# theEricMa/TriplaneTurbo

Hardware: AMD Instinct MI355X
Metric: rendered rays/sec (fwd+bwd) at 256x256 rays x 128 samples (higher is better)
Workload: dtype f32 (fp32-grade: exact 3-piece fp16 operand split, 6 x v_mfma_f32_32x32x16_f16 per k-step, fp32 accumulation)

## Files before the change

### include/tt_abi.h

```cpp
#ifndef TT_ABI_H
#define TT_ABI_H

#include <stdint.h>

#ifdef __cplusplus
extern "C" {
#endif

#define TT_ABI_VERSION 17
#define TT_CHANNELS 32
#define TT_HIDDEN 64

typedef enum {
    TT_OK = 0,
    TT_ERR_BAD_ARG = -1,
    TT_ERR_UNSUPPORTED = -2,
    TT_ERR_LAUNCH = -3,
    TT_ERR_DEVICE = -4
} tt_status;

typedef struct {
    const float* w1;
    const float* w2;
    const float* w3;
    const float* v1;
    const float* v2;
    const float* v3;
} tt_mlp_weights;

typedef struct {
    float* w1;
    float* w2;
    float* w3;
    float* v1;
    float* v2;
    float* v3;
} tt_mlp_grads;

typedef struct {
    int32_t n_prompts;
    int32_t views_per_prompt;
    int32_t plane_h, plane_w;
    int32_t rays_per_view;
    int32_t n_samples;
    int64_t n_rays;
    float radius;
    float sdf_bias_radius;
    float inv_std;
    float cos_anneal_ratio;
    float rgb_grad_shrink;
    int32_t flags;
    int32_t image_w;
    int32_t tile_sb;
    int32_t grad_copies;
    int32_t tile_chunk;
    float skip_eps_tex;
    float skip_eps_geo;
    const float* inv_std_dev;
    uint64_t* stats;
} tt_render_cfg;

#define TT_R_PER_SAMPLE 1
#define TT_R_EXACT_F32 2
#define TT_R_SPLIT2 32
#define TT_R_SPLIT3 64

#define TT_R_VOLSDF 128

#define TT_R_WGRAD_F32 4
#define TT_R_BWD_SOLO 8
#define TT_R_BWD_PAIR 16

#define TT_Q_NORMAL 1
#define TT_Q_TEX 2
#define TT_Q_EXACT_F32 4
#define TT_Q_SPLIT2 8
#define TT_Q_SPLIT3 16

const char* tt_strerror(int status);
int tt_abi_version(void);
const char* tt_source_hash(void);
int tt_debug_poison_queue(void* stream);

int tt_planes_pack(const float* space_cache, float* packed, int32_t n_prompts, int32_t plane_h, int32_t plane_w,
                   void* stream);
int tt_planes_unpack_grad(const float* grad_packed, float* grad_space_cache, int32_t n_prompts, int32_t plane_h,
                          int32_t plane_w, int32_t n_copies, void* stream);

int tt_query_points(const float* packed, const tt_mlp_weights* w, const float* points, int32_t n_batch,
                    int64_t n_points, int32_t n_prompts, int32_t views_per_prompt, int32_t plane_h, int32_t plane_w,
                    float radius, float sdf_bias_radius, int32_t flags, float* out_sdf, float* out_sdf_grad,
                    float* out_features, void* stream);

int tt_query_field(const float* packed, const tt_mlp_weights* w, const float* points, int32_t n_batch,
                   int64_t n_points, int32_t n_prompts, int32_t views_per_prompt, int32_t plane_h, int32_t plane_w,
                   float radius, float sdf_bias_radius, int32_t flags, float* out_sdf, float* out_deformation,
                   void* stream);

int tt_decode_rays(const float* packed, const tt_mlp_weights* w, const float* rays_o, const float* rays_d,
                   const float* t_starts, const float* t_ends, const tt_render_cfg* cfg, int32_t flags, float* sdf,
                   float* sdf_grad, float* features, void* stream);

enum tt_sample_placement { TT_PLACE_TT = 0, TT_PLACE_CENTER = 1 };
#define TT_PLACE_VOLSDF 0x100

int tt_sample_uniform(int64_t n_rays, int32_t n_samples, float near_plane, float far_plane, const float* jitter,
                      int32_t placement, float* t_starts, float* t_ends, void* stream);

int tt_sample_importance(const float* t_starts, const float* t_ends, const float* sdf, int64_t n_rays,
                         int32_t n_proposal, int32_t n_fine, float inv_std, const float* inv_std_dev,
                         float render_step_size, const float* u_jitter, int32_t placement, float* out_t_starts,
                         float* out_t_ends, void* stream);

int tt_render_fwd(const float* packed, const tt_mlp_weights* w, const float* rays_o, const float* rays_d,
                  const float* t_starts, const float* t_ends, const tt_render_cfg* cfg, float* opacity, float* depth,
                  float* rgb_fg, float* z_variance, float* normal_acc, float* weights, float* trans, float* sdf,
                  float* sdf_grad, float* features, void* stream);

int tt_render_fwd_h2mask(const float* packed, const tt_mlp_weights* w, const float* rays_o, const float* rays_d,
                         const float* t_starts, const float* t_ends, const tt_render_cfg* cfg, float* opacity,
                         float* depth, float* rgb_fg, float* z_variance, float* normal_acc, float* weights, float* trans,
                         float* sdf, float* sdf_grad, float* features, uint32_t* h2_mask, void* stream);

int tt_render_eval(const float* packed, const tt_mlp_weights* w, const float* rays_o, const float* rays_d,
                   const float* t_starts, const float* t_ends, const tt_render_cfg* cfg, float transmittance_eps,
                   float weight_eps, float* opacity, float* depth, float* rgb_fg, float* z_variance, float* normal_acc,
                   uint64_t* stats, void* stream);

int tt_march_fwd(const float* rays_d, const float* t_starts, const float* t_ends, const tt_render_cfg* cfg,
                 const float* sdf, const float* sdf_grad, const float* features, float* opacity, float* depth,
                 float* rgb_fg, float* z_variance, float* normal_acc, float* weights, float* trans, void* stream);

int tt_march_bwd(const float* rays_d, const float* t_starts, const float* t_ends, const tt_render_cfg* cfg,
                 const float* opacity, const float* depth, const float* trans, const float* sdf,
                 const float* sdf_grad, const float* features, const float* g_opacity, const float* g_depth,
                 const float* g_rgb_fg, const float* g_z_variance, const float* g_normal_acc, const float* g_weights,
                 const float* g_sdf, const float* g_sdf_grad, float* g_inv_std_rays, float* out_grad, void* stream);

int tt_render_bwd_geo(const float* packed, const tt_mlp_weights* w, const float* rays_o, const float* rays_d,
                      const float* t_starts, const float* t_ends, const tt_render_cfg* cfg, const float* opacity,
                      const float* depth, const float* trans, const float* sdf, const float* sdf_grad,
                      const float* features, const float* g_opacity, const float* g_depth, const float* g_rgb_fg,
                      const float* g_z_variance, const float* g_normal_acc, const float* g_weights,
                      const float* g_sdf, const float* g_sdf_grad, float* g_inv_std_rays, float* workspace,
                      float* grad_packed, const tt_mlp_grads* grads, void* stream);

int tt_render_bwd_geo_h2mask(const float* packed, const tt_mlp_weights* w, const float* rays_o, const float* rays_d,
                             const float* t_starts, const float* t_ends, const tt_render_cfg* cfg,
                             const float* opacity, const float* depth, const float* trans, const float* sdf,
                             const float* sdf_grad, const float* features, const float* g_opacity,
                             const float* g_depth, const float* g_rgb_fg, const float* g_z_variance,
                             const float* g_normal_acc, const float* g_weights, const float* g_sdf,
                             const float* g_sdf_grad, float* g_inv_std_rays, float* workspace, float* grad_packed,
                             const tt_mlp_grads* grads, const uint32_t* h2_mask, void* stream);

int tt_render_bwd_tex(const float* packed, const tt_mlp_weights* w, const float* rays_o, const float* rays_d,
                      const float* t_starts, const float* t_ends, const tt_render_cfg* cfg, const float* weights,
                      const float* features, const float* g_rgb_fg, const float* g_features, float* grad_packed,
                      const tt_mlp_grads* grads, void* stream);

int tt_points_bwd_geo(const float* packed, const tt_mlp_weights* w, const float* points, int32_t n_batch,
                      int64_t n_points, int32_t n_prompts, int32_t views_per_prompt, int32_t plane_h, int32_t plane_w,
                      float radius, float sdf_bias_radius, int32_t flags, const float* g_sdf, const float* g_sdf_grad,
                      float* workspace, float* grad_packed, const tt_mlp_grads* grads, void* stream);
int tt_points_bwd_tex(const float* packed, const tt_mlp_weights* w, const float* points, int32_t n_batch,
                      int64_t n_points, int32_t n_prompts, int32_t views_per_prompt, int32_t plane_h, int32_t plane_w,
                      float radius, int32_t plane_base, int32_t flags, const float* g_features, float* grad_packed,
                      const tt_mlp_grads* grads, void* stream);

int tt_points_bwd_x(const float* packed, const tt_mlp_weights* w, const float* points, int32_t n_batch,
                    int64_t n_points, int32_t n_prompts, int32_t views_per_prompt, int32_t plane_h, int32_t plane_w,
                    float radius, int32_t flags, const float* g_sdf, const float* g_sdf_grad, const float* g_features,
                    float* grad_points, void* stream);

typedef struct {
    int32_t n_levels;
    int32_t n_features_per_level;
    int32_t log2_hashmap_size;
    int32_t base_resolution;
    float per_level_scale;
} tt_hashgrid_cfg;
int64_t tt_hashgrid_n_params(const tt_hashgrid_cfg* cfg);
int tt_hashgrid_fwd(const float* x, int64_t n, const float* params, const tt_hashgrid_cfg* cfg, float* out,
                    void* stream);
int tt_hashgrid_bwd(const float* x, int64_t n, const float* g_out, const tt_hashgrid_cfg* cfg, float* grad_params,
                    void* stream);

int tt_patch_composite_fwd(const float* low, const float* patch, float* out, int32_t B, int32_t h, int32_t w, int32_t H,
                           int32_t W, int32_t C, int32_t PS, int32_t py, int32_t px, void* stream);
int tt_patch_composite_bwd(const float* g_out, float* g_low, float* g_patch, int32_t B, int32_t h, int32_t w, int32_t H,
                           int32_t W, int32_t C, int32_t PS, int32_t py, int32_t px, void* stream);

int tt_eikonal_fwd(const float* sdf_grad, int64_t n, float* loss, void* stream);
int tt_eikonal_bwd(const float* sdf_grad, const float* g_loss, int64_t n, float* g_sdf_grad, void* stream);

int tt_composite_fwd(const float* opacity, const float* depth, const float* rgb_fg, const float* normal_acc,
                     const float* bg, int32_t bg_stride, const float* camera_distances, const float* c2w, int64_t n_rays,
                     int32_t rays_per_view, int32_t mode, int32_t view_group, float* comp_rgb, float* disparity,
                     float* comp_normal, float* normal_cam_vis, float* normal_cam_vis_white, void* stream);
int tt_composite_bwd(const float* opacity, const float* depth, const float* rgb_fg, const float* normal_acc,
                     const float* bg, int32_t bg_stride, const float* camera_distances, const float* c2w, int64_t n_rays,
                     int32_t rays_per_view, int32_t mode, int32_t view_group, const float* g_comp_rgb,
                     const float* g_disparity, const float* g_comp_normal, const float* g_normal_cam_vis,
                     const float* g_normal_cam_vis_white, float* g_opacity, float* g_depth, float* g_rgb_fg,
                     float* g_normal_acc, float* g_bg, void* stream);

#define TT_DTYPE_F32 0
#define TT_DTYPE_F16 1
#define TT_DTYPE_F64 2
int tt_grid_sample_2d_grad2_typed(int32_t dtype, const void* grad2_grad_input, const void* grad2_grad_grid,
                                  const void* grad_output, const void* input, const void* grid, int32_t n, int32_t c,
                                  int32_t h, int32_t w, int64_t n_points_per_batch, int32_t padding_mode,
                                  int32_t align_corners, void* grad_grad_output, void* grad_input, void* grad_grid,
                                  void* stream);
int tt_grid_sample_2d_grad2(const float* grad2_grad_input, const float* grad2_grad_grid, const float* grad_output,
                            const float* input, const float* grid, int32_t n, int32_t c, int32_t h, int32_t w,
                            int64_t n_points_per_batch, int32_t padding_mode, int32_t align_corners,
                            float* grad_grad_output, float* grad_input, float* grad_grid, void* stream);

#define TT_MC_MAX_RES 512
int64_t tt_mc_workspace_bytes(int32_t res);
int tt_mc_count(const float* level, int32_t res, float isovalue, void* workspace, int32_t* out_totals, void* stream);
int tt_mc_emit(const float* level, const float* deformation, int32_t res, float isovalue, void* workspace, float* v_pos,
               int32_t* t_pos_idx, void* stream);
int tt_mc_bwd(const float* level, const float* deformation, int32_t res, float isovalue, void* workspace,
              const float* grad_v, float* grad_level, float* grad_deformation, void* stream);

int64_t tt_mt_workspace_bytes(int32_t n_edges, int32_t n_tets);
int tt_mt_count(const float* level, const int32_t* edges, const int32_t* tets, int32_t n_edges, int32_t n_tets,
                void* workspace, int32_t* out_totals, void* stream);
int tt_mt_emit(const float* pos, const float* level, const int32_t* edges, const int32_t* tet_edge, int32_t n_edges,
               int32_t n_tets, void* workspace, float* v_pos, int32_t* t_pos_idx, void* stream);
int tt_mt_bwd(const float* pos, const float* level, const int32_t* edges, const int32_t* vert_ptr,
              const int32_t* vert_col, int32_t n_vertices, int32_t n_edges, int32_t n_tets, void* workspace,
              const float* grad_v, float* grad_level, float* grad_pos, void* stream);

#define TT_RAST_MAX_TRIS (1 << 24)
int64_t tt_rast_workspace_bytes(int32_t B, int32_t T, int32_t H, int32_t W);
int tt_rast_fwd(const float* pos, const int32_t* tri, int32_t B, int32_t V, int32_t T, int32_t H, int32_t W,
                void* workspace, float* rast, void* stream);
int tt_rast_bwd(const float* pos, const int32_t* tri, const float* rast, const float* grad_rast, int32_t B, int32_t V,
                int32_t T, int32_t H, int32_t W, float* grad_pos, void* stream);
int tt_interp_fwd(const float* attr, int32_t attr_batch, const float* rast, const int32_t* tri, int32_t B, int32_t V,
                  int32_t T, int32_t H, int32_t W, int32_t C, float* out, void* stream);
int tt_interp_bwd(const float* attr, int32_t attr_batch, const float* rast, const int32_t* tri, const float* grad_out,
                  int32_t B, int32_t V, int32_t T, int32_t H, int32_t W, int32_t C, float* grad_attr, float* grad_rast,
                  void* stream);
int tt_aa_fwd(const float* color, const float* rast, const float* pos, const int32_t* tri, const int32_t* edge_ofs,
              const int32_t* edge_tri, int32_t B, int32_t V, int32_t T, int32_t H, int32_t W, int32_t C, float* out,
              void* stream);
int tt_aa_bwd(const float* color, const float* rast, const float* pos, const int32_t* tri, const int32_t* edge_ofs,
              const int32_t* edge_tri, const float* grad_out, int32_t B, int32_t V, int32_t T, int32_t H, int32_t W,
              int32_t C, float* grad_color, float* grad_pos, void* stream);
int64_t tt_rast_range_workspace_bytes(int32_t B, int64_t n_slots, int32_t H, int32_t W);
int tt_rast_range_fwd(const float* pos, const int32_t* tri, const int32_t* ranges_dev, const int32_t* ranges_host,
                      int32_t B, int32_t V, int32_t T, int32_t H, int32_t W, void* workspace, float* rast,
                      void* stream);
int tt_rast_range_bwd(const float* pos, const int32_t* tri, const float* rast, const float* grad_rast, int32_t B,
                      int32_t V, int32_t T, int32_t H, int32_t W, float* grad_pos, void* stream);
int tt_aa_range_fwd(const float* color, const float* rast, const float* pos, const int32_t* tri,
                    const int32_t* edge_ofs, const int32_t* edge_tri, int32_t B, int32_t V, int32_t T, int32_t H,
                    int32_t W, int32_t C, float* out, void* stream);
int tt_aa_range_bwd(const float* color, const float* rast, const float* pos, const int32_t* tri,
                    const int32_t* edge_ofs, const int32_t* edge_tri, const float* grad_out, int32_t B, int32_t V,
                    int32_t T, int32_t H, int32_t W, int32_t C, float* grad_color, float* grad_pos, void* stream);

#define TT_TEX_FILTER_NEAREST 0
#define TT_TEX_FILTER_LINEAR 1
#define TT_TEX_BOUNDARY_WRAP 0
#define TT_TEX_BOUNDARY_CLAMP 1
#define TT_TEX_BOUNDARY_ZERO 2
#define TT_TEX_MAX_SIZE 16777216
int tt_tex_fwd(const float* tex, int32_t tex_batch, const float* uv, int32_t B, int32_t H, int32_t W, int32_t TH,
               int32_t TW, int32_t C, int32_t filter, int32_t boundary, float* out, void* stream);
int tt_tex_bwd(const float* tex, int32_t tex_batch, const float* uv, const float* grad_out, int32_t B, int32_t H,
               int32_t W, int32_t TH, int32_t TW, int32_t C, int32_t filter, int32_t boundary, float* grad_tex,
               float* grad_uv, void* stream);

#define TT_MESH_MAX_ITEMS (1 << 28)
#define TT_MESH_COS_EPS 1e-8f
int64_t tt_mesh_workspace_bytes(int32_t V, int32_t T);
int tt_mesh_components(const int32_t* face_pairs, int32_t P, int32_t T, void* workspace, int32_t* labels,
                       void* stream);
int tt_mesh_compact_count(const int32_t* t_pos_idx, const int32_t* labels, int32_t V, int32_t T, int32_t frac_mode,
                          double frac, int64_t threshold, void* workspace, int32_t* out_totals, void* stream);
int tt_mesh_compact_emit(const float* v_pos, const int32_t* t_pos_idx, int32_t V, int32_t T, void* workspace,
                         float* v_out, int32_t* t_out, void* stream);
int tt_mesh_laplacian_fwd(const float* v_pos, const int32_t* nbr_ptr, const int32_t* nbr_col, int32_t V, int32_t T,
                          void* workspace, float* loss, void* stream);
int tt_mesh_laplacian_bwd(const float* v_pos, const int32_t* nbr_ptr, const int32_t* nbr_col, int32_t V, int32_t T,
                          const float* grad_loss, void* workspace, float* grad_v, void* stream);
int tt_mesh_nc_fwd(const float* v_nrm, const int32_t* edges, int32_t V, int32_t T, int32_t E, void* workspace,
                   float* loss, void* stream);
int tt_mesh_nc_bwd(const float* v_nrm, const int32_t* nbr_ptr, const int32_t* nbr_col, int32_t V, int32_t E,
                   const float* grad_loss, float* grad_nrm, void* stream);

#define TT_UV_DEFAULT_ROUNDS 8
#define TT_UV_DEFAULT_TAU 0.3f
#define TT_UV_MAX_TAU 0.577f
#define TT_UV_MAX_SMOOTH_ROUNDS 1024
#define TT_UV_MAX_FACES ((1 << 24) - 1)
#define TT_UV_MAX_TEX 16384
#define TT_UV_MAX_PADDING 256
#define TT_UV_MAX_CHANNELS 64
#define TT_UV_MAX_OVERLAP_ROUNDS 4
#define TT_UV_PACK_REL_PREC 1e-4
int64_t tt_uv_workspace_bytes(int32_t V, int32_t T, int32_t N);
int tt_uv_labels(const float* v_pos, const int32_t* t_pos_idx, const int32_t* face_pairs, int32_t V, int32_t T,
                 int32_t P, int32_t rounds, float tau, int32_t N, void* workspace, int32_t* labels, void* stream);
int tt_uv_charts(const float* v_pos, const int32_t* t_pos_idx, const int32_t* face_pairs, const int32_t* labels,
                 const uint8_t* singleton, int32_t V, int32_t T, int32_t P, int32_t N, void* workspace, int32_t* chart,
                 float* chart_box, int32_t* out_totals, void* stream);
int tt_uv_pack(const float* chart_box, int32_t C, int32_t N, int32_t padding, int32_t* offsets, float* scale);
int tt_uv_emit_count(const int32_t* t_pos_idx, const int32_t* chart, int32_t V, int32_t T, int32_t N, void* workspace,
                     int32_t* out_totals, void* stream);
int tt_uv_emit(const float* v_pos, const int32_t* t_pos_idx, const int32_t* labels, const int32_t* chart,
               const float* chart_box, const int32_t* offsets, int32_t C, float scale, int32_t V, int32_t T, int32_t N,
               int32_t padding, void* workspace, float* v_tex, int32_t* t_tex_idx, void* stream);
int tt_uv_overlap(const float* v_tex, const int32_t* t_tex_idx, int32_t Vt, int32_t V, int32_t T, int32_t N,
                  void* workspace, uint8_t* flags, int32_t* out_totals, void* stream);
int64_t tt_tex_fill_workspace_bytes(int32_t H, int32_t W);
int tt_tex_fill(const float* img, const uint8_t* mask, int32_t H, int32_t W, int32_t C, void* workspace, float* out,
                void* stream);

#define TT_SIMPLIFY_MIN_GRID 2
#define TT_SIMPLIFY_MAX_GRID 1024
#define TT_SIMPLIFY_MAX_CLUSTERS 2097151
int64_t tt_simplify_workspace_bytes(int32_t V, int32_t T);
int tt_simplify_keys(const float* v_pos, int32_t V, int32_t grid, float lo_x, float lo_y, float lo_z, float inv_h,
                     int64_t* keys, void* stream);
int tt_simplify_ranks(const int64_t* sorted_keys, const int64_t* perm, int32_t V, int32_t T, int32_t grid,
                      void* workspace, int32_t* rank, int32_t* out_totals, void* stream);
int tt_simplify_pairs(const int32_t* t_pos_idx, const int32_t* rank, int32_t V, int32_t T, int32_t C, void* workspace,
                      int64_t* pair_keys, void* stream);
int tt_simplify_solve(const float* v_pos, const int32_t* t_pos_idx, const int64_t* sorted_pair_keys,
                      const int64_t* perm, int32_t V, int32_t T, int32_t C, int32_t grid, float lo_x, float lo_y,
                      float lo_z, float h, double lam, void* workspace, float* cluster_pos, void* stream);
int tt_simplify_faces(const int32_t* t_pos_idx, const int32_t* rank, int32_t V, int32_t T, int32_t C,
                      int64_t* face_keys, void* stream);
int tt_simplify_emit_count(const int64_t* sorted_face_keys, const int64_t* face_perm, const int32_t* t_pos_idx,
                           const int32_t* rank, int32_t V, int32_t T, int32_t C, void* workspace, int32_t* out_totals,
                           void* stream);
int tt_simplify_emit(const float* cluster_pos, const int32_t* t_pos_idx, const int32_t* rank, int32_t V, int32_t T,
                     int32_t C, void* workspace, float* v_out, int32_t* t_out, int32_t* vertex_map, void* stream);

#define TT_BAKE_GROUP_POS 0
#define TT_BAKE_GROUP_TEX 1
#define TT_BAKE_MAX_POINTS 268435456
int tt_bake_tangents(const float* v_pos, const int32_t* t_pos_idx, const float* v_tex, const int32_t* t_tex_idx,
                     const float* v_nrm, const int32_t* group_ptr, const int32_t* group_corner, int32_t V, int32_t Vt,
                     int32_t T, int32_t group, float* out, void* stream);
int tt_bake_project(float* points, const float* sdf, const float* sdf_grad, const uint8_t* mask, int64_t M,
                    float max_step, void* stream);
int tt_bake_encode(const float* rast, const float* v_nrm, const int32_t* t_pos_idx, const float* tng_tex,
                   const int32_t* t_tex_idx, const float* field_nrm, int32_t V, int32_t Vt, int32_t T, int32_t H,
                   int32_t W, float* out, int32_t* out_counts, void* stream);

#define TT_DIST_MAX_GRID 256
#define TT_DIST_MAX_SAMPLES (1 << 26)
int64_t tt_dist_workspace_bytes(int32_t grid);
int tt_dist_build_count(const float* v_pos, const int32_t* t_pos_idx, int32_t V, int32_t T, int32_t grid, float lo_x,
                        float lo_y, float lo_z, float ext, float inv_h, void* workspace, float* records,
                        int32_t* cell_ptr, int64_t* out_total, void* stream);
int tt_dist_build_fill(const float* records, int32_t T, int32_t grid, float lo_x, float lo_y, float lo_z, float ext,
                       float inv_h, void* workspace, const int32_t* cell_ptr, int32_t M, int32_t* cell_tri,
                       void* stream);
int tt_dist_keys(const float* points, int32_t N, int32_t grid, float lo_x, float lo_y, float lo_z, float ext,
                 float inv_h, int64_t* keys, void* stream);
int tt_dist_query(const float* points, const int64_t* order, int32_t N, const float* records, const int32_t* cell_ptr,
                  const int32_t* cell_tri, int32_t T, int32_t M, int32_t grid, float lo_x, float lo_y, float lo_z,
                  float ext, float h, float inv_h, float* d2, int32_t* face, float* bary, void* stream);
int tt_dist_bwd(const float* points, const float* v_pos, const int32_t* t_pos_idx, const int32_t* face,
                const float* bary, const float* g_d2, int32_t N, int32_t V, int32_t T, float* grad_points,
                float* grad_v_pos, void* stream);
int64_t tt_dist_sample_workspace_bytes(int32_t T);
int tt_dist_sample_count(const float* v_pos, const int32_t* t_pos_idx, int32_t V, int32_t T, float spacing,
                         void* workspace, int64_t* offsets, void* stream);
int tt_dist_sample_emit(const float* v_pos, const int32_t* t_pos_idx, const int64_t* offsets, int32_t V, int32_t T,
                        float spacing, int32_t S, float* points, int32_t* face, void* stream);

#define TT_WIND_MAX_LEVELS 6
int64_t tt_wind_node_count(int32_t levels);
int tt_wind_face_keys(const float* v_pos, const int32_t* t_pos_idx, int32_t V, int32_t T, int32_t levels, float lo_x,
                      float lo_y, float lo_z, float ext, float inv_h, float* records, int64_t* keys, void* stream);
int tt_wind_build(const float* sorted_records, const int32_t* leaf_ptr, int32_t T, int32_t levels, float* nodes,
                  void* stream);
int tt_wind_point_keys(const float* points, int32_t N, int32_t levels, float lo_x, float lo_y, float lo_z, float ext,
                       float inv_h, int64_t* keys, void* stream);
int tt_wind_exact(const float* points, int32_t N, const float* records, int32_t T, float* out, void* stream);
int tt_wind_fast(const float* points, const int64_t* order, int32_t N, const float* sorted_records,
                 const int32_t* leaf_ptr, const float* nodes, int32_t T, int32_t levels, float beta, float* out,
                 void* stream);

#define TT_RAY_MAX_DIRS 1024
int tt_ray_cast(const float* origins, const float* dirs, const int64_t* order, int32_t N, float t_max,
                const float* records, const int32_t* cell_ptr, const int32_t* cell_tri, int32_t T, int32_t M,
                int32_t grid, float lo_x, float lo_y, float lo_z, float ext, float h, float inv_h, float* t,
                int32_t* face, float* bary, void* stream);
int tt_ray_any(const float* origins, const float* dirs, const int64_t* order, int32_t N, float t_max,
               const float* records, const int32_t* cell_ptr, const int32_t* cell_tri, int32_t T, int32_t M,
               int32_t grid, float lo_x, float lo_y, float lo_z, float ext, float h, float inv_h, uint8_t* hit,
               void* stream);
int tt_ray_ao(const float* points, const float* normals, const float* dirs_local, int32_t N, int32_t K, float bias,
              float max_distance, const float* records, const int32_t* cell_ptr, const int32_t* cell_tri, int32_t T,
              int32_t M, int32_t grid, float lo_x, float lo_y, float lo_z, float ext, float h, float inv_h,
              int32_t* hits, void* stream);

#ifdef __cplusplus
}
#endif
#endif
```

### triplaneturbo_amd/csrc/tt_backward.hip

```cpp
#include "tt_backward_common.h"

struct BwdGeoParams {
    const float* packed;
    MlpPtrs w;
    const float* rays_o;
    const float* rays_d;
    const float* t_starts;
    const float* t_ends;
    tt_render_cfg cfg;
    TileGeom geom;
    long long n_items;
    int* queue;
    const float* ws;
    const unsigned* h2_mask;
    int n_copies;
    float* grad_packed;
    MlpGradPtrs grads;
    unsigned long long* phase_cycles;
};

#define GEO_SCRATCH_FLOATS (2 * 64 * XS)
template <int PREC, bool FMASK>
struct GeoMap : LdsMap<PREC, LdsImage<64, 32>, LdsImage<64, 64, !(FMASK && PREC != PREC_F32)>, LdsRows<1, 64>,
                       LdsImage<32, 64>, LdsImage<64, 64>> {
    static constexpr bool NOW2 = FMASK && PREC != PREC_F32;
    typedef typename GeoMap::template at<0> W1;
    typedef typename GeoMap::template at<1> W2;
    typedef typename GeoMap::template at<2> W3;
    typedef typename GeoMap::template at<3> W1T;
    typedef typename GeoMap::template at<4> CT;
};

template <int PREC, bool STATS = false, bool FMASK = false>
__global__ __launch_bounds__(256, 1) void k_decode_bwd_geo(BwdGeoParams p) {
    constexpr bool EXACT = PREC == PREC_F32;
    constexpr bool WG16 = !EXACT;
    typedef GeoMap<PREC, FMASK> G;
    constexpr int NT = PrecNT<PREC>::value, WF = G::FLOATS;
    __shared__ __attribute__((aligned(16))) float L[WF + 4 * (GEO_SCRATCH_FLOATS + SCATTER_TAG_INTS)];
    stage_weights<PREC>(L, typename G::W1{}, p.w.w1);
    if constexpr (!G::NOW2) stage_weights<PREC>(L, typename G::W2{}, p.w.w2);
    stage_weights<PREC>(L, typename G::W3{}, p.w.w3);
    stage_weights_t<PREC>(L, typename G::W1T{}, p.w.w1);
    if constexpr (!EXACT) stage_image16_rowscaled_t<NT>(L, typename G::CT{}, p.w.w2, p.w.w3);
    const tt_render_cfg& cfg = p.cfg;
    float sA1 = 1.f, sU = 1.f, sV = 1.f;
    if (WG16) {
        const unsigned* bnd = reinterpret_cast<const unsigned*>(p.queue) + TT_SLOT_BOUNDS;
        const float Pm = __builtin_bit_cast(float, bnd[TT_BOUND_PLANES]), Sb = __builtin_bit_cast(float, bnd[TT_BOUND_UP0]),
                    Gb = __builtin_bit_cast(float, bnd[TT_BOUND_UP1]);
        unsigned* word = reinterpret_cast<unsigned*>(L + WF);
        const int t = threadIdx.x;
        float w1row = 0.f, a1col = 0.f;
        if (t < 64) {
            for (int c = 0; c < 32; ++c) w1row += __builtin_fabsf(p.w.w1[t * 32 + c]);
            for (int r = 0; r < 64; ++r) a1col += __builtin_fabsf(p.w.w2[r * 64 + t]) * __builtin_fabsf(p.w.w3[r]);
        }
        const float W1max = block_max(w1row, word), A1max = block_max(a1col, word);
        const float jsum = (0.5f * cfg.plane_w + 0.5f * cfg.plane_h) / cfg.radius;
        const float Fmax = 3.f * Pm, H1max = W1max * Fmax;
        const float Umax = Fmax * (Sb + 2.f * jsum * Gb), QBmax = Fmax * 2.f * jsum * Gb;
        const float Vmax = Sb * H1max + W1max * QBmax;
        sA1 = wg16_scale(A1max);
        sU = wg16_scale(Umax);
        sV = wg16_scale(Vmax);
    }
    const TileGeom& tg = p.geom;
    const int lane = threadIdx.x & 63, i = lane & 31, hi = lane >> 5, wave_in_blk = threadIdx.x >> 6;
    float* Xs = L + WF + wave_in_blk * (GEO_SCRATCH_FLOATS + SCATTER_TAG_INTS);
    float* Ys = Xs + 64 * XS;
    int* tags = reinterpret_cast<int*>(Ys + 64 * XS);
    scatter_init_tags(tags, lane);
    __syncthreads();
    const int S = cfg.n_samples;
    ItemQueue iq = item_queue(p.queue, tg.n_blocks, tg.n_chunks, tg.unit);
    const int H = cfg.plane_h, W = cfg.plane_w;
    const size_t HW = (size_t)H * W;
    const size_t plane_stride = 6 * HW * TT_C;
    const float ju = 0.5f * W / cfg.radius, jv = 0.5f * H / cfg.radius;
    float* const grad_out =
        p.grad_packed + (size_t)(blockIdx.x % (unsigned)p.n_copies) * cfg.n_prompts * plane_stride;
    const unsigned grad_bytes =
        TT_DBG(cfg.flags, TT_DBG_NO_ATOMICS) ? 0u : (unsigned)(cfg.n_prompts * plane_stride * sizeof(float));

    const TileStats st = STATS ? tile_stats(cfg.stats) : TileStats{nullptr};
    f32x16 accW1[2][1] = {{ZERO16}, {ZERO16}};
    f32x16 accW2[2][2] = {{ZERO16, ZERO16}, {ZERO16, ZERO16}};
#ifdef TT_TUNING
    unsigned long long ph_acc[20] = {0, 0, 0, 0, 0, 0, 0, 0, 0, 0, 0, 0, 0, 0, 0, 0, 0, 0, 0, 0};
    unsigned long long ph_t = __builtin_amdgcn_s_memtime();
#endif

#pragma nounroll
    for (;;) {
        long long b;
        int ck;
        if (!item_pop(iq, tg.order, tg.n_chunks, b, ck)) break;
        if (b >= tg.n_blocks) continue;
        bool ray_ok;
        const long long ray = tile_ray(tg, b, i, ray_ok);
        const float ray_okf = tt_opaque(ray_ok ? 1.f : 0.f);
        const int ks = i % tg.sb;
        const int view = (int)(ray / cfg.rays_per_view);
        const size_t pofs = (size_t)(view / cfg.views_per_prompt) * plane_stride;
        const float ox = p.rays_o[ray * 3 + 0], oy = p.rays_o[ray * 3 + 1], oz = p.rays_o[ray * 3 + 2];
        const float dx = p.rays_d ? p.rays_d[ray * 3 + 0] : 0.f, dy = p.rays_d ? p.rays_d[ray * 3 + 1] : 0.f,
                    dz = p.rays_d ? p.rays_d[ray * 3 + 2] : 0.f;
        const int s_end = (ck + 1) * tg.chunk < S ? (ck + 1) * tg.chunk : S;
        struct StepIn {
            f32x4 up;
            float ts, te;
            unsigned m2;
        };
        auto load_step = [&](int sb0) {
            StepIn r;
            const int si = sb0 + ks;
            const long long sidx = ray * S + (si < S ? si : S - 1);
            r.up = *reinterpret_cast<const f32x4*>(p.ws + sidx * 4);
            r.ts = p.rays_d ? p.t_starts[sidx] : 0.f;
            r.te = p.rays_d ? p.t_ends[sidx] : 0.f;
            r.m2 = FMASK ? p.h2_mask[2 * sidx + hi] : 0u;
            return r;
        };
        StepIn in = load_step(ck * tg.chunk), in_next;
#pragma nounroll
        for (int sb0 = ck * tg.chunk; sb0 < s_end; sb0 += tg.sb, in = in_next) {
            in_next = load_step(sb0 + tg.sb);
            const int si = sb0 + ks;
            const bool rvalid = ray_ok && si < s_end;
            const float vf = ray_okf * (si < s_end ? 1.f : 0.f);
            const float sbar = in.up[0] * vf, gbx = in.up[1] * vf, gby = in.up[2] * vf, gbz = in.up[3] * vf;
            tile_stat(st, TT_STAT_VISITED);
            TT_PHASE(0);
            if (!__any(!((__builtin_fabsf(sbar) + __builtin_fabsf(gbx)) + (__builtin_fabsf(gby) + __builtin_fabsf(gbz)) <=
                         cfg.skip_eps_geo)))
                continue;
            float tm, px, py, pz;
            sample_position(ox, oy, oz, dx, dy, dz, in.ts, in.te, tm, px, py, pz);
            const float X = scale_coord(px, cfg.radius), Y = scale_coord(py, cfg.radius),
                        Z = scale_coord(pz, cfg.radius);
            float f[16], u[16];
            unsigned pmask;
            const bool any = __any(gather_geo_bwd_c(p.packed, (unsigned)(pofs / TT_C), H, W, X, Y, Z, rvalid, sbar, gbx,
                                                    gby, gbz, ju, jv, lane, Xs, f, u, pmask,
                                                    tile_stat_ptr(st, TT_STAT_INBOUNDS)));
            TT_PHASE(1);
            if (!any) continue;
            const bool one = single_plane(pmask);
            tile_stat_executed(st, one);
            float h1[32], h2[32], a1[32], q[16], u1, uh2;
            mvx<PREC, true>(L, typename G::W1{}, f, h1, i, hi, 1.f, &u1);
#pragma unroll
            for (int r = 0; r < 32; ++r) h1[r] = fmaxf(h1[r], 0.f);
            const unsigned m2w = FMASK ? in.m2 & (0u - (unsigned)vf) : 0u;
            if constexpr (!FMASK) {
                mvx<PREC, true>(L, typename G::W2{}, h1, h2, i, hi, u1, &uh2);
#pragma unroll
                for (int r = 0; r < 32; ++r) h2[r] = fmaxf(h2[r], 0.f);
            } else if constexpr (EXACT) {
#pragma unroll
                for (int r = 0; r < 32; ++r) h2[r] = (float)((m2w >> r) & 1u);
            }
            unsigned m2p[16];
            Split16<64, PAIR_SEQ, NT> a1s;
            float ua1 = 1.f;
            if (WG16) {
                if constexpr (FMASK)
                    mask16_pairs_bits<64>(m2w, m2p);
                else
                    mask16_pairs<64>(h2, m2p);
                mv16_mask<NT>(L, typename G::CT{}, m2p, a1, i, hi, &ua1);
            } else {
                float a2[32];
#pragma unroll
                for (int g = 0; g < 8; ++g) {
                    f32x4 w3 = *reinterpret_cast<const f32x4*>(lds_at(L, typename G::W3{}) + 8 * g + 4 * hi);
#pragma unroll
                    for (int e2 = 0; e2 < 4; ++e2) a2[4 * g + e2] = h2[4 * g + e2] > 0.f ? w3[e2] : 0.f;
                }
                mvtx_copy<PREC>(L, typename G::CT{}, typename G::W2{}, a2, a1, i, hi);
            }
#pragma unroll
            for (int r = 0; r < 32; ++r) a1[r] = h1[r] > 0.f ? a1[r] : 0.f;
            float uq = 1.f;
            if (WG16) {
                split16_vec<64, PAIR_SEQ, NT>(a1, sA1 * ua1, a1s);
                mv16_pre<true, true>(L, typename G::W1T{}, a1s, 1.f / sA1, q, i, hi, &uq);
            } else {
                mvtx_copy<PREC>(L, typename G::W1T{}, typename G::W1{}, a1, q, i, hi);
            }
            TT_PHASE(3);
            {
                float qb[16];
#pragma unroll
                for (int r = 0; r < 16; ++r) qb[r] = fmaf(-sbar, f[r], u[r]);
                const bool region = WG16 || cfg.flags >= 0;
                const bool do_wgrad = region && !TT_DBG(cfg.flags, TT_DBG_NO_WGRAD);
                if (do_wgrad) {
                    if (WG16) {
                        stage_rows16_pre<64>(Xs, a1s, i, hi);
                        stage_rows16<32>(Ys, u, i, hi, sU);
                        wgrad16<64, 32>(accW1, Xs, Ys, i, hi);
                    } else {
                        stage_rows<64>(Xs, a1, i, hi);
                        stage_rows<32>(Ys, u, i, hi);
                        wgrad<64, 32>(accW1, Xs, Ys, i, hi);
                    }
                }
                TT_PHASE(7);
                float t1[32];
                mvx<PREC>(L, typename G::W1{}, qb, t1, i, hi);
#pragma unroll
                for (int r = 0; r < 32; ++r) t1[r] = h1[r] > 0.f ? t1[r] : 0.f;
                float v[32];
#pragma unroll
                for (int r = 0; r < 32; ++r) v[r] = fmaf(sbar * u1, h1[r], t1[r]);
                TT_PHASE(4);
                if (do_wgrad) {
                    if (WG16) {
                        stage_rows16_mask<64>(Xs, m2p, i, hi);
                        stage_rows16<64>(Ys, v, i, hi, sV);
                        wgrad16_mask<64, 64>(accW2, Xs, Ys, i, hi);
                    } else {
                        stage_rows_mask<64>(Xs, h2, i, hi);
                        stage_rows<64>(Ys, v, i, hi);
                        wgrad<64, 64>(accW2, Xs, Ys, i, hi);
                    }
                }
                TT_PHASE(8);
                if (region && !TT_DBG(cfg.flags, TT_DBG_NO_SCATTER)) {
                    scatter_clear<EXACT>(Xs, lane);
                    float* Qs = Xs + SCATTER_M_FLOATS;
                    TT_PHASE(9);
                    const int tex0 = (int)(pofs / TT_C);
                    auto corners = [&](int pl, PlaneRefs& refs) {
                        Corners c;
                        float coef[4];
                        geo_corner_coefs(pl, H, W, X, Y, Z, rvalid, sbar, gbx, gby, gbz, ju, jv, c, coef);
                        int aoff[4];
#pragma unroll
                        for (int q4 = 0; q4 < 4; ++q4) aoff[q4] = tex0 + (int)(pl * HW) + c.off[q4];
                        refs = plane_refs<!EXACT>(coef, aoff, c.hs, hi);
                    };
#ifdef TT_TUNING
                    unsigned long long* const sc_st = ph_acc + 14;
#else
                    unsigned long long* const sc_st = nullptr;
#endif
                    const ScatterQ<EXACT> sq{Qs, tags, i, hi};
                    if (one)
                        scatter_one_plane<EXACT>(grad_out, grad_bytes, sq, Xs, Qs + 32 * 33,
                                                 single_plane_index(pmask), corners, q, uq, sc_st);
                    else
                        scatter_planes<EXACT>(grad_out, grad_bytes, sq, Xs, Qs + 32 * 33, corners, [&](int) { return q; }, uq, sc_st);
                    TT_PHASE(10);
                }
            }
        }
    }
#ifdef TT_TUNING
    TT_PHASE(11);
    if (p.phase_cycles && lane == 0)
        for (int k = 0; k < 20; ++k) atomicAdd(p.phase_cycles + 20 + k, ph_acc[k]);
#endif
    __syncthreads();
    int parity = 0;
    flush_wgrad_reduced<64, 32>(L, parity, accW1, p.grads.w1, wave_in_blk, lane, 1.f / sA1, 1.f / sU);
    flush_d_reduced<64, 64>(L, parity, accW2, p.w.w2, p.w.w3, p.grads.w2, p.grads.w3, wave_in_blk, lane, 1.f / sV);
    tile_stats_flush(st);
}

#ifdef TT_TUNING
unsigned long long* g_phase_cycles = nullptr;
extern "C" int tt_tuning_phase_cycles(unsigned long long* out40) {
    if (!g_phase_cycles) {
        if (hipMalloc((void**)&g_phase_cycles, 40 * sizeof(unsigned long long)) != hipSuccess) return -4;
        if (hipMemset(g_phase_cycles, 0, 40 * sizeof(unsigned long long)) != hipSuccess) return -4;
    }
    if (hipDeviceSynchronize() != hipSuccess) return -4;
    if (out40 && hipMemcpy(out40, g_phase_cycles, 40 * sizeof(unsigned long long), hipMemcpyDeviceToHost) != hipSuccess)
        return -4;
    return hipMemset(g_phase_cycles, 0, 40 * sizeof(unsigned long long)) == hipSuccess ? 0 : -4;
}
#endif
static void launch_bwd_geo(const BwdGeoParams& p0, long long blocks, hipStream_t s) {
    BwdGeoParams p = p0;
#ifdef TT_TUNING
    p.phase_cycles = g_phase_cycles;
#else
    p.phase_cycles = nullptr;
#endif
    if (use_wg16(p.cfg)) {
        unsigned* bnd = reinterpret_cast<unsigned*>(p.queue) + TT_SLOT_BOUNDS;
        launch_planes_bound(p.packed, p.cfg, 0, bnd + TT_BOUND_PLANES, s);
        const long long n = p.cfg.n_rays * p.cfg.n_samples;
        hipLaunchKernelGGL(k_absmax4, dim3(absmax_blocks(n), 1), dim3(256), 0, s, reinterpret_cast<const f32x4*>(p.ws), n, n,
                           bnd + TT_BOUND_UP0, bnd + TT_BOUND_UP1);
    }
    tt_dispatch_prec(tt_prec_of_r(p.cfg.flags), [&](auto P) {
        constexpr int PREC = decltype(P)::value;
        const dim3 grid((unsigned)blocks), block(256);
        if (p.cfg.stats && p.h2_mask)
            hipLaunchKernelGGL((k_decode_bwd_geo<PREC, true, true>), grid, block, 0, s, p);
        else if (p.cfg.stats)
            hipLaunchKernelGGL((k_decode_bwd_geo<PREC, true>), grid, block, 0, s, p);
        else if (p.h2_mask)
            hipLaunchKernelGGL((k_decode_bwd_geo<PREC, false, true>), grid, block, 0, s, p);
        else
            hipLaunchKernelGGL((k_decode_bwd_geo<PREC>), grid, block, 0, s, p);
    });
}

static int render_bwd_geo(const float* packed, const tt_mlp_weights* w, const float* rays_o, const float* rays_d,
                          const float* t_starts, const float* t_ends, const tt_render_cfg* cfg, const float* opacity,
                          const float* depth, const float* trans, const float* sdf, const float* sdf_grad,
                          const float* features, const float* g_opacity, const float* g_depth, const float* g_rgb_fg,
                          const float* g_z_variance, const float* g_normal_acc, const float* g_weights,
                          const float* g_sdf, const float* g_sdf_grad, float* g_inv_std_rays, float* workspace,
                          float* grad_packed, const tt_mlp_grads* grads, const uint32_t* h2_mask, void* stream) {
    int st = tt_validate_cfg(cfg);
    if (st != TT_OK) return st;
    if (!packed || !w || !rays_o || !rays_d || !t_starts || !t_ends || !opacity || !depth || !trans || !sdf ||
        !sdf_grad || !features || !workspace || !grad_packed || !grads)
        return TT_ERR_BAD_ARG;
    if (!w->w1 || !w->w2 || !w->w3 || !grads->w1 || !grads->w2 || !grads->w3) return TT_ERR_BAD_ARG;
    if (grad_buffer_too_large(cfg)) return TT_ERR_UNSUPPORTED;
    int cus = tt_num_cus();
    if (cus <= 0) return TT_ERR_DEVICE;
    hipStream_t s = (hipStream_t)stream;
    st = tt_launch_march_bwd(rays_d, t_starts, t_ends, cfg, sdf, sdf_grad, features, trans, opacity, depth, g_opacity,
                             g_depth, g_rgb_fg, g_z_variance, g_normal_acc, g_weights, g_sdf, g_sdf_grad, g_inv_std_rays,
                             workspace, s);
    if (st != TT_OK) return st;
    BwdGeoParams p;
    tt_fill_rays(p, packed, w, rays_o, rays_d, t_starts, t_ends, *cfg);
    p.cfg.flags |= debug_flags();
    p.ws = workspace;
    p.h2_mask = h2_mask;
    p.grad_packed = grad_packed;
    p.n_copies = cfg->grad_copies > 0 ? cfg->grad_copies : 1;
    p.grads = to_gptrs(grads);
    st = tt_plan_queue(cfg, 4LL * cus, s, &p.geom, &p.n_items, &p.queue);
    if (st != TT_OK) return st;
    launch_bwd_geo(p, tt_persistent_blocks(p.n_items, cus, 4), s);
    return tt_check_launch();
}

extern "C" int tt_render_bwd_geo(const float* packed, const tt_mlp_weights* w, const float* rays_o,
                                 const float* rays_d, const float* t_starts, const float* t_ends,
                                 const tt_render_cfg* cfg, const float* opacity, const float* depth,
                                 const float* trans, const float* sdf, const float* sdf_grad, const float* features,
                                 const float* g_opacity, const float* g_depth, const float* g_rgb_fg,
                                 const float* g_z_variance, const float* g_normal_acc, const float* g_weights,
                                 const float* g_sdf, const float* g_sdf_grad, float* g_inv_std_rays, float* workspace,
                                 float* grad_packed, const tt_mlp_grads* grads, void* stream) {
    return render_bwd_geo(packed, w, rays_o, rays_d, t_starts, t_ends, cfg, opacity, depth, trans, sdf, sdf_grad, features,
                          g_opacity, g_depth, g_rgb_fg, g_z_variance, g_normal_acc, g_weights, g_sdf, g_sdf_grad,
                          g_inv_std_rays, workspace, grad_packed, grads, nullptr, stream);
}

extern "C" int tt_render_bwd_geo_h2mask(const float* packed, const tt_mlp_weights* w, const float* rays_o,
                                        const float* rays_d, const float* t_starts, const float* t_ends,
                                        const tt_render_cfg* cfg, const float* opacity, const float* depth,
                                        const float* trans, const float* sdf, const float* sdf_grad,
                                        const float* features, const float* g_opacity, const float* g_depth,
                                        const float* g_rgb_fg, const float* g_z_variance, const float* g_normal_acc,
                                        const float* g_weights, const float* g_sdf, const float* g_sdf_grad,
                                        float* g_inv_std_rays, float* workspace, float* grad_packed,
                                        const tt_mlp_grads* grads, const uint32_t* h2_mask, void* stream) {
    if (!h2_mask) return TT_ERR_BAD_ARG;
    return render_bwd_geo(packed, w, rays_o, rays_d, t_starts, t_ends, cfg, opacity, depth, trans, sdf, sdf_grad, features,
                          g_opacity, g_depth, g_rgb_fg, g_z_variance, g_normal_acc, g_weights, g_sdf, g_sdf_grad,
                          g_inv_std_rays, workspace, grad_packed, grads, h2_mask, stream);
}

__global__ void k_interleave_ws(const float* __restrict__ g_sdf, const float* __restrict__ g_sdf_grad,
                                float* __restrict__ ws, long long n) {
    const long long i = (long long)blockIdx.x * blockDim.x + threadIdx.x;
    if (i >= n) return;
    f32x4 o = {g_sdf ? g_sdf[i] : 0.f, g_sdf_grad ? g_sdf_grad[i * 3 + 0] : 0.f,
               g_sdf_grad ? g_sdf_grad[i * 3 + 1] : 0.f, g_sdf_grad ? g_sdf_grad[i * 3 + 2] : 0.f};
    *reinterpret_cast<f32x4*>(ws + i * 4) = o;
}

extern "C" int tt_points_bwd_geo(const float* packed, const tt_mlp_weights* w, const float* points, int32_t n_batch,
                                 int64_t n_points, int32_t n_prompts, int32_t views_per_prompt, int32_t plane_h,
                                 int32_t plane_w, float radius, float sdf_bias_radius, int32_t flags,
                                 const float* g_sdf, const float* g_sdf_grad, float* workspace, float* grad_packed,
                                 const tt_mlp_grads* grads, void* stream) {
    tt_render_cfg cfg;
    int st = points_cfg(&cfg, n_batch, n_points, n_prompts, views_per_prompt, plane_h, plane_w, radius,
                        sdf_bias_radius, 1, flags);
    if (st != TT_OK) return st;
    if (grad_buffer_too_large(&cfg)) return TT_ERR_UNSUPPORTED;
    if (!packed || !w || !points || !workspace || !grad_packed || !grads || (!g_sdf && !g_sdf_grad))
        return TT_ERR_BAD_ARG;
    if (!w->w1 || !w->w2 || !w->w3 || !grads->w1 || !grads->w2 || !grads->w3) return TT_ERR_BAD_ARG;
    int cus = tt_num_cus();
    if (cus <= 0) return TT_ERR_DEVICE;
    hipStream_t s = (hipStream_t)stream;
    const long long n = cfg.n_rays;
    hipLaunchKernelGGL(k_interleave_ws, dim3((unsigned)((n + 255) / 256)), dim3(256), 0, s, g_sdf, g_sdf_grad,
                       workspace, n);
    st = tt_check_launch();
    if (st != TT_OK) return st;
    BwdGeoParams p;
    tt_fill_rays(p, packed, w, points, nullptr, nullptr, nullptr, cfg);
    p.ws = workspace;
    p.h2_mask = nullptr;
    p.grad_packed = grad_packed;
    p.n_copies = 1;
    p.grads = to_gptrs(grads);
    st = tt_plan_queue(&cfg, 4LL * cus, s, &p.geom, &p.n_items, &p.queue);
    if (st != TT_OK) return st;
    launch_bwd_geo(p, tt_persistent_blocks(p.n_items, cus, 4), s);
    return tt_check_launch();
}
```

### triplaneturbo_amd/csrc/tt_device.h

```cpp
#pragma once
#include <hip/hip_runtime.h>
#include <stdint.h>

typedef float f32x16 __attribute__((ext_vector_type(16)));
typedef float f32x4 __attribute__((ext_vector_type(4)));

#ifdef TT_TUNING
#define TT_DBG(flags, bit) (((flags) & (bit)) != 0)
#else
#define TT_DBG(flags, bit) false
#endif
#define TT_DBG_NO_SCATTER 0x100
#define TT_DBG_NO_WGRAD 0x200
#define TT_DBG_NO_GATHER 0x400
#define TT_DBG_NO_MLP 0x800
#define TT_DBG_NO_STORE 0x1000
#define TT_DBG_NO_ATOMICS 0x2000

#define TT_C 32
#define TT_TILE 32

#define LIDX(r, hi) (((r) & 3) + 8 * ((r) >> 2) + 4 * (hi))

#include "tt_mask.h"
// ... 25 lines not shown
#pragma unroll
    for (int m = 0; m < MT; ++m) {
        acc[m] = f32x16{0.f, 0.f, 0.f, 0.f, 0.f, 0.f, 0.f, 0.f, 0.f, 0.f, 0.f, 0.f, 0.f, 0.f, 0.f, 0.f};
        a_cur[m] = *reinterpret_cast<const f32x4*>(row + 32 * m * (NIN + 4));
    }
#pragma unroll
    for (int g = 0; g < NIN / 8; ++g) {
        if (g + 1 < NIN / 8) {
#pragma unroll
            for (int m = 0; m < MT; ++m)
                a_nxt[m] = *reinterpret_cast<const f32x4*>(row + 32 * m * (NIN + 4) + 8 * (g + 1));
        }
#pragma unroll
        for (int k = 0; k < 4; ++k)
#pragma unroll
            for (int m = 0; m < MT; ++m)
                acc[m] = __builtin_amdgcn_mfma_f32_32x32x2f32(a_cur[m][k], x[4 * g + k], acc[m], 0, 0, 0);
#pragma unroll
        for (int m = 0; m < MT; ++m) a_cur[m] = a_nxt[m];
    }
#pragma unroll
    for (int m = 0; m < MT; ++m)
#pragma unroll
        for (int k = 0; k < 16; ++k) y[16 * m + k] = acc[m][k];
}

template <int NOUT, int NIN, int NG>
__device__ __forceinline__ void mv_fwd_cols(const float* Wl, const float (&x)[4 * NG], int g0, float (&y)[NOUT / 2], int i,
                                            int hi) {
    constexpr int MT = NOUT / 32;
    f32x16 acc[MT];
    const float* row = Wl + i * (NIN + 4) + 4 * hi + 8 * g0;
#pragma unroll
    for (int m = 0; m < MT; ++m)
        acc[m] = f32x16{0.f, 0.f, 0.f, 0.f, 0.f, 0.f, 0.f, 0.f, 0.f, 0.f, 0.f, 0.f, 0.f, 0.f, 0.f, 0.f};
#pragma unroll
    for (int g = 0; g < NG; ++g) {
        f32x4 a[MT];
#pragma unroll
        for (int m = 0; m < MT; ++m) a[m] = *reinterpret_cast<const f32x4*>(row + 32 * m * (NIN + 4) + 8 * g);
#pragma unroll
        for (int k = 0; k < 4; ++k)
#pragma unroll
            for (int m = 0; m < MT; ++m)
                acc[m] = __builtin_amdgcn_mfma_f32_32x32x2f32(a[m][k], x[4 * g + k], acc[m], 0, 0, 0);
    }
#pragma unroll
    for (int m = 0; m < MT; ++m)
#pragma unroll
        for (int k = 0; k < 16; ++k) y[16 * m + k] = acc[m][k];
}

template <int NOUT, int NIN, int STRIDE = NOUT + 4>
__device__ __forceinline__ void mv_bwd(const float* Wl, const float (&x)[NIN / 2], float (&y)[NOUT / 2], int i,
                                       int hi) {
    constexpr int MT = NOUT / 32;
    const float* base = Wl + 4 * hi * STRIDE + i;
    if (MT == 1) {
        f32x16 acc0 = {0.f, 0.f, 0.f, 0.f, 0.f, 0.f, 0.f, 0.f, 0.f, 0.f, 0.f, 0.f, 0.f, 0.f, 0.f, 0.f};
        f32x16 acc1 = acc0;
#pragma unroll
        for (int r = 0; r < NIN / 4; ++r) {
            const float a0 = base[LIDX(r, 0) * STRIDE], a1 = base[LIDX(r + NIN / 4, 0) * STRIDE];
            acc0 = __builtin_amdgcn_mfma_f32_32x32x2f32(a0, x[r], acc0, 0, 0, 0);
            acc1 = __builtin_amdgcn_mfma_f32_32x32x2f32(a1, x[r + NIN / 4], acc1, 0, 0, 0);
        }
#pragma unroll
        for (int k = 0; k < 16; ++k) y[k] = acc0[k] + acc1[k];
    } else {
        f32x16 acc[MT];
#pragma unroll
        for (int m = 0; m < MT; ++m)
            acc[m] = f32x16{0.f, 0.f, 0.f, 0.f, 0.f, 0.f, 0.f, 0.f, 0.f, 0.f, 0.f, 0.f, 0.f, 0.f, 0.f, 0.f};
#pragma unroll
        for (int r = 0; r < NIN / 2; ++r) {
#pragma unroll
            for (int m = 0; m < MT; ++m) {
                const float a = base[LIDX(r, 0) * STRIDE + 32 * m];
                acc[m] = __builtin_amdgcn_mfma_f32_32x32x2f32(a, x[r], acc[m], 0, 0, 0);
            }
        }
#pragma unroll
        for (int m = 0; m < MT; ++m)
#pragma unroll
            for (int k = 0; k < 16; ++k) y[16 * m + k] = acc[m][k];
    }
}

template <int N>
__device__ __forceinline__ float dot_lds(const float* wl, const float (&x)[N / 2], int hi) {
    float s = 0.f;
#pragma unroll
    for (int g = 0; g < N / 8; ++g) {
        f32x4 a = *reinterpret_cast<const f32x4*>(wl + 8 * g + 4 * hi);
        s = fmaf(a[0], x[4 * g + 0], s);
        s = fmaf(a[1], x[4 * g + 1], s);
        s = fmaf(a[2], x[4 * g + 2], s);
        s = fmaf(a[3], x[4 * g + 3], s);
    }
    return s + __shfl_xor(s, 32);
}

struct Corners {
    int off[4];
    float w[4];
    float du[4];
    float dv[4];
    int hs[4];
    bool any;
    int inmask;
};

#pragma clang fp contract(off)
__device__ __forceinline__ void corners_setup(float gx, float gy, int H, int W, bool valid, Corners& c) {
    gx = __builtin_fabsf(gx) < 1e30f ? gx : 4.f;
    gy = __builtin_fabsf(gy) < 1e30f ? gy : 4.f;
    float ix = ((gx + 1.f) * (float)W - 1.f) / 2.f;
    float iy = ((gy + 1.f) * (float)H - 1.f) / 2.f;
    float fx = floorf(ix), fy = floorf(iy);
    float wx1 = ix - fx, wx0 = (fx + 1.f) - ix;
    float wy1 = iy - fy, wy0 = (fy + 1.f) - iy;
    int x0 = (int)fminf(fmaxf(fx, -2.f), (float)W + 1.f);
    int y0 = (int)fminf(fmaxf(fy, -2.f), (float)H + 1.f);
    x0 = valid ? x0 : -2;
    const float bx0 = (unsigned)x0 < (unsigned)W ? 1.f : 0.f, bx1 = (unsigned)(x0 + 1) < (unsigned)W ? 1.f : 0.f;
    const float by0 = (unsigned)y0 < (unsigned)H ? 1.f : 0.f, by1 = (unsigned)(y0 + 1) < (unsigned)H ? 1.f : 0.f;
    const float mx0 = wx0 * bx0, mx1 = wx1 * bx1, my0 = wy0 * by0, my1 = wy1 * by1;
    c.w[0] = mx0 * my0;
    c.w[1] = mx1 * my0;
    c.w[2] = mx0 * my1;
    c.w[3] = mx1 * my1;
    c.du[0] = -(my0 * bx0);
    c.du[1] = my0 * bx1;
    c.du[2] = -(my1 * bx0);
    c.du[3] = my1 * bx1;
    c.dv[0] = -(mx0 * by0);
    c.dv[1] = -(mx1 * by0);
    c.dv[2] = mx0 * by1;
    c.dv[3] = mx1 * by1;
    const int xc0 = min(max(x0, 0), W - 1), xc1 = min(max(x0 + 1, 0), W - 1);
    const int yc0 = min(max(y0, 0), H - 1) * W, yc1 = min(max(y0 + 1, 0), H - 1) * W;
    c.off[0] = yc0 + xc0;
    c.off[1] = yc0 + xc1;
    c.off[2] = yc1 + xc0;
    c.off[3] = yc1 + xc1;
    const float i0 = bx0 * by0, i1 = bx1 * by0, i2 = bx0 * by1, i3 = bx1 * by1;
    c.hs[0] = ((y0 & 15) << 4) | (x0 & 15);
    c.hs[1] = ((y0 & 15) << 4) | ((x0 + 1) & 15);
    c.hs[2] = (((y0 + 1) & 15) << 4) | (x0 & 15);
    c.hs[3] = (((y0 + 1) & 15) << 4) | ((x0 + 1) & 15);
    c.any = (bx0 + bx1) * (by0 + by1) != 0.f;
    c.inmask = (int)i0 | ((int)i1 << 1) | ((int)i2 << 2) | ((int)i3 << 3);
}

__device__ __forceinline__ float scale_coord(float x, float radius) {
    float t = (x - (-radius)) / (radius - (-radius));
    return t * 2.f + (-1.f);
}

__device__ __forceinline__ void sample_position(float ox, float oy, float oz, float dx, float dy, float dz, float ts,
                                                float te, float& tm, float& px, float& py, float& pz) {
    tm = (ts + te) / 2.f;
    px = ox + dx * tm;
    py = oy + dy * tm;
    pz = oz + dz * tm;
}

__device__ __forceinline__ float sphere_bias(float px, float py, float pz, float bias_radius, float& nrm) {
    nrm = sqrtf((px * px + py * py) + pz * pz);
    return nrm - bias_radius;
}
#pragma clang fp contract(fast)

#define PLANE_U(p, X, Y, Z) ((p) == 2 ? (Z) : (X))
#define PLANE_V(p, X, Y, Z) ((p) == 1 ? (Z) : (Y))

template <bool NEED_J>
__device__ __forceinline__ bool gather_geo(const float* __restrict__ planes, int H, int W, float X, float Y, float Z,
                                           bool valid, float jscale_u, float jscale_v, int hi, float (&f)[16],
                                           float (&jx)[16], float (&jy)[16], float (&jz)[16], int dbg = 0) {
#pragma unroll
    for (int r = 0; r < 16; ++r) {
        f[r] = 0.f;
        jx[r] = 0.f;
        jy[r] = 0.f;
        jz[r] = 0.f;
    }
    bool any = false;
    const size_t HW = (size_t)H * W;
#pragma unroll
    for (int p = 0; p < 3; ++p) {
        Corners c;
        corners_setup(PLANE_U(p, X, Y, Z), PLANE_V(p, X, Y, Z), H, W, valid, c);
        if (!__any(c.any)) continue;
        any = any || c.any;
#pragma unroll
        for (int k = 0; k < 4; ++k) {
            const f32x4* t = reinterpret_cast<const f32x4*>(planes + (p * HW + (size_t)c.off[k]) * TT_C) + hi;
            f32x4 v[4];
            if (TT_DBG(dbg, TT_DBG_NO_GATHER)) {
                const f32x4 z = {c.w[k], c.du[k], c.dv[k], X};
                v[0] = v[1] = v[2] = v[3] = z;
            } else {
                v[0] = t[0];
                v[1] = t[2];
                v[2] = t[4];
                v[3] = t[6];
            }
            const float wk = c.w[k], a = c.du[k] * jscale_u, b = c.dv[k] * jscale_v;
#pragma unroll
            for (int q = 0; q < 4; ++q)
#pragma unroll
                for (int e = 0; e < 4; ++e) {
                    const float tv = v[q][e];
                    f[4 * q + e] = fmaf(wk, tv, f[4 * q + e]);
                    if (NEED_J) {
                        if (p == 0) {
                            jx[4 * q + e] = fmaf(a, tv, jx[4 * q + e]);
                            jy[4 * q + e] = fmaf(b, tv, jy[4 * q + e]);
                        } else if (p == 1) {
                            jx[4 * q + e] = fmaf(a, tv, jx[4 * q + e]);
                            jz[4 * q + e] = fmaf(b, tv, jz[4 * q + e]);
                        } else {
                            jz[4 * q + e] = fmaf(a, tv, jz[4 * q + e]);
                            jy[4 * q + e] = fmaf(b, tv, jy[4 * q + e]);
                        }
                    }
                }
        }
    }
    return any;
}

__device__ __forceinline__ bool gather_tex(const float* __restrict__ planes, int H, int W, float X, float Y, float Z,
                                           bool valid, int hi, float (&e)[48], int dbg = 0) {
#pragma unroll
    for (int r = 0; r < 48; ++r) e[r] = 0.f;
    bool any = false;
    const size_t HW = (size_t)H * W;
#pragma unroll
    for (int p = 0; p < 3; ++p) {
        Corners c;
        corners_setup(PLANE_U(p, X, Y, Z), PLANE_V(p, X, Y, Z), H, W, valid, c);
        if (!__any(c.any)) continue;
        any = any || c.any;
#pragma unroll
        for (int k = 0; k < 4; ++k) {
            const f32x4* t = reinterpret_cast<const f32x4*>(planes + ((3 + p) * HW + (size_t)c.off[k]) * TT_C) + hi;
            f32x4 v[4];
            if (TT_DBG(dbg, TT_DBG_NO_GATHER)) {
                const f32x4 z = {c.w[k], Y, Z, X};
                v[0] = v[1] = v[2] = v[3] = z;
            } else {
                v[0] = t[0];
                v[1] = t[2];
                v[2] = t[4];
                v[3] = t[6];
            }
            const float wk = c.w[k];
#pragma unroll
            for (int q = 0; q < 4; ++q)
#pragma unroll
                for (int ee = 0; ee < 4; ++ee) e[16 * p + 4 * q + ee] = fmaf(wk, v[q][ee], e[16 * p + 4 * q + ee]);
        }
    }
    return any;
}

struct TileStats {
    unsigned long long* p;
    unsigned* w;
};
enum { TT_STAT_VISITED = 0, TT_STAT_EXECUTED = 1, TT_STAT_INBOUNDS = 2, TT_STAT_SINGLE = 3 };
__device__ __forceinline__ TileStats tile_stats(uint64_t* stats64) {
    TileStats st = {nullptr, nullptr};
    __shared__ unsigned tt_stat_slots[16 * 4];
    st.p = reinterpret_cast<unsigned long long*>(stats64);
    if (st.p) {
        st.w = tt_stat_slots + 4 * __builtin_amdgcn_readfirstlane((int)(threadIdx.x >> 6));
        if ((threadIdx.x & 63) < 4) st.w[threadIdx.x & 63] = 0u;
    }
    return st;
}
__device__ __forceinline__ void tile_stat(const TileStats& st, int which, unsigned v = 1) {
    if (st.p) {
        if ((threadIdx.x & 63) == 0) st.w[which] += v;
    }
}
__device__ __forceinline__ void tile_stat_executed(const TileStats& st, bool single) {
    if (st.p) {
        if ((threadIdx.x & 63) == 0) {
            st.w[TT_STAT_EXECUTED] += 1u;
            st.w[TT_STAT_SINGLE] += single ? 1u : 0u;
        }
    }
}
__device__ __forceinline__ unsigned* tile_stat_ptr(const TileStats& st, int which) { return st.p ? st.w + which : nullptr; }
__device__ __forceinline__ void tile_stats_flush(const TileStats& st) {
    if (st.p) {
        const int l = threadIdx.x & 63;
        if (l < 4) atomicAdd(st.p + l, (unsigned long long)st.w[l]);
    }
}

__device__ __forceinline__ bool single_plane(unsigned pmask) { return pmask != 0u && (pmask & (pmask - 1u)) == 0u; }
__device__ __forceinline__ int single_plane_index(unsigned pmask) { return __builtin_ctz(pmask | 8u); }
__device__ __forceinline__ void live_block16(const float (&e)[48], float (&e1)[16]) {
#pragma unroll
    for (int r = 0; r < 16; ++r)
        e1[r] = __builtin_bit_cast(float, __builtin_bit_cast(unsigned, e[r]) | __builtin_bit_cast(unsigned, e[16 + r]) |
                                              __builtin_bit_cast(unsigned, e[32 + r]));
}

typedef int ti32x4 __attribute__((ext_vector_type(4)));
#define GC_TABLE_FLOATS(NW) (3 * 32 * 4 * (1 + (NW)))
#define GC_TILE_FLOATS (32 * 36)

#define GC_PLANE_TABLE_FLOATS (32 * 16)
#define GC_SCRATCH_FLOATS (GC_PLANE_TABLE_FLOATS + GC_TILE_FLOATS)

__device__ __forceinline__ const f32x4* gc_addr(const float* __restrict__ planes, int texel, unsigned cbyte) {
    return reinterpret_cast<const f32x4*>(reinterpret_cast<const char*>(planes) + (((unsigned)texel << 7) | cbyte));
}

__device__ __forceinline__ void gc_load16(const float* __restrict__ pl, const int* Toff, int js, f32x4 (&t)[4][4]) {
#pragma unroll
    for (int n = 0; n < 4; ++n) {
        const ti32x4 o4 = *reinterpret_cast<const ti32x4*>(Toff + (8 * n + js) * 4);
#pragma unroll
        for (int k = 0; k < 4; ++k) t[n][k] = *reinterpret_cast<const f32x4*>(pl + (size_t)(unsigned)o4[k] * TT_C);
    }
}

__device__ __forceinline__ void gc_transpose(float* R, const f32x4 (&acc)[4], int i, int hi, int js, int c,
                                             float* out16) {
#pragma unroll
    for (int n = 0; n < 4; ++n) *reinterpret_cast<f32x4*>(R + (8 * n + js) * 36 + 4 * c) = acc[n];
#pragma unroll
    for (int q = 0; q < 4; ++q) {
        const f32x4 v = *reinterpret_cast<const f32x4*>(R + i * 36 + 4 * (hi + 2 * q));
#pragma unroll
        for (int ee = 0; ee < 4; ++ee) out16[4 * q + ee] = v[ee];
    }
}

template <bool NEED_J>
__device__ __forceinline__ bool gather_geo_c(const float* __restrict__ planes, unsigned tex0, int H, int W, float X,
                                             float Y, float Z, bool valid, float jscale_u, float jscale_v, int lane,
                                             float* T, float (&f)[16], float (&jx)[16], float (&jy)[16],
                                             float (&jz)[16], unsigned& pmask, unsigned* inb = nullptr) {
    const int i = lane & 31, hi = lane >> 5, js = lane >> 3, c = lane & 7;
    int* Toff = reinterpret_cast<int*>(T);
    float* Tw = T + 32 * 4;
    float* Ta = T + 2 * 32 * 4;
    float* Tb = T + 3 * 32 * 4;
    float* R = T + GC_PLANE_TABLE_FLOATS;
    const size_t HW = (size_t)H * W;
    const f32x4 z4 = {0.f, 0.f, 0.f, 0.f};
    f32x4 af[4] = {z4, z4, z4, z4}, ax[4] = {z4, z4, z4, z4}, ay[4] = {z4, z4, z4, z4}, az[4] = {z4, z4, z4, z4};
    bool any = false;
    pmask = 0u;
#pragma unroll
    for (int p = 0; p < 3; ++p) {
        Corners cn;
        corners_setup(PLANE_U(p, X, Y, Z), PLANE_V(p, X, Y, Z), H, W, valid, cn);
        any = any || cn.any;
        const unsigned long long inmask = __ballot(cn.any);
        if (inb) {
            if ((threadIdx.x & 63) == 0) *inb += (unsigned)__popcll(inmask & 0xffffffffull);
        }
        if (inmask == 0) continue;
        pmask |= 1u << p;
        if (hi == 0) {
            const unsigned b = tex0 + (unsigned)(p * HW);
            const ti32x4 o = {(int)(b + cn.off[0]), (int)(b + cn.off[1]), (int)(b + cn.off[2]), (int)(b + cn.off[3])};
            *reinterpret_cast<ti32x4*>(Toff + i * 4) = o;
            const f32x4 w = {cn.w[0], cn.w[1], cn.w[2], cn.w[3]};
            *reinterpret_cast<f32x4*>(Tw + i * 4) = w;
        } else if (NEED_J) {
            const f32x4 a = {cn.du[0] * jscale_u, cn.du[1] * jscale_u, cn.du[2] * jscale_u, cn.du[3] * jscale_u};
            const f32x4 b = {cn.dv[0] * jscale_v, cn.dv[1] * jscale_v, cn.dv[2] * jscale_v, cn.dv[3] * jscale_v};
            *reinterpret_cast<f32x4*>(Ta + i * 4) = a;
            *reinterpret_cast<f32x4*>(Tb + i * 4) = b;
        }
        f32x4 t[4][4];
        gc_load16(planes + 4 * c, Toff, js, t);
#pragma unroll
        for (int n = 0; n < 4; ++n) {
            const f32x4 w4 = *reinterpret_cast<const f32x4*>(Tw + (8 * n + js) * 4);
            f32x4 a4 = z4, b4 = z4;
            if (NEED_J) {
                a4 = *reinterpret_cast<const f32x4*>(Ta + (8 * n + js) * 4);
                b4 = *reinterpret_cast<const f32x4*>(Tb + (8 * n + js) * 4);
            }
#pragma unroll
            for (int k = 0; k < 4; ++k)
#pragma unroll
                for (int ee = 0; ee < 4; ++ee) {
                    const float tv = t[n][k][ee];
                    af[n][ee] = fmaf(w4[k], tv, af[n][ee]);
                    if (NEED_J) {
                        if (p == 0) {
                            ax[n][ee] = fmaf(a4[k], tv, ax[n][ee]);
                            ay[n][ee] = fmaf(b4[k], tv, ay[n][ee]);
                        } else if (p == 1) {
                            ax[n][ee] = fmaf(a4[k], tv, ax[n][ee]);
                            az[n][ee] = fmaf(b4[k], tv, az[n][ee]);
                        } else {
                            az[n][ee] = fmaf(a4[k], tv, az[n][ee]);
                            ay[n][ee] = fmaf(b4[k], tv, ay[n][ee]);
                        }
                    }
                }
        }
    }
    gc_transpose(R, af, i, hi, js, c, f);
    if (NEED_J) {
        gc_transpose(R, ax, i, hi, js, c, jx);
        gc_transpose(R, ay, i, hi, js, c, jy);
        gc_transpose(R, az, i, hi, js, c, jz);
    }
    return any;
}

__device__ __forceinline__ bool gather_tex_cp(const float* __restrict__ planes, unsigned tex0, int H, int W, float X,
                                              float Y, float Z, bool valid, int lane, float* T, float (&e)[48],
                                              unsigned& pmask) {
    const int i = lane & 31, hi = lane >> 5, js = lane >> 3, c = lane & 7;
    int* Toff = reinterpret_cast<int*>(T);
    float* Tw = T + 32 * 4;
    float* R = T + GC_PLANE_TABLE_FLOATS;
    const size_t HW = (size_t)H * W;
    bool any = false;
    pmask = 0u;
#pragma unroll
    for (int p = 0; p < 3; ++p) {
        Corners cn;
        corners_setup(PLANE_U(p, X, Y, Z), PLANE_V(p, X, Y, Z), H, W, valid, cn);
        any = any || cn.any;
        if (!__any(cn.any)) {
#pragma unroll
            for (int r = 0; r < 16; ++r) e[16 * p + r] = 0.f;
            continue;
        }
        pmask |= 1u << p;
        if (hi == 0) {
            const unsigned b = tex0 + (unsigned)((3 + p) * HW);
            const ti32x4 o = {(int)(b + cn.off[0]), (int)(b + cn.off[1]), (int)(b + cn.off[2]), (int)(b + cn.off[3])};
            *reinterpret_cast<ti32x4*>(Toff + i * 4) = o;
        } else {
            const f32x4 w = {cn.w[0], cn.w[1], cn.w[2], cn.w[3]};
            *reinterpret_cast<f32x4*>(Tw + i * 4) = w;
        }
        f32x4 t[4][4], acc[4];
        gc_load16(planes + 4 * c, Toff, js, t);
#pragma unroll
        for (int n = 0; n < 4; ++n) {
            const f32x4 w4 = *reinterpret_cast<const f32x4*>(Tw + (8 * n + js) * 4);
            f32x4 a = {0.f, 0.f, 0.f, 0.f};
#pragma unroll
            for (int k = 0; k < 4; ++k)
#pragma unroll
                for (int ee = 0; ee < 4; ++ee) a[ee] = fmaf(w4[k], t[n][k][ee], a[ee]);
            acc[n] = a;
        }
        gc_transpose(R, acc, i, hi, js, c, &e[16 * p]);
    }
    return any;
}

__device__ __forceinline__ bool gather_tex_c(const float* __restrict__ planes, unsigned tex0, int H, int W, float X,
                                             float Y, float Z, bool valid, int lane, float* T, float (&e)[48],
                                             unsigned& pmask, unsigned* inb = nullptr) {
    const int i = lane & 31, hi = lane >> 5, js = lane >> 3, c = lane & 7;
    int* Toff = reinterpret_cast<int*>(T);
    float* Tw = T + 3 * 32 * 4;
    float* R = T + GC_TABLE_FLOATS(1);
    const size_t HW = (size_t)H * W;
    bool any = false, anyp[3];
    pmask = 0u;
#pragma unroll
    for (int p = 0; p < 3; ++p) {
        Corners cn;
        corners_setup(PLANE_U(p, X, Y, Z), PLANE_V(p, X, Y, Z), H, W, valid, cn);
        const unsigned long long inmask = __ballot(cn.any);
        if (inb) {
            if ((threadIdx.x & 63) == 0) *inb += (unsigned)__popcll(inmask & 0xffffffffull);
        }
        anyp[p] = inmask != 0;
        pmask |= anyp[p] ? 1u << p : 0u;
        any = any || cn.any;
        if (hi == 0) {
            const unsigned b = tex0 + (unsigned)((3 + p) * HW);
            const ti32x4 o = {(int)(b + cn.off[0]), (int)(b + cn.off[1]), (int)(b + cn.off[2]), (int)(b + cn.off[3])};
            *reinterpret_cast<ti32x4*>(Toff + (p * 32 + i) * 4) = o;
        } else {
            const f32x4 w = {cn.w[0], cn.w[1], cn.w[2], cn.w[3]};
            *reinterpret_cast<f32x4*>(Tw + (p * 32 + i) * 4) = w;
        }
    }
#pragma unroll
    for (int p = 0; p < 3; ++p) {
        if (!anyp[p]) {
#pragma unroll
            for (int r = 0; r < 16; ++r) e[16 * p + r] = 0.f;
            continue;
        }
        f32x4 acc[4];
#pragma unroll
        for (int n = 0; n < 4; ++n) {
            const int sidx = (p * 32 + 8 * n + js) * 4;
            const ti32x4 o4 = *reinterpret_cast<const ti32x4*>(Toff + sidx);
            const f32x4 w4 = *reinterpret_cast<const f32x4*>(Tw + sidx);
            f32x4 a = {0.f, 0.f, 0.f, 0.f};
#pragma unroll
            for (int k = 0; k < 4; ++k) {
                const f32x4 t = *gc_addr(planes, o4[k], 16u * (unsigned)c);
#pragma unroll
                for (int ee = 0; ee < 4; ++ee) a[ee] = fmaf(w4[k], t[ee], a[ee]);
            }
            acc[n] = a;
        }
#pragma unroll
        for (int n = 0; n < 4; ++n) *reinterpret_cast<f32x4*>(R + (8 * n + js) * 36 + 4 * c) = acc[n];
#pragma unroll
        for (int q = 0; q < 4; ++q) {
            const f32x4 v = *reinterpret_cast<const f32x4*>(R + i * 36 + 4 * (hi + 2 * q));
#pragma unroll
            for (int ee = 0; ee < 4; ++ee) e[16 * p + 4 * q + ee] = v[ee];
        }
    }
    return any;
}

__device__ __forceinline__ void geo_corner_coefs(int p, int H, int W, float X, float Y, float Z, bool valid, float sbar,
                                                 float gux, float guy, float guz, float jscale_u, float jscale_v,
                                                 Corners& cn, float (&coef)[4]) {
    corners_setup(PLANE_U(p, X, Y, Z), PLANE_V(p, X, Y, Z), H, W, valid, cn);
    const float gu = (p == 2 ? guz : gux) * jscale_u, gv = (p == 1 ? guz : guy) * jscale_v;
#pragma unroll
    for (int k = 0; k < 4; ++k) coef[k] = fmaf(cn.w[k], sbar, fmaf(cn.du[k], gu, cn.dv[k] * gv));
}

__device__ __forceinline__ bool gather_geo_bwd_c(const float* __restrict__ planes, unsigned tex0, int H, int W, float X,
                                                 float Y, float Z, bool valid, float sbar, float gux, float guy,
                                                 float guz, float jscale_u, float jscale_v, int lane, float* T,
                                                 float (&f)[16], float (&u)[16], unsigned& pmask,
                                                 unsigned* inb = nullptr) {
    const int i = lane & 31, hi = lane >> 5, js = lane >> 3, c = lane & 7;
    int* Toff = reinterpret_cast<int*>(T);
    float* Tw = T + 3 * 32 * 4;
    float* Tc = T + 2 * 3 * 32 * 4;
    float* R = T + GC_TABLE_FLOATS(2);
    const size_t HW = (size_t)H * W;
    bool any = false, anyp[3];
    pmask = 0u;
#pragma unroll
    for (int p = 0; p < 3; ++p) {
        Corners cn;
        float coef[4];
        geo_corner_coefs(p, H, W, X, Y, Z, valid, sbar, gux, guy, guz, jscale_u, jscale_v, cn, coef);
        const unsigned long long inmask = __ballot(cn.any);
        if (inb) {
            if ((threadIdx.x & 63) == 0) *inb += (unsigned)__popcll(inmask & 0xffffffffull);
        }
        anyp[p] = inmask != 0;
        pmask |= anyp[p] ? 1u << p : 0u;
        any = any || cn.any;
        if (hi == 0) {
            const unsigned b = tex0 + (unsigned)(p * HW);
            const ti32x4 o = {(int)(b + cn.off[0]), (int)(b + cn.off[1]), (int)(b + cn.off[2]), (int)(b + cn.off[3])};
            *reinterpret_cast<ti32x4*>(Toff + (p * 32 + i) * 4) = o;
            const f32x4 w = {cn.w[0], cn.w[1], cn.w[2], cn.w[3]};
            *reinterpret_cast<f32x4*>(Tw + (p * 32 + i) * 4) = w;
        } else {
            const f32x4 w = {coef[0], coef[1], coef[2], coef[3]};
            *reinterpret_cast<f32x4*>(Tc + (p * 32 + i) * 4) = w;
        }
    }
    f32x4 af[4], au[4];
#pragma unroll
    for (int n = 0; n < 4; ++n) {
        const f32x4 z = {0.f, 0.f, 0.f, 0.f};
        af[n] = z;
        au[n] = z;
    }
#pragma unroll
    for (int p = 0; p < 3; ++p) {
        if (!anyp[p]) continue;
        f32x4 t[4][4];
#pragma unroll
        for (int n = 0; n < 4; ++n) {
            const ti32x4 o4 = *reinterpret_cast<const ti32x4*>(Toff + (p * 32 + 8 * n + js) * 4);
#pragma unroll
            for (int k = 0; k < 4; ++k)
                t[n][k] = *gc_addr(planes, o4[k], 16u * (unsigned)c);
        }
#pragma unroll
        for (int n = 0; n < 4; ++n) {
            const int sidx = (p * 32 + 8 * n + js) * 4;
            const f32x4 w4 = *reinterpret_cast<const f32x4*>(Tw + sidx);
            const f32x4 c4 = *reinterpret_cast<const f32x4*>(Tc + sidx);
#pragma unroll
            for (int k = 0; k < 4; ++k)
#pragma unroll
                for (int ee = 0; ee < 4; ++ee) {
                    af[n][ee] = fmaf(w4[k], t[n][k][ee], af[n][ee]);
                    au[n][ee] = fmaf(c4[k], t[n][k][ee], au[n][ee]);
                }
        }
    }
#pragma unroll
    for (int n = 0; n < 4; ++n) *reinterpret_cast<f32x4*>(R + (8 * n + js) * 36 + 4 * c) = af[n];
#pragma unroll
    for (int q = 0; q < 4; ++q) {
        const f32x4 v = *reinterpret_cast<const f32x4*>(R + i * 36 + 4 * (hi + 2 * q));
#pragma unroll
        for (int ee = 0; ee < 4; ++ee) f[4 * q + ee] = v[ee];
    }
#pragma unroll
    for (int n = 0; n < 4; ++n) *reinterpret_cast<f32x4*>(R + (8 * n + js) * 36 + 4 * c) = au[n];
#pragma unroll
    for (int q = 0; q < 4; ++q) {
        const f32x4 v = *reinterpret_cast<const f32x4*>(R + i * 36 + 4 * (hi + 2 * q));
#pragma unroll
        for (int ee = 0; ee < 4; ++ee) u[4 * q + ee] = v[ee];
    }
    return any;
}

struct ItemQueue {
    int* ctr;
    long long unit;
    long long nb;
    long long n_local;
    int home;
    int hop;
};
__device__ __forceinline__ ItemQueue item_queue(int* ctr, long long n_blocks, int n_chunks, long long unit) {
    ItemQueue q;
    q.ctr = ctr;
    q.unit = unit;
    const long long n_units = (n_blocks + unit - 1) / unit;
    q.nb = ((n_units + 7) / 8) * unit;
    q.n_local = q.nb * n_chunks;
    q.home = blockIdx.x & 7;
    q.hop = 0;
    return q;
}
__device__ __forceinline__ bool item_pop(ItemQueue& q, int order, int n_chunks, long long& b, int& ck) {
    while (q.hop < 8) {
        const int xcd = (q.home + q.hop) & 7;
        int li = 0;
        if ((threadIdx.x & 63) == 0) li = atomicAdd(q.ctr + xcd, 1);
        li = __builtin_amdgcn_readfirstlane(li);
        if (li < q.n_local) {
            long long bl;
            if (order == 0) {
                ck = (int)(li / q.nb);
                bl = li - (long long)ck * q.nb;
            } else {
                bl = li / n_chunks;
                ck = (int)(li - bl * n_chunks);
            }
            const long long round = bl / q.unit;
            b = (round * 8 + xcd) * q.unit + (bl - round * q.unit);
            return true;
        }
        ++q.hop;
    }
    return false;
}

struct TileGeom {
    long long n_rays;
    int rays_per_view;
    int image_w, image_h;
    int sb, bw, bh;
    int bpr, bpv;
    int n_samples, chunk, n_chunks;
    long long n_blocks;
    long long unit;
    int order;
};

__device__ __forceinline__ long long tile_ray(const TileGeom& g, long long b, int j, bool& rvalid) {
    long long ray;
    float okf = 1.f;
    const int jr = j / g.sb;
    if (g.image_w > 0) {
        const long long view = b / g.bpv;
        const int rem = (int)(b - view * g.bpv);
        const int by = rem / g.bpr, bx = rem - by * g.bpr;
        const int x = bx * g.bw + (jr % g.bw), y = by * g.bh + (jr / g.bw);
        okf = tt_opaque(x < g.image_w ? 1.f : 0.f) * (y < g.image_h ? 1.f : 0.f);
        ray = view * g.rays_per_view + (long long)min(y, g.image_h - 1) * g.image_w + min(x, g.image_w - 1);
    } else {
        ray = b * (32 / g.sb) + jr;
    }
    okf = tt_opaque(okf) * (ray < g.n_rays ? 1.f : 0.f);
    rvalid = okf != 0.f;
    return ray < g.n_rays - 1 ? ray : g.n_rays - 1;
}

__device__ __forceinline__ float sigmoidf_(float x) { return 1.f / (1.f + expf(-x)); }
```

### triplaneturbo_amd/csrc/tt_forward.hip

```cpp
#ifndef TT_MV16_FENCE
#define TT_MV16_FENCE 1
#endif
#include "tt_device.h"
#include "tt_mfma16.h"
#include "tt_alpha.h"
#include "tt_launch.h"

__device__ __forceinline__ void rot_dst(int k3, int y, int x, int H, int W, int& h, int& w) {
    if (k3 == 0) {
        h = x;
        w = y;
    } else if (k3 == 1) {
        h = H - 1 - y;
        w = W - 1 - x;
    } else {
        h = x;
        w = H - 1 - y;
    }
}

template <bool UNPACK>
__global__ __launch_bounds__(256) void k_planes_pack(const float* __restrict__ src, float* __restrict__ dst, int H,
                                                     int W, int n_copies, size_t copy_stride) {
    extern __shared__ float tile[];
    const int y = blockIdx.x, plane = blockIdx.y;
    const int k3 = plane % 3;
    const size_t HW = (size_t)H * W;
    const float* nchw_c = (UNPACK ? dst : src) + (size_t)plane * TT_C * HW;
    float* nchw = const_cast<float*>(nchw_c);
    const float* nhwc_c = (UNPACK ? src : dst) + (size_t)plane * HW * TT_C;
    float* nhwc = const_cast<float*>(nhwc_c);
    const int ws = W + 1;
    if (!UNPACK) {
        for (int e = threadIdx.x; e < TT_C * W; e += blockDim.x) {
            int c = e / W, x = e - c * W;
            tile[c * ws + x] = nchw[(size_t)c * HW + (size_t)y * W + x];
        }
        __syncthreads();
        for (int e = threadIdx.x; e < TT_C * W; e += blockDim.x) {
            int x = e >> 5, c = e & 31, h, w;
            rot_dst(k3, y, x, H, W, h, w);
            nhwc[((size_t)h * W + w) * TT_C + c] = tile[c * ws + x];
        }
    } else {
        for (int e = threadIdx.x; e < TT_C * W; e += blockDim.x) {
            int x = e >> 5, c = e & 31, h, w;
            rot_dst(k3, y, x, H, W, h, w);
            const size_t o = ((size_t)h * W + w) * TT_C + c;
            float acc = nhwc[o];
            for (int k = 1; k < n_copies; ++k) acc += nhwc[o + (size_t)k * copy_stride];
            tile[c * ws + x] = acc;
        }
        __syncthreads();
        for (int e = threadIdx.x; e < TT_C * W; e += blockDim.x) {
            int c = e / W, x = e - c * W;
            nchw[(size_t)c * HW + (size_t)y * W + x] = tile[c * ws + x];
        }
    }
}

__host__ __device__ inline int pack4_row_stride(int W) { return W + (36 - W % 32) % 32; }
template <bool UNPACK>
__global__ __launch_bounds__(256) void k_planes_pack4(const float* __restrict__ src, float* __restrict__ dst, int H,
                                                      int W, int n_copies, size_t copy_stride) {
    extern __shared__ __attribute__((aligned(16))) float tile[];
    const int y = blockIdx.x, plane = blockIdx.y;
    const int k3 = plane % 3;
    const size_t HW = (size_t)H * W;
    const float* nchw_c = (UNPACK ? dst : src) + (size_t)plane * TT_C * HW + (size_t)y * W;
    float* nchw = const_cast<float*>(nchw_c);
    const float* nhwc_c = (UNPACK ? src : dst) + (size_t)plane * HW * TT_C;
    float* nhwc = const_cast<float*>(nhwc_c);
    const int RS = pack4_row_stride(W), W4 = W >> 2;
    const int c_lane = threadIdx.x & 31, x4_0 = threadIdx.x >> 5;
    if (!UNPACK) {
        for (int e4 = threadIdx.x; e4 < TT_C * W4; e4 += 256) {
            const int c = e4 / W4, x4 = e4 - c * W4;
            *reinterpret_cast<f32x4*>(tile + c * RS + 4 * x4) =
                *reinterpret_cast<const f32x4*>(nchw_c + (size_t)c * HW + 4 * x4);
        }
        __syncthreads();
        for (int x4 = x4_0; x4 < W4; x4 += 8) {
            const f32x4 v = *reinterpret_cast<const f32x4*>(tile + c_lane * RS + 4 * x4);
#pragma unroll
            for (int j = 0; j < 4; ++j) {
                int h, w;
                rot_dst(k3, y, 4 * x4 + j, H, W, h, w);
                nhwc[((size_t)h * W + w) * TT_C + c_lane] = v[j];
            }
        }
    } else {
        for (int x4 = x4_0; x4 < W4; x4 += 8) {
            f32x4 v;
#pragma unroll
            for (int j = 0; j < 4; ++j) {
                int h, w;
                rot_dst(k3, y, 4 * x4 + j, H, W, h, w);
                const size_t o = ((size_t)h * W + w) * TT_C + c_lane;
                float acc = nhwc_c[o];
                for (int k = 1; k < n_copies; ++k) acc += nhwc_c[o + (size_t)k * copy_stride];
                v[j] = acc;
            }
            *reinterpret_cast<f32x4*>(tile + c_lane * RS + 4 * x4) = v;
        }
        __syncthreads();
        for (int e4 = threadIdx.x; e4 < TT_C * W4; e4 += 256) {
            const int c = e4 / W4, x4 = e4 - c * W4;
            *reinterpret_cast<f32x4*>(nchw + (size_t)c * HW + 4 * x4) =
                *reinterpret_cast<const f32x4*>(tile + c * RS + 4 * x4);
        }
    }
}

template <int PREC>
using FwdMap = DecodeMap<PREC, 96>;

struct DecodeCfg {
    const float* planes;
    unsigned tex0;
    float* T;
    int H, W;
    float radius;
    float ju, jv;
    int dbg;
    TileStats st = {nullptr};
};


template <int PREC>
__device__ __forceinline__ void decode_tex_fwd(const float* L, const DecodeCfg& dc, float X, float Y, float Z,
                                               bool valid, int i, int hi, float (&c)[3]) {
    typedef FwdMap<PREC> F;
    c[0] = c[1] = c[2] = 0.f;
    float e[48];
    unsigned pmask;
    bool any = gather_tex_cp(dc.planes, dc.tex0, dc.H, dc.W, X, Y, Z, valid, 32 * hi + i, dc.T, e, pmask);
    if (TT_DBG(dc.dbg, TT_DBG_NO_MLP)) {
        float t = 0.f;
#pragma unroll
        for (int r = 0; r < 48; ++r) t += e[r];
        c[0] = c[1] = c[2] = t;
    } else if (__any(any)) {
        float k1[32], k2[32], u1, u2;
        if (single_plane(pmask)) {
            tile_stat(dc.st, TT_STAT_SINGLE);
            float e1[16];
            live_block16(e, e1);
            mvx_plane<PREC, true>(L, typename F::V1{}, e1, single_plane_index(pmask), k1, i, hi, &u1);
        } else {
            mvx<PREC, true>(L, typename F::V1{}, e, k1, i, hi, 1.f, &u1);
        }
#pragma unroll
        for (int r = 0; r < 32; ++r) k1[r] = fmaxf(k1[r], 0.f);
        mvx<PREC, true>(L, typename F::V2{}, k1, k2, i, hi, u1, &u2);
#pragma unroll
        for (int r = 0; r < 32; ++r) k2[r] = fmaxf(k2[r], 0.f);
#pragma unroll
        for (int o = 0; o < 3; ++o) c[o] = dot_lds<64>(lds_at(L, typename F::V3{}) + 64 * o, k2, hi) * u2;
    }
}

__device__ __forceinline__ unsigned sign_mask32(const float (&h)[32]) {
    unsigned m = 0u;
#pragma unroll
    for (int g = 3; g >= 0; --g)
        asm("v_cmp_lt_f32 vcc, 0, %8\n\tv_addc_co_u32 %0, vcc, %0, %0, vcc\n\t"
            "v_cmp_lt_f32 vcc, 0, %7\n\tv_addc_co_u32 %0, vcc, %0, %0, vcc\n\t"
            "v_cmp_lt_f32 vcc, 0, %6\n\tv_addc_co_u32 %0, vcc, %0, %0, vcc\n\t"
            "v_cmp_lt_f32 vcc, 0, %5\n\tv_addc_co_u32 %0, vcc, %0, %0, vcc\n\t"
            "v_cmp_lt_f32 vcc, 0, %4\n\tv_addc_co_u32 %0, vcc, %0, %0, vcc\n\t"
            "v_cmp_lt_f32 vcc, 0, %3\n\tv_addc_co_u32 %0, vcc, %0, %0, vcc\n\t"
            "v_cmp_lt_f32 vcc, 0, %2\n\tv_addc_co_u32 %0, vcc, %0, %0, vcc\n\t"
            "v_cmp_lt_f32 vcc, 0, %1\n\tv_addc_co_u32 %0, vcc, %0, %0, vcc"
            : "+v"(m)
            : "v"(h[8 * g]), "v"(h[8 * g + 1]), "v"(h[8 * g + 2]), "v"(h[8 * g + 3]), "v"(h[8 * g + 4]), "v"(h[8 * g + 5]),
              "v"(h[8 * g + 6]), "v"(h[8 * g + 7])
            : "vcc");
    return m;
}

__device__ __forceinline__ void store_mask_word(unsigned* mask, long long sidx, int hi, bool valid, unsigned m) {
    asm volatile("" : "+v"(sidx));
    if (valid) mask[2 * sidx + hi] = m;
}

template <bool NEED_N, int PREC, bool MASK = false>
__device__ __forceinline__ void decode_geo_fwd(const float* L, const DecodeCfg& dc, float X, float Y, float Z,
                                               bool valid, int i, int hi, float& s0, float (&gq)[3],
                                               unsigned* mask = nullptr, long long sidx = 0) {
    typedef FwdMap<PREC> F;
    s0 = 0.f;
    gq[0] = gq[1] = gq[2] = 0.f;
    float f[16], jx[16], jy[16], jz[16];
    unsigned pmask;
    bool any = gather_geo_c<NEED_N>(dc.planes, dc.tex0, dc.H, dc.W, X, Y, Z, valid, dc.ju, dc.jv, 32 * hi + i, dc.T, f, jx,
                                 jy, jz, pmask, tile_stat_ptr(dc.st, TT_STAT_INBOUNDS));
    if (TT_DBG(dc.dbg, TT_DBG_NO_MLP)) {
        float t = 0.f, tx = 0.f, ty = 0.f, tz = 0.f;
#pragma unroll
        for (int r = 0; r < 16; ++r) {
            t += f[r];
            tx += jx[r];
            ty += jy[r];
            tz += jz[r];
        }
        s0 = t;
        gq[0] = tx;
        gq[1] = ty;
        gq[2] = tz;
    } else if (__any(any)) {
        tile_stat(dc.st, TT_STAT_EXECUTED);
        float h1[32], h2[32], u1, u2;
        mvx<PREC, true>(L, typename F::W1{}, f, h1, i, hi, 1.f, &u1);
#pragma unroll
        for (int r = 0; r < 32; ++r) h1[r] = fmaxf(h1[r], 0.f);
        mvx<PREC, true>(L, typename F::W2{}, h1, h2, i, hi, u1, &u2);
#pragma unroll
        for (int r = 0; r < 32; ++r) h2[r] = fmaxf(h2[r], 0.f);
        if constexpr (MASK) {
            store_mask_word(mask, sidx, hi, valid, sign_mask32(h2));
        }
        s0 = dot_lds<64>(lds_at(L, typename F::W3{}), h2, hi) * u2;
        if (NEED_N) {
            float a2[32], a1[32], q[16];
#pragma unroll
            for (int g = 0; g < 8; ++g) {
                f32x4 w3 = *reinterpret_cast<const f32x4*>(lds_at(L, typename F::W3{}) + 8 * g + 4 * hi);
#pragma unroll
                for (int e2 = 0; e2 < 4; ++e2) a2[4 * g + e2] = h2[4 * g + e2] > 0.f ? w3[e2] : 0.f;
            }
            float ua1;
            mvtx<PREC, true>(L, typename F::W2{}, a2, a1, i, hi, 1.f, &ua1);
#pragma unroll
            for (int r = 0; r < 32; ++r) a1[r] = h1[r] > 0.f ? a1[r] : 0.f;
            mvtx<PREC>(L, typename F::W1{}, a1, q, i, hi, ua1);
            float sx = 0.f, sy = 0.f, sz = 0.f;
#pragma unroll
            for (int r = 0; r < 16; ++r) {
                sx = fmaf(q[r], jx[r], sx);
                sy = fmaf(q[r], jy[r], sy);
                sz = fmaf(q[r], jz[r], sz);
            }
            gq[0] = sx + __shfl_xor(sx, 32);
            gq[1] = sy + __shfl_xor(sy, 32);
            gq[2] = sz + __shfl_xor(sz, 32);
        }
    } else if constexpr (MASK) {
        store_mask_word(mask, sidx, hi, valid, 0u);
    }
}

template <bool NEED_N, bool NEED_TEX, int PREC, bool MASK = false>
__device__ __forceinline__ void decode_fwd(const float* L, const DecodeCfg& dc, float px, float py, float pz,
                                           bool valid, int i, int hi, float& s0, float (&gq)[3], float (&c)[3],
                                           unsigned* mask = nullptr, long long sidx = 0) {
    const float X = scale_coord(px, dc.radius), Y = scale_coord(py, dc.radius), Z = scale_coord(pz, dc.radius);
    c[0] = c[1] = c[2] = 0.f;
    if (NEED_TEX) decode_tex_fwd<PREC>(L, dc, X, Y, Z, valid, i, hi, c);
    decode_geo_fwd<NEED_N, PREC, MASK>(L, dc, X, Y, Z, valid, i, hi, s0, gq, mask, sidx);
}

struct QueryParams {
    const float* packed;
    MlpPtrs w;
    const float* points;
    int n_batch;
    long long n_points;
    int views_per_prompt;
    int H, W;
    float radius, bias_radius;
    float* out_sdf;
    float* out_grad;
    float* out_feat;
};

#define TT_DR_GEO_SAMPLES 64
#define TT_DR_GEO_MIN_ITEMS 0
#define DECODE_THREADS 512

template <bool NEED_N, bool NEED_TEX, int PREC>
__global__ __launch_bounds__(DECODE_THREADS) void k_query_points(QueryParams p) {
    __shared__ __attribute__((aligned(16))) float L[FwdMap<PREC>::FLOATS + (DECODE_THREADS / 64) * GC_SCRATCH_FLOATS];
    float* T = L + FwdMap<PREC>::FLOATS + (threadIdx.x >> 6) * GC_SCRATCH_FLOATS;
    stage_weights(L, FwdMap<PREC>{}, p.w, NEED_TEX);
    __syncthreads();
    const int lane = threadIdx.x & 63, i = lane & 31, hi = lane >> 5;
    const long long tiles_per_batch = (p.n_points + TT_TILE - 1) / TT_TILE;
    const long long n_tiles = tiles_per_batch * p.n_batch;
    const long long wave0 = (long long)blockIdx.x * (blockDim.x >> 6) + (threadIdx.x >> 6);
    const long long n_waves = (long long)gridDim.x * (blockDim.x >> 6);
    const size_t plane_stride = (size_t)6 * p.H * p.W * TT_C;
#pragma nounroll
    for (long long tile = wave0; tile < n_tiles; tile += n_waves) {
        const int b = (int)(tile / tiles_per_batch);
        const long long n = (tile - (long long)b * tiles_per_batch) * TT_TILE + i;
        const bool valid = n < p.n_points;
        const long long idx = (long long)b * p.n_points + (valid ? n : 0);
        DecodeCfg dc;
        dc.planes = p.packed;
        dc.tex0 = (unsigned)((size_t)(b / p.views_per_prompt) * (plane_stride / TT_C));
        dc.T = T;
        dc.H = p.H;
        dc.W = p.W;
        dc.radius = p.radius;
        dc.ju = 0.5f * p.W / p.radius;
        dc.jv = 0.5f * p.H / p.radius;
        dc.dbg = 0;
        const float px = p.points[idx * 3 + 0], py = p.points[idx * 3 + 1], pz = p.points[idx * 3 + 2];
        float s0, gq[3], c[3];
        decode_fwd<NEED_N, NEED_TEX, PREC>(L, dc, px, py, pz, valid, i, hi, s0, gq, c);
        float nrm;
        const float sdf = s0 + sphere_bias(px, py, pz, p.bias_radius, nrm);
        if (valid && hi == 0) {
            if (p.out_sdf) p.out_sdf[idx] = sdf;
            if (NEED_N && p.out_grad) {
                p.out_grad[idx * 3 + 0] = gq[0] + px / nrm;
                p.out_grad[idx * 3 + 1] = gq[1] + py / nrm;
                p.out_grad[idx * 3 + 2] = gq[2] + pz / nrm;
            }
            if (NEED_TEX && p.out_feat) {
                p.out_feat[idx * 3 + 0] = c[0];
                p.out_feat[idx * 3 + 1] = c[1];
                p.out_feat[idx * 3 + 2] = c[2];
            }
        }
    }
}

struct QueryFieldParams {
    const float* packed;
    MlpPtrs w;
    const float* points;
    int n_batch;
    long long n_points;
    int views_per_prompt;
    int H, W;
    float radius, bias_radius;
    float* out_sdf;
    float* out_def;
};

template <int PREC>
struct QueryFieldWaves {
    static constexpr int value = PREC == PREC_S3 ? 8 : 4;
};
template <int PREC>
__global__ __launch_bounds__(64 * QueryFieldWaves<PREC>::value, PREC == PREC_S3 ? 1 : 2) void k_query_field(QueryFieldParams p) {
    typedef DecodeMap<PREC, 32> F;
    __shared__ __attribute__((aligned(16))) float L[DecodeMap<PREC, 32>::FLOATS + QueryFieldWaves<PREC>::value * GC_SCRATCH_FLOATS];
    float* T = L + DecodeMap<PREC, 32>::FLOATS + (threadIdx.x >> 6) * GC_SCRATCH_FLOATS;
    stage_weights(L, F{}, p.w, true);
    __syncthreads();
    const int lane = threadIdx.x & 63, i = lane & 31, hi = lane >> 5;
    const long long tiles_per_batch = (p.n_points + TT_TILE - 1) / TT_TILE;
    const long long n_tiles = tiles_per_batch * p.n_batch;
    const long long wave0 = (long long)blockIdx.x * (blockDim.x >> 6) + (threadIdx.x >> 6);
    const long long n_waves = (long long)gridDim.x * (blockDim.x >> 6);
    const size_t plane_stride = (size_t)6 * p.H * p.W * TT_C;
#pragma nounroll
    for (long long tile = wave0; tile < n_tiles; tile += n_waves) {
        const int b = (int)(tile / tiles_per_batch);
        const long long n = (tile - (long long)b * tiles_per_batch) * TT_TILE + i;
        const bool valid = n < p.n_points;
        const long long idx = (long long)b * p.n_points + (valid ? n : 0);
        const unsigned tex0 = (unsigned)((size_t)(b / p.views_per_prompt) * (plane_stride / TT_C));
        const float px = p.points[idx * 3 + 0], py = p.points[idx * 3 + 1], pz = p.points[idx * 3 + 2];
        const float X = scale_coord(px, p.radius), Y = scale_coord(py, p.radius), Z = scale_coord(pz, p.radius);
        float f[16], jx[16], jy[16], jz[16];
        unsigned pmask;
        const bool any =
            __any(gather_geo_c<false>(p.packed, tex0, p.H, p.W, X, Y, Z, valid, 0.f, 0.f, lane, T, f, jx, jy, jz, pmask));
        float s0 = 0.f, d[3] = {0.f, 0.f, 0.f};
        if (any) {
            float h1[32], h2[32];
            mvx<PREC>(L, typename F::W1{}, f, h1, i, hi);
#pragma unroll
            for (int r = 0; r < 32; ++r) h1[r] = fmaxf(h1[r], 0.f);
            mvx<PREC>(L, typename F::W2{}, h1, h2, i, hi);
#pragma unroll
            for (int r = 0; r < 32; ++r) h2[r] = fmaxf(h2[r], 0.f);
            s0 = dot_lds<64>(lds_at(L, typename F::W3{}), h2, hi);
            mvx<PREC>(L, typename F::V1{}, f, h1, i, hi);
#pragma unroll
            for (int r = 0; r < 32; ++r) h1[r] = fmaxf(h1[r], 0.f);
            mvx<PREC>(L, typename F::V2{}, h1, h2, i, hi);
#pragma unroll
            for (int r = 0; r < 32; ++r) h2[r] = fmaxf(h2[r], 0.f);
#pragma unroll
            for (int o = 0; o < 3; ++o) d[o] = dot_lds<64>(lds_at(L, typename F::V3{}) + 64 * o, h2, hi);
        }
        float nrm;
        const float sdf = s0 + sphere_bias(px, py, pz, p.bias_radius, nrm);
        if (valid && hi == 0) {
            p.out_sdf[idx] = sdf;
            p.out_def[idx * 3 + 0] = d[0];
            p.out_def[idx * 3 + 1] = d[1];
            p.out_def[idx * 3 + 2] = d[2];
        }
    }
}

struct DecodeRaysParams {
    const float* packed;
    MlpPtrs w;
    const float* rays_o;
    const float* rays_d;
    const float* t_starts;
    const float* t_ends;
    tt_render_cfg cfg;
    TileGeom geom;
    long long n_items;
    int* queue;
    float* sdf;
    float* sdf_grad;
    float* features;
    unsigned* h2_mask;
};

template <bool NEED_N, bool NEED_TEX, int PREC, bool MASK = false>
__global__ __launch_bounds__(DECODE_THREADS) void k_decode_rays(DecodeRaysParams p) {
    __shared__ __attribute__((aligned(16))) float L[FwdMap<PREC>::FLOATS + (DECODE_THREADS / 64) * GC_SCRATCH_FLOATS];
    float* T = L + FwdMap<PREC>::FLOATS + (threadIdx.x >> 6) * GC_SCRATCH_FLOATS;
    stage_weights(L, FwdMap<PREC>{}, p.w, NEED_TEX);
    __syncthreads();
    const tt_render_cfg& cfg = p.cfg;
    const TileGeom& tg = p.geom;
    const int lane = threadIdx.x & 63, i = lane & 31, hi = lane >> 5;
    const int S = cfg.n_samples;
    ItemQueue iq = item_queue(p.queue, tg.n_blocks, tg.n_chunks, tg.unit);
    const size_t plane_stride = (size_t)6 * cfg.plane_h * cfg.plane_w * TT_C;
    const TileStats st = tile_stats(cfg.stats);

#pragma nounroll
    for (;;) {
        long long b;
        int ck;
        if (!item_pop(iq, tg.order, tg.n_chunks, b, ck)) break;
        if (b >= tg.n_blocks) continue;
        bool ray_ok;
        const long long ray = tile_ray(tg, b, i, ray_ok);
        const float ray_okf = tt_opaque(ray_ok ? 1.f : 0.f);
        const int ks = i % tg.sb;
        const int view = (int)(ray / cfg.rays_per_view);
        DecodeCfg dc;
        dc.st = st;
        dc.planes = p.packed;
        dc.tex0 = (unsigned)((size_t)(view / cfg.views_per_prompt) * (plane_stride / TT_C));
        dc.T = T;
        dc.H = cfg.plane_h;
        dc.W = cfg.plane_w;
        dc.radius = cfg.radius;
        dc.ju = 0.5f * cfg.plane_w / cfg.radius;
        dc.jv = 0.5f * cfg.plane_h / cfg.radius;
        dc.dbg = cfg.flags;
        const float ox = p.rays_o[ray * 3 + 0], oy = p.rays_o[ray * 3 + 1], oz = p.rays_o[ray * 3 + 2];
        const float dx = p.rays_d[ray * 3 + 0], dy = p.rays_d[ray * 3 + 1], dz = p.rays_d[ray * 3 + 2];
        const int s_end = (ck + 1) * tg.chunk < S ? (ck + 1) * tg.chunk : S;
        auto load_t = [&](int sb0_, float& ts_, float& te_) {
            const int si_ = sb0_ + ks;
            const long long sidx_ = ray * S + (si_ < S ? si_ : S - 1);
            ts_ = p.t_starts[sidx_];
            te_ = p.t_ends[sidx_];
        };
        float ts_n, te_n;
        load_t(ck * tg.chunk, ts_n, te_n);
#pragma nounroll
        for (int sb0 = ck * tg.chunk; sb0 < s_end; sb0 += tg.sb) {
            const int si = sb0 + ks;
            const bool rvalid = ray_okf * (si < s_end ? 1.f : 0.f) != 0.f;
            tile_stat(st, TT_STAT_VISITED);
            const long long sidx = ray * S + (si < S ? si : S - 1);
            const float ts = ts_n, te = te_n;
            load_t(sb0 + tg.sb, ts_n, te_n);
            float tm, px, py, pz;
            sample_position(ox, oy, oz, dx, dy, dz, ts, te, tm, px, py, pz);
            float s0, gq[3], c[3];
            decode_fwd<NEED_N, NEED_TEX, PREC, MASK>(L, dc, px, py, pz, rvalid, i, hi, s0, gq, c, p.h2_mask, sidx);
            float nrm;
            const float sdf = s0 + sphere_bias(px, py, pz, cfg.sdf_bias_radius, nrm);
            if (rvalid && hi == 0 && !TT_DBG(cfg.flags, TT_DBG_NO_STORE)) {
                p.sdf[sidx] = sdf;
                if (NEED_N) {
                    p.sdf_grad[sidx * 3 + 0] = gq[0] + px / nrm;
                    p.sdf_grad[sidx * 3 + 1] = gq[1] + py / nrm;
                    p.sdf_grad[sidx * 3 + 2] = gq[2] + pz / nrm;
                }
                if (NEED_TEX) {
                    p.features[sidx * 3 + 0] = c[0];
                    p.features[sidx * 3 + 1] = c[1];
                    p.features[sidx * 3 + 2] = c[2];
                }
            }
        }
    }
    tile_stats_flush(st);
}

struct RenderEvalParams {
    const float* packed;
    MlpPtrs w;
    const float* rays_o;
    const float* rays_d;
    const float* t_starts;
    const float* t_ends;
    tt_render_cfg cfg;
    TileGeom geom;
    int* queue;
    float eps_T, eps_w;
    float* opacity;
    float* depth;
    float* rgb_fg;
    float* z_var;
    float* nacc;
    unsigned long long* stats;
};

template <int PREC>
__global__ __launch_bounds__(DECODE_THREADS) void k_render_eval(RenderEvalParams p) {
    __shared__ __attribute__((aligned(16))) float L[FwdMap<PREC>::FLOATS + (DECODE_THREADS / 64) * GC_SCRATCH_FLOATS];
    float* T = L + FwdMap<PREC>::FLOATS + (threadIdx.x >> 6) * GC_SCRATCH_FLOATS;
    stage_weights(L, FwdMap<PREC>{}, p.w, true);
    __syncthreads();
    const tt_render_cfg& cfg = p.cfg;
    const TileGeom& tg = p.geom;
    const int lane = threadIdx.x & 63, i = lane & 31, hi = lane >> 5;
    const int S = cfg.n_samples;
    const float kstd = load_inv_std(cfg.inv_std_dev, cfg.inv_std);
    ItemQueue iq = item_queue(p.queue, tg.n_blocks, 1, tg.unit);
    const size_t plane_stride = (size_t)6 * cfg.plane_h * cfg.plane_w * TT_C;
    unsigned long long n_geo = 0, n_tex = 0;
#pragma nounroll
    for (;;) {
        long long b;
        int ck;
        if (!item_pop(iq, 1, 1, b, ck)) break;
        if (b >= tg.n_blocks) continue;
        bool ray_ok;
        const long long ray = tile_ray(tg, b, i, ray_ok);
        const float ray_okf = tt_opaque(ray_ok ? 1.f : 0.f);
        const int view = (int)(ray / cfg.rays_per_view);
        DecodeCfg dc;
        dc.planes = p.packed;
        dc.tex0 = (unsigned)((size_t)(view / cfg.views_per_prompt) * (plane_stride / TT_C));
        dc.T = T;
        dc.H = cfg.plane_h;
        dc.W = cfg.plane_w;
        dc.radius = cfg.radius;
        dc.ju = 0.5f * cfg.plane_w / cfg.radius;
        dc.jv = 0.5f * cfg.plane_h / cfg.radius;
        dc.dbg = 0;
        float T = 1.f, acc0 = 0.f, acc1 = 0.f, acc2 = 0.f, acc3 = 0.f, acc4 = 0.f;
        const float hif = (float)hi, lof = 1.f - hif;
#pragma nounroll
        for (int si = 0; si < S; ++si) {
            float tm, px, py, pz, cosv, ux, uy, uz, sdf, dt;
            {
                long long rr = ray;
                asm volatile("" : "+v"(rr));
                const float* ro = p.rays_o + rr * 3;
                const float* rd = p.rays_d + rr * 3;
                const float ts = p.t_starts[rr * S + si], te = p.t_ends[rr * S + si];
                const float ox = ro[0], oy = ro[1], oz = ro[2];
                const float dx = rd[0], dy = rd[1], dz = rd[2];
                sample_position(ox, oy, oz, dx, dy, dz, ts, te, tm, px, py, pz);
            }
            const float X = scale_coord(px, dc.radius), Y = scale_coord(py, dc.radius), Z = scale_coord(pz, dc.radius);
            const float livef = ray_okf * (__builtin_fabsf(T) < p.eps_T ? 0.f : 1.f);
            const bool live = livef != 0.f;
            {
                float s0, gq[3];
                decode_geo_fwd<true, PREC>(L, dc, X, Y, Z, live, i, hi, s0, gq);
                ++n_geo;
                float nrm;
                long long rr = ray;
                asm volatile("" : "+v"(rr));
                const float* ro = p.rays_o + rr * 3;
                const float* rd = p.rays_d + rr * 3;
                const float ts = p.t_starts[rr * S + si], te = p.t_ends[rr * S + si];
                dt = te - ts;
                const float ox = ro[0], oy = ro[1], oz = ro[2];
                const float dx = rd[0], dy = rd[1], dz = rd[2];
                sample_position(ox, oy, oz, dx, dy, dz, ts, te, tm, px, py, pz);
                sdf = s0 + sphere_bias(px, py, pz, cfg.sdf_bias_radius, nrm);
                const float gx = gq[0] + px / nrm, gy = gq[1] + py / nrm, gz = gq[2] + pz / nrm;
                const float gn = fmaxf(sqrtf(gx * gx + gy * gy + gz * gz), 1e-12f);
                const float ign = rcp_(gn);
                ux = gx * ign, uy = gy * ign, uz = gz * ign;
                cosv = dx * ux + dy * uy + dz * uz;
            }
            float alpha = (cfg.flags & TT_R_VOLSDF) ? volsdf_alpha_terms(sdf, dt, kstd).alpha
                                                    : neus_alpha_terms(sdf, cosv, dt, kstd, cfg.cos_anneal_ratio).alpha;
            if (!live) alpha = 0.f;
            const float wgt = alpha * T;
            T *= 1.f - alpha;
            acc0 = fmaf(wgt, lof, acc0);
            acc1 = fmaf(wgt * lof, tm, acc1);
            acc2 = fmaf(wgt * lof * tm, tm, acc2);
            acc3 = fmaf(wgt, hi ? uz : ux, acc3);
            acc4 = fmaf(wgt * lof, uy, acc4);
            const bool want_tex = __builtin_fabsf(wgt) > p.eps_w;
            if (__any(want_tex)) {
                float c[3];
                if constexpr (PREC == PREC_F32) {
                    long long rr = ray;
                    asm volatile("" : "+v"(rr));
                    const float* ro = p.rays_o + rr * 3;
                    const float* rd = p.rays_d + rr * 3;
                    float tm2, qx, qy, qz;
                    sample_position(ro[0], ro[1], ro[2], rd[0], rd[1], rd[2], p.t_starts[rr * S + si], p.t_ends[rr * S + si], tm2,
                                    qx, qy, qz);
                    decode_tex_fwd<PREC>(L, dc, scale_coord(qx, dc.radius), scale_coord(qy, dc.radius),
                                         scale_coord(qz, dc.radius), want_tex, i, hi, c);
                } else {
                    decode_tex_fwd<PREC>(L, dc, X, Y, Z, want_tex, i, hi, c);
                }
                ++n_tex;
                if (want_tex) {
                    const float wh = wgt * hif;
                    acc0 = fmaf(wh, sigmoid_(c[0]) * 1.002f - 0.001f, acc0);
                    acc1 = fmaf(wh, sigmoid_(c[1]) * 1.002f - 0.001f, acc1);
                    acc2 = fmaf(wh, sigmoid_(c[2]) * 1.002f - 0.001f, acc2);
                }
            }
            if (p.eps_T > 0.f && !__any(ray_okf * (__builtin_fabsf(T) < p.eps_T ? 0.f : 1.f) != 0.f)) break;
        }
        if (ray_ok) {
            if (hi == 0) {
                const float op = acc0, dep = acc1, wt2 = acc2;
                p.opacity[ray] = op;
                p.depth[ray] = dep;
                p.z_var[ray] = wt2 - 2.f * dep * dep + dep * dep * op;
                p.nacc[ray * 3 + 0] = acc3;
                p.nacc[ray * 3 + 1] = acc4;
            } else {
                p.rgb_fg[ray * 3 + 0] = acc0;
                p.rgb_fg[ray * 3 + 1] = acc1;
                p.rgb_fg[ray * 3 + 2] = acc2;
                p.nacc[ray * 3 + 2] = acc3;
            }
        }
    }
    if (p.stats && lane == 0) {
        atomicAdd(p.stats + 0, n_geo);
        atomicAdd(p.stats + 1, n_tex);
    }
}

extern "C" int tt_planes_pack(const float* space_cache, float* packed, int32_t n_prompts, int32_t plane_h,
                              int32_t plane_w, void* stream) {
    if (!space_cache || !packed || n_prompts <= 0 || plane_h <= 0 || plane_w <= 0) return TT_ERR_BAD_ARG;
    if (plane_h != plane_w) return TT_ERR_UNSUPPORTED;
    dim3 grid(plane_h, n_prompts * 6);
    if (plane_w % 4 == 0 && ((uintptr_t)space_cache & 15) == 0) {
        size_t lds = (size_t)TT_C * pack4_row_stride(plane_w) * sizeof(float);
        hipLaunchKernelGGL(k_planes_pack4<false>, grid, dim3(256), lds, (hipStream_t)stream, space_cache, packed,
                           plane_h, plane_w, 1, (size_t)0);
    } else {
        size_t lds = (size_t)TT_C * (plane_w + 1) * sizeof(float);
        hipLaunchKernelGGL(k_planes_pack<false>, grid, dim3(256), lds, (hipStream_t)stream, space_cache, packed,
                           plane_h, plane_w, 1, (size_t)0);
    }
    return tt_check_launch();
}

extern "C" int tt_planes_unpack_grad(const float* grad_packed, float* grad_space_cache, int32_t n_prompts,
                                     int32_t plane_h, int32_t plane_w, int32_t n_copies, void* stream) {
    if (!grad_packed || !grad_space_cache || n_prompts <= 0 || plane_h <= 0 || plane_w <= 0 || n_copies <= 0)
        return TT_ERR_BAD_ARG;
    if (plane_h != plane_w) return TT_ERR_UNSUPPORTED;
    dim3 grid(plane_h, n_prompts * 6);
    const size_t copy_stride = (size_t)n_prompts * 6 * plane_h * plane_w * TT_C;
    if (plane_w % 4 == 0 && ((uintptr_t)grad_space_cache & 15) == 0) {
        size_t lds = (size_t)TT_C * pack4_row_stride(plane_w) * sizeof(float);
        hipLaunchKernelGGL(k_planes_pack4<true>, grid, dim3(256), lds, (hipStream_t)stream, grad_packed,
                           grad_space_cache, plane_h, plane_w, n_copies, copy_stride);
    } else {
        size_t lds = (size_t)TT_C * (plane_w + 1) * sizeof(float);
        hipLaunchKernelGGL(k_planes_pack<true>, grid, dim3(256), lds, (hipStream_t)stream, grad_packed,
                           grad_space_cache, plane_h, plane_w, n_copies, copy_stride);
    }
    return tt_check_launch();
}

extern "C" int tt_query_points(const float* packed, const tt_mlp_weights* w, const float* points, int32_t n_batch,
                               int64_t n_points, int32_t n_prompts, int32_t views_per_prompt, int32_t plane_h,
                               int32_t plane_w, float radius, float sdf_bias_radius, int32_t flags, float* out_sdf,
                               float* out_sdf_grad, float* out_features, void* stream) {
    if (!packed || !w || !points) return TT_ERR_BAD_ARG;
    const int st = tt_validate_points(n_batch, n_points, n_prompts, views_per_prompt, plane_h, plane_w, radius, flags);
    if (st != TT_OK) return st;
    const bool need_n = (flags & TT_Q_NORMAL) != 0, need_t = (flags & TT_Q_TEX) != 0;
    if (!w->w1 || !w->w2 || !w->w3 || (need_t && (!w->v1 || !w->v2 || !w->v3))) return TT_ERR_BAD_ARG;
    QueryParams p;
    tt_fill_points(p, packed, w, points, n_batch, n_points, views_per_prompt, plane_h, plane_w, radius);
    p.bias_radius = sdf_bias_radius;
    p.out_sdf = out_sdf;
    p.out_grad = out_sdf_grad;
    p.out_feat = out_features;
    const int cus = tt_num_cus();
    if (cus <= 0) return TT_ERR_DEVICE;
    const dim3 grid = tt_point_blocks(n_points, n_batch, DECODE_THREADS / 64, cus);
    tt_dispatch(tt_prec_of_q(flags), need_n, need_t, [&](auto P, auto N, auto T) {
        hipLaunchKernelGGL((k_query_points<decltype(N)::value, decltype(T)::value, decltype(P)::value>), grid,
                           dim3(DECODE_THREADS), 0, (hipStream_t)stream, p);
    });
    return tt_check_launch();
}

bool tt_planes_too_large(long long n_prompts, int plane_h, int plane_w) {
    return n_prompts * 6 * plane_h * plane_w * TT_C * 4 >= (1LL << 32);
}

int tt_validate_cfg(const tt_render_cfg* cfg) {
    if (!cfg) return TT_ERR_BAD_ARG;
    if (cfg->n_prompts <= 0 || cfg->views_per_prompt <= 0 || cfg->rays_per_view <= 0 || cfg->n_samples <= 0 ||
        cfg->n_rays <= 0)
        return TT_ERR_BAD_ARG;
    if (cfg->n_rays != (int64_t)cfg->n_prompts * cfg->views_per_prompt * cfg->rays_per_view) return TT_ERR_BAD_ARG;
    if (cfg->plane_h <= 0 || cfg->plane_h != cfg->plane_w) return TT_ERR_UNSUPPORTED;
    if (tt_planes_too_large(cfg->n_prompts, cfg->plane_h, cfg->plane_w)) return TT_ERR_UNSUPPORTED;
    if (!(cfg->radius > 0.f) || (!cfg->inv_std_dev && !(cfg->inv_std > 0.f))) return TT_ERR_BAD_ARG;
    if (cfg->flags < 0) return TT_ERR_BAD_ARG;
    {
        const int pbits = cfg->flags & (TT_R_EXACT_F32 | TT_R_SPLIT2 | TT_R_SPLIT3);
        if (pbits & (pbits - 1)) return TT_ERR_BAD_ARG;
    }
    if (cfg->flags & (TT_R_BWD_PAIR | TT_R_WGRAD_F32)) return TT_ERR_UNSUPPORTED;
    if (!(cfg->skip_eps_tex >= 0.f) || !(cfg->skip_eps_geo >= 0.f)) return TT_ERR_BAD_ARG;
    return TT_OK;
}

long long tt_make_geom(const tt_render_cfg* cfg, long long wave_slots, TileGeom* g, int default_order,
                       int steps_per_item, int min_items_per_slot) {
    g->n_rays = cfg->n_rays;
    g->rays_per_view = cfg->rays_per_view;
    g->n_samples = cfg->n_samples;
    g->image_w = 0;
    g->image_h = 0;
    g->bpr = g->bpv = 0;
    int sb = cfg->tile_sb;
#ifdef TT_TUNING
    if (const char* e = getenv("TT_SB")) sb = atoi(e);
#endif
    if (!(sb == 1 || sb == 2 || sb == 4 || sb == 8 || sb == 16 || sb == 32)) sb = 2;
    while (sb > 1 && sb > cfg->n_samples) sb /= 2;
    g->sb = sb;
    static const int BW[6] = {8, 4, 4, 2, 2, 1}, BH[6] = {4, 4, 2, 2, 1, 1};
    int l2 = 0;
    while ((1 << l2) < sb) ++l2;
    g->bw = BW[l2];
    g->bh = BH[l2];
    const int rb = 32 / sb;
    long long n_blocks;
    if (cfg->image_w > 0 && cfg->rays_per_view % cfg->image_w == 0) {
        g->image_w = cfg->image_w;
        g->image_h = cfg->rays_per_view / cfg->image_w;
        g->bpr = (g->image_w + g->bw - 1) / g->bw;
        g->bpv = g->bpr * ((g->image_h + g->bh - 1) / g->bh);
        n_blocks = (cfg->n_rays / cfg->rays_per_view) * g->bpv;
    } else {
        n_blocks = (cfg->n_rays + rb - 1) / rb;
    }
    const int n_steps = (cfg->n_samples + sb - 1) / sb;
    int n_chunks = (n_steps + steps_per_item - 1) / steps_per_item;
    const int min_chunks = (int)(((long long)min_items_per_slot * wave_slots + n_blocks - 1) / n_blocks);
    if (n_chunks < min_chunks) n_chunks = min_chunks;
    if (n_chunks < 1) n_chunks = 1;
    if (n_chunks > n_steps) n_chunks = n_steps;
    if (cfg->tile_chunk > 0) {
        n_chunks = (cfg->n_samples + cfg->tile_chunk - 1) / cfg->tile_chunk;
        if (n_chunks > n_steps) n_chunks = n_steps;
    }
#ifdef TT_TUNING
    if (const char* e = getenv("TT_CHUNK")) {
        int c = atoi(e);
        if (c > 0) n_chunks = (cfg->n_samples + c - 1) / c;
        if (n_chunks > n_steps) n_chunks = n_steps;
    }
#endif
    const int steps_per_chunk = (n_steps + n_chunks - 1) / n_chunks;
    g->chunk = steps_per_chunk * sb;
    g->n_chunks = (cfg->n_samples + g->chunk - 1) / g->chunk;
    g->n_blocks = n_blocks;
    g->unit = n_blocks / 256;
    if (g->unit > 32) g->unit = 32;
#ifdef TT_TUNING
    if (const char* e = getenv("TT_UNIT")) {
        long long u = atoll(e);
        if (u > 0) g->unit = u;
    }
#endif
    if (g->unit < 1) g->unit = 1;
    g->order = default_order;
#ifdef TT_TUNING
    if (const char* e = getenv("TT_ORDER")) g->order = atoi(e) ? 1 : 0;
#endif
    return n_blocks * g->n_chunks;
}

static int render_fwd(const float* packed, const tt_mlp_weights* w, const float* rays_o, const float* rays_d,
                      const float* t_starts, const float* t_ends, const tt_render_cfg* cfg, float* opacity, float* depth,
                      float* rgb_fg, float* z_variance, float* normal_acc, float* weights, float* trans, float* sdf,
                      float* sdf_grad, float* features, uint32_t* h2_mask, void* stream) {
    int st = tt_validate_cfg(cfg);
    if (st != TT_OK) return st;
    if (!packed || !w || !rays_o || !rays_d || !t_starts || !t_ends || !opacity || !depth || !rgb_fg || !z_variance ||
        !normal_acc || !weights || !trans || !sdf || !sdf_grad || !features)
        return TT_ERR_BAD_ARG;
    if (!w->w1 || !w->w2 || !w->w3 || !w->v1 || !w->v2 || !w->v3) return TT_ERR_BAD_ARG;
    const int cus = tt_num_cus();
    if (cus <= 0) return TT_ERR_DEVICE;
    DecodeRaysParams p;
    tt_fill_rays(p, packed, w, rays_o, rays_d, t_starts, t_ends, *cfg);
    p.cfg.flags |= debug_flags();
    p.sdf = sdf;
    p.sdf_grad = sdf_grad;
    p.features = features;
    p.h2_mask = h2_mask;
    hipStream_t s = (hipStream_t)stream;
    st = tt_plan_queue(cfg, (long long)cus * (DECODE_THREADS / 64), s, &p.geom, &p.n_items, &p.queue, 12);
    if (st != TT_OK) return st;
    const dim3 grid((unsigned)tt_persistent_blocks(p.n_items, cus, DECODE_THREADS / 64));
    tt_dispatch_prec(tt_prec_of_r(cfg->flags), [&](auto P) {
        if (h2_mask)
            hipLaunchKernelGGL((k_decode_rays<true, true, decltype(P)::value, true>), grid, dim3(DECODE_THREADS), 0, s, p);
        else
            hipLaunchKernelGGL((k_decode_rays<true, true, decltype(P)::value>), grid, dim3(DECODE_THREADS), 0, s, p);
    });
    st = tt_check_launch();
    if (st != TT_OK) return st;
    return tt_launch_march_fwd(rays_d, t_starts, t_ends, cfg, sdf, sdf_grad, features, opacity, depth, rgb_fg,
                               z_variance, normal_acc, weights, trans, s);
}

extern "C" int tt_render_fwd(const float* packed, const tt_mlp_weights* w, const float* rays_o, const float* rays_d,
                             const float* t_starts, const float* t_ends, const tt_render_cfg* cfg, float* opacity,
                             float* depth, float* rgb_fg, float* z_variance, float* normal_acc, float* weights,
                             float* trans, float* sdf, float* sdf_grad, float* features, void* stream) {
    return render_fwd(packed, w, rays_o, rays_d, t_starts, t_ends, cfg, opacity, depth, rgb_fg, z_variance, normal_acc,
                      weights, trans, sdf, sdf_grad, features, nullptr, stream);
}

extern "C" int tt_render_fwd_h2mask(const float* packed, const tt_mlp_weights* w, const float* rays_o,
                                    const float* rays_d, const float* t_starts, const float* t_ends,
                                    const tt_render_cfg* cfg, float* opacity, float* depth, float* rgb_fg,
                                    float* z_variance, float* normal_acc, float* weights, float* trans, float* sdf,
                                    float* sdf_grad, float* features, uint32_t* h2_mask, void* stream) {
    if (!h2_mask) return TT_ERR_BAD_ARG;
    return render_fwd(packed, w, rays_o, rays_d, t_starts, t_ends, cfg, opacity, depth, rgb_fg, z_variance, normal_acc,
                      weights, trans, sdf, sdf_grad, features, h2_mask, stream);
}

extern "C" int tt_decode_rays(const float* packed, const tt_mlp_weights* w, const float* rays_o, const float* rays_d,
                              const float* t_starts, const float* t_ends, const tt_render_cfg* cfg, int32_t flags,
                              float* sdf, float* sdf_grad, float* features, void* stream) {
    int st = tt_validate_cfg(cfg);
    if (st != TT_OK) return st;
    const bool need_n = (flags & TT_Q_NORMAL) != 0, need_t = (flags & TT_Q_TEX) != 0;
    if (!packed || !w || !rays_o || !rays_d || !t_starts || !t_ends || !sdf || (need_n && !sdf_grad) ||
        (need_t && !features) || !tt_qflags_ok(flags))
        return TT_ERR_BAD_ARG;
    if (!w->w1 || !w->w2 || !w->w3 || (need_t && (!w->v1 || !w->v2 || !w->v3))) return TT_ERR_BAD_ARG;
    const int cus = tt_num_cus();
    if (cus <= 0) return TT_ERR_DEVICE;
    DecodeRaysParams p;
    tt_fill_rays(p, packed, w, rays_o, rays_d, t_starts, t_ends, *cfg);
    p.sdf = sdf;
    p.sdf_grad = sdf_grad;
    p.features = features;
    p.h2_mask = nullptr;
    hipStream_t s = (hipStream_t)stream;
    const long long slots = (long long)cus * (DECODE_THREADS / 64);
    int steps_per_item = 12, min_items_per_slot = 8;
    if (!need_n && !need_t) {
        const int sb = cfg->tile_sb > 0 ? cfg->tile_sb : 2;
        const int spi = (TT_DR_GEO_SAMPLES + sb - 1) / sb;
        steps_per_item = spi > 1 ? spi : 1;
        min_items_per_slot = TT_DR_GEO_MIN_ITEMS;
    }
    st = tt_plan_queue(cfg, slots, s, &p.geom, &p.n_items, &p.queue, steps_per_item, min_items_per_slot);
    if (st != TT_OK) return st;
    const dim3 grid((unsigned)tt_persistent_blocks(p.n_items, cus, DECODE_THREADS / 64));
    const int prec = (flags & (TT_Q_EXACT_F32 | TT_Q_SPLIT2 | TT_Q_SPLIT3)) ? tt_prec_of_q(flags) : tt_prec_of_r(cfg->flags);
    tt_dispatch(prec, need_n, need_t, [&](auto P, auto N, auto T) {
        hipLaunchKernelGGL((k_decode_rays<decltype(N)::value, decltype(T)::value, decltype(P)::value>), grid,
                           dim3(DECODE_THREADS), 0, s, p);
    });
    return tt_check_launch();
}

extern "C" int tt_query_field(const float* packed, const tt_mlp_weights* w, const float* points, int32_t n_batch,
                              int64_t n_points, int32_t n_prompts, int32_t views_per_prompt, int32_t plane_h,
                              int32_t plane_w, float radius, float sdf_bias_radius, int32_t flags, float* out_sdf,
                              float* out_deformation, void* stream) {
    if (!packed || !w || !points || !out_sdf || !out_deformation) return TT_ERR_BAD_ARG;
    const int st = tt_validate_points(n_batch, n_points, n_prompts, views_per_prompt, plane_h, plane_w, radius, flags);
    if (st != TT_OK) return st;
    if (!w->w1 || !w->w2 || !w->w3 || !w->v1 || !w->v2 || !w->v3) return TT_ERR_BAD_ARG;
    QueryFieldParams p;
    tt_fill_points(p, packed, w, points, n_batch, n_points, views_per_prompt, plane_h, plane_w, radius);
    p.bias_radius = sdf_bias_radius;
    p.out_sdf = out_sdf;
    p.out_def = out_deformation;
    const int cus = tt_num_cus();
    if (cus <= 0) return TT_ERR_DEVICE;
    tt_dispatch_prec(tt_prec_of_q(flags), [&](auto P) {
        constexpr int PREC = decltype(P)::value, waves = QueryFieldWaves<PREC>::value;
        hipLaunchKernelGGL(k_query_field<PREC>, tt_point_blocks(n_points, n_batch, waves, (8LL / waves) * cus),
                           dim3(64 * waves), 0, (hipStream_t)stream, p);
    });
    return tt_check_launch();
}

extern "C" int tt_render_eval(const float* packed, const tt_mlp_weights* w, const float* rays_o, const float* rays_d,
                              const float* t_starts, const float* t_ends, const tt_render_cfg* cfg,
                              float transmittance_eps, float weight_eps, float* opacity, float* depth, float* rgb_fg,
                              float* z_variance, float* normal_acc, uint64_t* stats, void* stream) {
    int st = tt_validate_cfg(cfg);
    if (st != TT_OK) return st;
    if (!packed || !w || !rays_o || !rays_d || !t_starts || !t_ends || !opacity || !depth || !rgb_fg || !z_variance ||
        !normal_acc)
        return TT_ERR_BAD_ARG;
    if (!w->w1 || !w->w2 || !w->w3 || !w->v1 || !w->v2 || !w->v3) return TT_ERR_BAD_ARG;
    if (!(transmittance_eps >= 0.f) || !(weight_eps >= 0.f)) return TT_ERR_BAD_ARG;
    const int cus = tt_num_cus();
    if (cus <= 0) return TT_ERR_DEVICE;
    RenderEvalParams p;
    tt_fill_rays(p, packed, w, rays_o, rays_d, t_starts, t_ends, *cfg);
    p.cfg.tile_sb = 1;
    p.cfg.tile_chunk = cfg->n_samples;
    p.eps_T = transmittance_eps;
    p.eps_w = weight_eps;
    p.opacity = opacity;
    p.depth = depth;
    p.rgb_fg = rgb_fg;
    p.z_var = z_variance;
    p.nacc = normal_acc;
    p.stats = (unsigned long long*)stats;
    hipStream_t s = (hipStream_t)stream;
    long long n_items;
    st = tt_plan_queue(&p.cfg, (long long)cus * (DECODE_THREADS / 64), s, &p.geom, &n_items, &p.queue);
    if (st != TT_OK) return st;
    if (p.geom.n_chunks != 1) return TT_ERR_UNSUPPORTED;
    const dim3 grid((unsigned)tt_persistent_blocks(n_items, cus, DECODE_THREADS / 64));
    tt_dispatch_prec(tt_prec_of_r(cfg->flags), [&](auto P) {
        hipLaunchKernelGGL(k_render_eval<decltype(P)::value>, grid, dim3(DECODE_THREADS), 0, s, p);
    });
    return tt_check_launch();
}
```

### triplaneturbo_amd/ops.py

```python
from __future__ import annotations

import ctypes
import dataclasses
from dataclasses import dataclass
from functools import cached_property
from typing import List, NamedTuple, Optional, Sequence, Tuple, Union

import numpy as np
import torch

from . import _lib

Tensor = torch.Tensor


class KernelTimer:

    def __init__(self):
        self.events = []

    def summary(self, median: bool = False):
        torch.cuda.synchronize()
        acc = {}
        for label, a, b in self.events:
            acc.setdefault(label, []).append(a.elapsed_time(b))
        mid = (lambda v: sorted(v)[len(v) // 2]) if median else (lambda v: sum(v) / len(v))
        return {k: (mid(v), len(v)) for k, v in acc.items()}


_TIMER: Optional[KernelTimer] = None


def set_kernel_timer(t: Optional[KernelTimer]) -> None:
    global _TIMER
    _TIMER = t


class _timed:
    def __init__(self, label):
        self.label = label

    def __enter__(self):
        if _TIMER is not None:
            self.a = torch.cuda.Event(enable_timing=True)
            self.b = torch.cuda.Event(enable_timing=True)
            self.a.record()
        return self

    def __exit__(self, *exc):
        if _TIMER is not None:
            self.b.record()
            _TIMER.events.append((self.label, self.a, self.b))
        return False


def _ptr(t: Optional[Tensor]) -> ctypes.c_void_p:
    if t is None:
        return ctypes.c_void_p(0)
    return ctypes.c_void_p(t.data_ptr())


def _stream() -> ctypes.c_void_p:
    return ctypes.c_void_p(torch.cuda.current_stream().cuda_stream)


def _contig(t: Optional[Tensor]) -> Optional[Tensor]:
    return None if t is None else t.contiguous()


def _launch(name: str, *args, label: Optional[str] = None) -> None:
    fn = getattr(_lib.load(), name)
    ptrs = [a.data_ptr() if isinstance(a, Tensor) else a for a in args]
    if label is None:
        status = fn(*ptrs, _stream())
    else:
        with _timed(label):
            status = fn(*ptrs, _stream())
    _lib.check(status, name)


def _workspace(name: str, *dims: int, device) -> Tensor:
    nbytes = int(getattr(_lib.load(), name)(*dims))
    _lib.check(min(nbytes, 0), name)
    return torch.empty(nbytes, device=device, dtype=torch.uint8)


def _chk_gpu(t: Tensor, name: str) -> None:
    if not isinstance(t, torch.Tensor):
        raise TypeError(f"{name} must be a tensor")
    if not t.is_cuda:
        raise RuntimeError(f"{name} must live on the GPU (triplaneturbo_amd has no CPU path)")
    if t.device.index != torch.cuda.current_device():
        raise RuntimeError(f"{name} lives on {t.device} but the current device is cuda:{torch.cuda.current_device()}; "
                           f"call torch.cuda.set_device (one process per GPU)")


def _chk(t: Tensor, name: str, shape: Optional[Sequence[Optional[int]]] = None, dtype=torch.float32) -> Tensor:
    _chk_gpu(t, name)
    if t.dtype != dtype:
        raise TypeError(f"{name} must be {dtype}, got {t.dtype}")
    if shape is not None and (t.dim() != len(shape) or any(e not in (None, n) for e, n in zip(shape, t.shape))):
        raise ValueError(f"{name} has shape {tuple(t.shape)}, expected {str(tuple(shape)).replace('None', '*')}")
    return t.contiguous()


def _chk_index(t: Tensor, name: str, width: int, rows: Optional[int] = None) -> Tensor:
    _chk_gpu(t, name)
    if t.dtype not in (torch.int32, torch.int64) or t.dim() != 2 or t.shape[1] != width:
        raise TypeError(f"{name} must be (N,{width}) int32 / int64, got {tuple(t.shape)} {t.dtype}")
    if rows is not None and t.shape[0] != rows:
        raise ValueError(f"{name} has {t.shape[0]} rows, expected {rows}")
    return t


def _minmax(*tables: Tensor) -> Tensor:
    return torch.stack([x for t in tables for x in (t.aminmax() if t.numel() else t.new_tensor([0, -1]).unbind())])


def _chk_range(name: str, lo: int, hi: int, n: int) -> None:
    if lo < 0 or hi >= n:
        raise ValueError(f"{name} holds an index outside [0, {n})")


def _chk_size(what: str, **counts: int) -> None:
    if max(counts.values()) > _lib.TT_MESH_MAX_ITEMS:
        sizes = ", ".join(f"{k}={v}" for k, v in counts.items())
        raise ValueError(f"{what}: {sizes} (limit TT_MESH_MAX_ITEMS = {_lib.TT_MESH_MAX_ITEMS})")


def _csr(row: Tensor, col: Optional[Tensor], n_rows: int, n_cols: int) -> Tuple[Tensor, Tensor]:
    order = torch.sort(row if col is None else torch.add(col, row, alpha=max(n_cols, 1)), stable=True)[1]
    out = (order if col is None else col[order]).int().contiguous()
    ptr = torch.zeros(n_rows + 1, dtype=torch.int64, device=row.device)
    ptr[1:] = torch.cumsum(torch.bincount(row, minlength=n_rows), 0)
    return ptr.int().contiguous(), out


def _weights_struct(sdf_w: Sequence[Tensor], net2_w: Optional[Sequence[Tensor]], net2: str = "feat v",
                    net2_in: int = 96):
    sw = [_chk(sdf_w[0], "sdf w1", (64, 32)), _chk(sdf_w[1], "sdf w2", (64, 64)), _chk(sdf_w[2], "sdf w3", (1, 64))]
    fw: List[Optional[Tensor]] = [None, None, None]
    if net2_w is not None:
        fw = [_chk(net2_w[0], net2 + "1", (64, net2_in)), _chk(net2_w[1], net2 + "2", (64, 64)),
              _chk(net2_w[2], net2 + "3", (3, 64))]
    st = _lib.MlpWeights(*[_ptr(t) for t in sw + fw])
    return st, sw + fw


@dataclass
class RenderConfig:
    radius: float = 1.0
    sdf_bias_radius: float = 0.5
    inv_std: float = 100.0
    cos_anneal_ratio: float = 1.0
    rgb_grad_shrink: float = 1.0
    tile_sb: int = 0
    grad_copies: int = 1
    tile_chunk: int = 0
    precision: Optional[str] = None
    exact_f32: bool = False
    use_volsdf: bool = False

    @property
    def prec(self) -> str:
        return _lib.resolve_precision(self.precision, self.exact_f32)
    skip_eps_tex: float = 0.0
    skip_eps_geo: float = 0.0
    inv_std_t: Optional[Tensor] = None
    stats: Optional[Tensor] = None
    fwd_mask: bool = True


def planes_pack(space_cache: Tensor) -> Tensor:
    space_cache = _chk(space_cache, "space_cache", (None, 6, 32, None, None))
    P, _, _, H, W = space_cache.shape
    out = torch.empty((P, 6, H, W, 32), device=space_cache.device, dtype=torch.float32)
    _launch("tt_planes_pack", space_cache, out, P, H, W)
    return out


def planes_unpack_grad(grad_packed: Tensor) -> Tensor:
    grad_packed = _chk(grad_packed, "grad_packed")
    copies = grad_packed.shape[0] if grad_packed.ndim == 6 else 1
    P, _, H, W, _ = grad_packed.shape[-5:]
    out = torch.empty((P, 6, 32, H, W), device=grad_packed.device, dtype=torch.float32)
    _launch("tt_planes_unpack_grad", grad_packed, out, P, H, W, copies)
    return out


class _PackPlanesFn(torch.autograd.Function):

    @staticmethod
    def forward(ctx, space_cache):
        return planes_pack(space_cache)

    @staticmethod
    @torch.autograd.function.once_differentiable
    def backward(ctx, grad_packed):
        return planes_unpack_grad(grad_packed.contiguous())


def pack_planes(space_cache: Tensor) -> Tensor:
    return _PackPlanesFn.apply(space_cache)


def query_points(packed: Tensor, sdf_w: Sequence[Tensor], feat_w: Optional[Sequence[Tensor]], points: Tensor,
                 views_per_prompt: int = 1, radius: float = 1.0, sdf_bias_radius: float = 0.5,
                 need_normal: bool = True, need_features: bool = True, exact_f32: bool = False,
                 precision: Optional[str] = None):
    packed = _chk(packed, "packed")
    points = _chk(points, "points")
    B, N, _ = points.shape
    P, _, H, W, _ = packed.shape
    wst, keep = _weights_struct(sdf_w, feat_w if need_features else None)
    dev = points.device
    sdf = torch.empty((B * N, 1), device=dev, dtype=torch.float32)
    grad = torch.empty((B * N, 3), device=dev, dtype=torch.float32) if need_normal else None
    feat = torch.empty((B * N, 3), device=dev, dtype=torch.float32) if need_features else None
    flags = (_lib.TT_Q_NORMAL if need_normal else 0) | (_lib.TT_Q_TEX if need_features else 0) | _lib.q_flag(
        _lib.resolve_precision(precision, exact_f32))
    _launch("tt_query_points", packed, wst, points, B, N, P, views_per_prompt, H, W, radius, sdf_bias_radius, flags,
            sdf, grad, feat, label="tt_query_points")
    return sdf, grad, feat


def query_field(packed: Tensor, sdf_w: Sequence[Tensor], deform_w: Sequence[Tensor], points: Tensor,
                views_per_prompt: int = 1, radius: float = 1.0, sdf_bias_radius: float = 0.5, exact_f32: bool = False,
                precision: Optional[str] = None):
    packed = _chk(packed, "packed")
    points = _chk(points, "points")
    B, N, _ = points.shape
    P, _, H, W, _ = packed.shape
    wst, keep = _weights_struct(sdf_w, deform_w, "def d", 32)
    sdf = torch.empty((B * N, 1), device=points.device, dtype=torch.float32)
    deform = torch.empty((B * N, 3), device=points.device, dtype=torch.float32)
    _launch("tt_query_field", packed, wst, points, B, N, P, views_per_prompt, H, W, radius, sdf_bias_radius,
            _lib.q_flag(_lib.resolve_precision(precision, exact_f32)), sdf, deform, label="tt_query_field")
    return sdf, deform


class _QueryPointsFn(torch.autograd.Function):

    @staticmethod
    def forward(ctx, space_cache, w1, w2, w3, v1, v2, v3, points, views_per_prompt, radius, sdf_bias_radius,
                need_normal, prec):
        ctx.set_materialize_grads(False)
        packed = planes_pack(space_cache)
        sdf, grad, feat = query_points(packed, (w1, w2, w3), (v1, v2, v3), points, views_per_prompt, radius,
                                       sdf_bias_radius, need_normal=need_normal, need_features=True,
                                       precision=prec)
        ctx.save_for_backward(packed, w1, w2, w3, v1, v2, v3, points)
        ctx.meta = (views_per_prompt, radius, sdf_bias_radius, _lib.q_flag(prec))
        if grad is None:
            grad = sdf.new_zeros((sdf.shape[0], 3))
            ctx.mark_non_differentiable(grad)
        return sdf, grad, feat

    @staticmethod
    @torch.autograd.function.once_differentiable
    def backward(ctx, g_sdf, g_grad, g_feat):
        packed, w1, w2, w3, v1, v2, v3, points = ctx.saved_tensors
        vpp, radius, bias_r, qf = ctx.meta
        B, N, _ = points.shape
        P, _, H, W, _ = packed.shape
        wst, keep = _weights_struct((w1, w2, w3), (v1, v2, v3))
        g_sdf, g_grad, g_feat = _contig(g_sdf), _contig(g_grad), _contig(g_feat)
        gw = [None] * 6
        g_cache = None
        if any(ctx.needs_input_grad[:7]):
            grad_packed = torch.zeros_like(packed)
            gw = [torch.zeros_like(t) for t in (w1, w2, w3, v1, v2, v3)]
            gst = _grads_struct(gw)
            if g_sdf is not None or g_grad is not None:
                ws = torch.empty((B * N, 4), device=packed.device, dtype=torch.float32)
                _launch("tt_points_bwd_geo", packed, wst, points, B, N, P, vpp, H, W, radius, bias_r, qf, g_sdf, g_grad,
                        ws, grad_packed, gst)
            if g_feat is not None:
                _launch("tt_points_bwd_tex", packed, wst, points, B, N, P, vpp, H, W, radius, 3, qf, g_feat,
                        grad_packed, gst)
            g_cache = planes_unpack_grad(grad_packed) if ctx.needs_input_grad[0] else None
        g_points = None
        if ctx.needs_input_grad[7]:
            g_points = torch.empty_like(points)
            _launch("tt_points_bwd_x", packed, wst, points, B, N, P, vpp, H, W, radius, qf, g_sdf, g_grad, g_feat,
                    g_points)
        return (g_cache, *gw, g_points, None, None, None, None, None)


def query_points_grad(space_cache: Tensor, sdf_w: Sequence[Tensor], feat_w: Sequence[Tensor], points: Tensor,
                      views_per_prompt: int = 1, radius: float = 1.0, sdf_bias_radius: float = 0.5,
                      need_normal: bool = True, exact_f32: bool = False, precision: Optional[str] = None):
    return _QueryPointsFn.apply(space_cache, sdf_w[0], sdf_w[1], sdf_w[2], feat_w[0], feat_w[1], feat_w[2],
                                _chk(points, "points"), int(views_per_prompt), float(radius), float(sdf_bias_radius),
                                bool(need_normal), _lib.resolve_precision(precision, bool(exact_f32)))


class _QueryFieldFn(torch.autograd.Function):

    @staticmethod
    def forward(ctx, space_cache, w1, w2, w3, d1, d2, d3, points, views_per_prompt, radius, sdf_bias_radius,
                prec):
        ctx.set_materialize_grads(False)
        packed = planes_pack(space_cache)
        sdf, deform = query_field(packed, (w1, w2, w3), (d1, d2, d3), points, views_per_prompt, radius,
                                  sdf_bias_radius, precision=prec)
        ctx.save_for_backward(packed, w1, w2, w3, d1, d2, d3, points)
        ctx.meta = (views_per_prompt, radius, sdf_bias_radius, _lib.q_flag(prec))
        return sdf, deform

    @staticmethod
    @torch.autograd.function.once_differentiable
    def backward(ctx, g_sdf, g_def):
        packed, w1, w2, w3, d1, d2, d3, points = ctx.saved_tensors
        vpp, radius, bias_r, qf = ctx.meta
        B, N, _ = points.shape
        P, _, H, W, _ = packed.shape
        d1x3 = d1.repeat(1, 3).contiguous()
        keep = [w1.contiguous(), w2.contiguous(), w3.contiguous(), d1x3, d2.contiguous(), d3.contiguous()]
        wst = _lib.MlpWeights(*[_ptr(t) for t in keep])
        grad_packed = torch.zeros_like(packed)
        gw = [torch.zeros_like(t) for t in (w1, w2, w3, d1x3, d2, d3)]
        gst = _grads_struct(gw)
        if g_sdf is not None:
            ws = torch.empty((B * N, 4), device=packed.device, dtype=torch.float32)
            _launch("tt_points_bwd_geo", packed, wst, points, B, N, P, vpp, H, W, radius, bias_r, qf,
                    g_sdf.contiguous(), None, ws, grad_packed, gst)
        if g_def is not None:
            _launch("tt_points_bwd_tex", packed, wst, points, B, N, P, vpp, H, W, radius, 0, qf, g_def.contiguous(),
                    grad_packed, gst)
        gw[3] = gw[3].view(64, 3, 32).sum(dim=1)
        g_cache = planes_unpack_grad(grad_packed) if ctx.needs_input_grad[0] else None
        return (g_cache, *gw, None, None, None, None, None)


def query_field_grad(space_cache: Tensor, sdf_w: Sequence[Tensor], deform_w: Sequence[Tensor], points: Tensor,
                     views_per_prompt: int = 1, radius: float = 1.0, sdf_bias_radius: float = 0.5,
                     exact_f32: bool = False, precision: Optional[str] = None):
    return _QueryFieldFn.apply(space_cache, sdf_w[0], sdf_w[1], sdf_w[2], deform_w[0], deform_w[1], deform_w[2],
                               _chk(points, "points"), int(views_per_prompt), float(radius), float(sdf_bias_radius),
                               _lib.resolve_precision(precision, bool(exact_f32)))


def _inv_std_args(rc: RenderConfig):
    inv_std = min(max(float(rc.inv_std), 1.0e-6), 1.0e6)
    if rc.inv_std_t is None:
        return inv_std, None
    t = _chk(rc.inv_std_t, "inv_std_t")
    if t.numel() != 1:
        raise ValueError("inv_std_t must hold one float")
    if t.data_ptr() != rc.inv_std_t.data_ptr():
        raise ValueError("inv_std_t must be a contiguous float32 CUDA tensor (the kernels read it in place)")
    return inv_std, t.data_ptr()


def _make_cfg(packed: Tensor, n_rays: int, rays_per_view: int, n_samples: int, rc: RenderConfig,
              per_sample: bool, image_w: int = 0, stats_row: int = 0) -> "_lib.RenderCfg":
    P, _, H, W, _ = packed.shape
    n_views = n_rays // rays_per_view
    if n_views * rays_per_view != n_rays or n_views % P != 0:
        raise ValueError(f"n_rays={n_rays} is not views*rays_per_view with views a multiple of P={P}")
    inv_std, inv_std_dev = _inv_std_args(rc)
    stats = None
    if rc.stats is not None:
        if rc.stats.dtype != torch.int64 or not rc.stats.is_cuda or tuple(rc.stats.shape) != (3, 4):
            raise ValueError("stats must be a CUDA int64 tensor of shape (3, 4)")
        stats = rc.stats.data_ptr() + 32 * stats_row
    return _lib.RenderCfg(P, n_views // P, H, W, rays_per_view, n_samples, n_rays, rc.radius, rc.sdf_bias_radius,
                          inv_std, rc.cos_anneal_ratio, rc.rgb_grad_shrink,
                          (_lib.TT_R_PER_SAMPLE if per_sample else 0) | _lib.r_flag(rc.prec) |
                          (_lib.TT_R_VOLSDF if rc.use_volsdf else 0),
                          image_w if (image_w > 0 and rays_per_view % image_w == 0) else 0, int(rc.tile_sb),
                          max(1, int(rc.grad_copies)), max(0, int(rc.tile_chunk)), max(0.0, float(rc.skip_eps_tex)),
                          max(0.0, float(rc.skip_eps_geo)), inv_std_dev, stats)


def _ray_args(packed: Tensor, rays_o: Tensor, rays_d: Tensor, t_starts: Tensor, t_ends: Tensor):
    packed = _chk(packed, "packed")
    rays_o, rays_d = _chk(rays_o, "rays_o"), _chk(rays_d, "rays_d")
    t_starts, t_ends = _chk(t_starts, "t_starts"), _chk(t_ends, "t_ends")
    n_rays, S = t_starts.shape
    if rays_o.shape != (n_rays, 3) or rays_d.shape != (n_rays, 3) or t_ends.shape != (n_rays, S):
        raise ValueError("ray / interval shapes disagree")
    return packed, rays_o, rays_d, t_starts, t_ends


def _ray_outputs(n_rays: int, device, S: Optional[int] = None) -> dict:
    f32 = dict(device=device, dtype=torch.float32)
    out = {"opacity": torch.empty((n_rays, 1), **f32), "depth": torch.empty((n_rays, 1), **f32),
           "rgb_fg": torch.empty((n_rays, 3), **f32), "z_variance": torch.empty((n_rays, 1), **f32),
           "normal_acc": torch.empty((n_rays, 3), **f32)}
    if S is not None:
        out.update(weights=torch.empty((n_rays * S, 1), **f32), trans=torch.empty((n_rays * S, 1), **f32))
    return out


def render_forward_raw(packed: Tensor, sdf_w: Sequence[Tensor], feat_w: Sequence[Tensor], rays_o: Tensor,
                       rays_d: Tensor, t_starts: Tensor, t_ends: Tensor, rays_per_view: int, rc: RenderConfig,
                       per_sample: bool = True, image_w: int = 0, h2_mask: Union[bool, Tensor] = False):
    packed, rays_o, rays_d, t_starts, t_ends = _ray_args(packed, rays_o, rays_d, t_starts, t_ends)
    n_rays, S = t_starts.shape
    cfg = _make_cfg(packed, n_rays, rays_per_view, S, rc, per_sample, image_w)
    wst, keep = _weights_struct(sdf_w, feat_w)
    f32 = dict(device=packed.device, dtype=torch.float32)
    out = _ray_outputs(n_rays, packed.device, S)
    out.update(sdf=torch.empty((n_rays * S, 1), **f32), sdf_grad=torch.empty((n_rays * S, 3), **f32),
               features=torch.empty((n_rays * S, 3), **f32))
    if h2_mask is not False:
        if h2_mask is True:
            h2_mask = torch.empty((n_rays * S, 2), device=packed.device, dtype=torch.int32)
        out["h2_mask"] = _chk(h2_mask, "h2_mask", (n_rays * S, 2), torch.int32)
        if out["h2_mask"].data_ptr() != h2_mask.data_ptr():
            raise ValueError("h2_mask must be contiguous (the kernel writes it in place)")
        _launch("tt_render_fwd_h2mask", packed, wst, rays_o, rays_d, t_starts, t_ends, cfg, *out.values(),
                label="tt_render_fwd")
    else:
        _launch("tt_render_fwd", packed, wst, rays_o, rays_d, t_starts, t_ends, cfg, *out.values(),
                label="tt_render_fwd")
    return out


@torch.no_grad()
def render_eval_raw(packed: Tensor, sdf_w: Sequence[Tensor], feat_w: Sequence[Tensor], rays_o: Tensor, rays_d: Tensor,
                    t_starts: Tensor, t_ends: Tensor, rays_per_view: int, rc: RenderConfig, image_w: int = 0,
                    transmittance_eps: float = 0.0, weight_eps: float = 0.0, stats: Optional[Tensor] = None):
    packed, rays_o, rays_d, t_starts, t_ends = _ray_args(packed, rays_o, rays_d, t_starts, t_ends)
    n_rays, S = t_starts.shape
    cfg = _make_cfg(packed, n_rays, rays_per_view, S, rc, False, image_w)
    wst, keep = _weights_struct(sdf_w, feat_w)
    out = _ray_outputs(n_rays, packed.device)
    if stats is not None and (stats.dtype != torch.int64 or stats.numel() < 2 or not stats.is_cuda):
        raise ValueError("stats must be a CUDA int64 tensor with 2 elements")
    _launch("tt_render_eval", packed, wst, rays_o, rays_d, t_starts, t_ends, cfg, float(transmittance_eps),
            float(weight_eps), *out.values(), stats, label="tt_render_eval")
    return out


def _placement(name: str) -> int:
    if name not in _lib.PLACEMENTS:
        raise ValueError(f"placement must be one of {sorted(_lib.PLACEMENTS)}, got {name!r}")
    return _lib.PLACEMENTS[name]


@torch.no_grad()
def sample_uniform(n_rays: int, n_samples: int, near: float, far: float, device, jitter: Optional[Tensor] = None,
                   placement: str = "tt"):
    device = torch.device(device)
    place = _placement(placement)
    if device.type != "cuda":
        raise RuntimeError("triplaneturbo_amd samplers run on the GPU only (no CPU fallback)")
    f32 = dict(device=device, dtype=torch.float32)
    ts, te = torch.empty((n_rays, n_samples), **f32), torch.empty((n_rays, n_samples), **f32)
    if jitter is not None:
        jitter = _chk(jitter, "jitter")
        if jitter.shape != (n_rays, n_samples + 1):
            raise ValueError("jitter must be (n_rays, n_samples + 1)")
    with torch.cuda.device(device):
        _launch("tt_sample_uniform", n_rays, n_samples, float(near), float(far), jitter, place, ts, te)
    return ts, te


@torch.no_grad()
def sample_importance(t_starts: Tensor, t_ends: Tensor, sdf: Tensor, n_fine: int, inv_std: float,
                      render_step_size: float, u_jitter: Optional[Tensor] = None, placement: str = "tt",
                      inv_std_t: Optional[Tensor] = None, use_volsdf: bool = False):
    place = _placement(placement) | (_lib.TT_PLACE_VOLSDF if use_volsdf else 0)
    if inv_std_t is not None:
        inv_std_t = _chk(inv_std_t.detach(), "inv_std_t")
    t_starts, t_ends, sdf = _chk(t_starts, "t_starts"), _chk(t_ends, "t_ends"), _chk(sdf, "sdf")
    n_rays, K = t_starts.shape
    if t_ends.shape != (n_rays, K) or sdf.numel() != n_rays * K:
        raise ValueError("proposal intervals / sdf shapes disagree")
    if u_jitter is not None:
        u_jitter = _chk(u_jitter, "u_jitter")
        if u_jitter.shape != (n_rays, n_fine + 1):
            raise ValueError("u_jitter must be (n_rays, n_fine + 1)")
    f32 = dict(device=t_starts.device, dtype=torch.float32)
    M = K + n_fine + 1
    ots, ote = torch.empty((n_rays, M), **f32), torch.empty((n_rays, M), **f32)
    _launch("tt_sample_importance", t_starts, t_ends, sdf, n_rays, K, int(n_fine), float(inv_std), inv_std_t,
            float(render_step_size), u_jitter, place, ots, ote, label="tt_sample_importance")
    return ots, ote


def _march_cfg(rc: RenderConfig, n_rays: int, S: int) -> "_lib.RenderCfg":
    inv_std, inv_std_dev = _inv_std_args(rc)
    return _lib.RenderCfg(n_prompts=1, views_per_prompt=1, plane_h=1, plane_w=1, rays_per_view=n_rays, n_samples=S,
                          n_rays=n_rays, radius=rc.radius, sdf_bias_radius=rc.sdf_bias_radius, inv_std=inv_std,
                          cos_anneal_ratio=rc.cos_anneal_ratio, rgb_grad_shrink=rc.rgb_grad_shrink,
                          flags=_lib.TT_R_VOLSDF if rc.use_volsdf else 0, image_w=0,
                          tile_sb=0, grad_copies=1, tile_chunk=0, inv_std_dev=inv_std_dev)


@torch.no_grad()
def march_forward_raw(rays_d: Tensor, t_starts: Tensor, t_ends: Tensor, sdf: Tensor, sdf_grad: Tensor,
                      features: Tensor, rc: RenderConfig, out: Optional[dict] = None):
    rays_d, t_starts, t_ends = _chk(rays_d, "rays_d"), _chk(t_starts, "t_starts"), _chk(t_ends, "t_ends")
    sdf, sdf_grad, features = _chk(sdf, "sdf"), _chk(sdf_grad, "sdf_grad"), _chk(features, "features")
    n_rays, S = t_starts.shape
    if sdf.numel() != n_rays * S or sdf_grad.numel() != 3 * n_rays * S or features.numel() != 3 * n_rays * S:
        raise ValueError("per-sample tensors do not match (n_rays, S)")
    cfg = _march_cfg(rc, n_rays, S)
    if out is None:
        out = _ray_outputs(n_rays, rays_d.device, S)
    _launch("tt_march_fwd", rays_d, t_starts, t_ends, cfg, sdf, sdf_grad, features, out["opacity"], out["depth"],
            out["rgb_fg"], out["z_variance"], out["normal_acc"], out["weights"], out["trans"], label="tt_march_fwd")
    return out


@torch.no_grad()
def march_backward_raw(rays_d: Tensor, t_starts: Tensor, t_ends: Tensor, fwd: dict, sdf: Tensor, sdf_grad: Tensor,
                       features: Tensor, rc: RenderConfig, g_opacity=None, g_depth=None, g_rgb_fg=None,
                       g_z_variance=None, g_normal_acc=None, g_weights=None, g_sdf=None, g_sdf_grad=None,
                       out: Optional[Tensor] = None, g_inv_std_rays: Optional[Tensor] = None):
    n_rays, S = t_starts.shape
    cfg = _march_cfg(rc, n_rays, S)
    if out is None:
        out = torch.empty((n_rays * S, 4), device=rays_d.device, dtype=torch.float32)
    gs = [_contig(t)
          for t in (g_opacity, g_depth, g_rgb_fg, g_z_variance, g_normal_acc, g_weights, g_sdf, g_sdf_grad)]
    _launch("tt_march_bwd", rays_d, t_starts, t_ends, cfg, fwd["opacity"], fwd["depth"], fwd["trans"], sdf, sdf_grad,
            features, *gs, g_inv_std_rays, out, label="tt_march_bwd")
    return out


def _zeros_like_flat(tensors: Sequence[Tensor]) -> List[Tensor]:
    sizes = [t.numel() for t in tensors]
    flat = torch.zeros(sum(sizes), device=tensors[0].device, dtype=tensors[0].dtype)
    out, ofs = [], 0
    for t, n in zip(tensors, sizes):
        out.append(flat[ofs:ofs + n].view_as(t))
        ofs += n
    return out


def _grads_struct(tensors: Sequence[Tensor]):
    return _lib.MlpWeights(*[_ptr(t) for t in tensors])


class _TriplaneRenderFn(torch.autograd.Function):

    @staticmethod
    def forward(ctx, packed, w1, w2, w3, v1, v2, v3, rays_o, rays_d, t_starts, t_ends, rays_per_view, rc,
                image_w, inv_std_t=None):
        need_grad = any(ctx.needs_input_grad[:7]) or ctx.needs_input_grad[14]
        if inv_std_t is not None:
            rc = dataclasses.replace(rc, inv_std_t=inv_std_t.detach())
        ctx.set_materialize_grads(False)
        raw = render_forward_raw(packed, (w1, w2, w3), (v1, v2, v3), rays_o, rays_d, t_starts, t_ends, rays_per_view,
                                 rc, per_sample=True, image_w=image_w, h2_mask=need_grad and rc.fwd_mask)
        ctx.rays_per_view = rays_per_view
        ctx.rc = rc
        ctx.image_w = image_w
        ctx.inv_std_shape = None if inv_std_t is None else tuple(inv_std_t.shape)
        if need_grad:
            ctx.save_for_backward(packed, w1, w2, w3, v1, v2, v3, rays_o, rays_d, t_starts, t_ends, raw["opacity"],
                                  raw["depth"], raw["trans"], raw["weights"], raw["features"], raw["sdf"],
                                  raw["sdf_grad"], *([raw["h2_mask"]] if rc.fwd_mask else []))
        ctx.mark_non_differentiable(raw["trans"])
        return (raw["opacity"], raw["depth"], raw["rgb_fg"], raw["z_variance"], raw["normal_acc"], raw["weights"],
                raw["sdf"], raw["sdf_grad"], raw["features"], raw["trans"])

    @staticmethod
    @torch.autograd.function.once_differentiable
    def backward(ctx, g_op, g_depth, g_rgb, g_zvar, g_nacc, g_weights, g_sdf, g_sdf_grad, g_features, _g_trans):
        (packed, w1, w2, w3, v1, v2, v3, rays_o, rays_d, t_starts, t_ends, opacity, depth, trans, weights,
         features, sdf, sdf_grad) = ctx.saved_tensors[:18]
        h2_mask = ctx.saved_tensors[18:]
        n_rays, S = t_starts.shape
        cfg = _make_cfg(packed, n_rays, ctx.rays_per_view, S, ctx.rc, True, ctx.image_w, stats_row=1)
        cfg_tex = _make_cfg(packed, n_rays, ctx.rays_per_view, S, ctx.rc, True, ctx.image_w, stats_row=2)
        workspace = torch.empty((n_rays * S, 4), device=packed.device, dtype=torch.float32)
        wst, keep = _weights_struct((w1, w2, w3), (v1, v2, v3))
        copies = max(1, int(ctx.rc.grad_copies))
        grad_packed = torch.zeros((copies,) + tuple(packed.shape), device=packed.device, dtype=torch.float32)
        gw = _zeros_like_flat((w1, w2, w3, v1, v2, v3))
        gst = _grads_struct(gw)

        g_op, g_depth, g_rgb, g_zvar, g_nacc, g_weights, g_sdf, g_sdf_grad, g_features = (
            _contig(t) for t in (g_op, g_depth, g_rgb, g_zvar, g_nacc, g_weights, g_sdf, g_sdf_grad, g_features))
        g_k_rays = None
        if ctx.needs_input_grad[14]:
            g_k_rays = torch.empty((n_rays,), device=packed.device, dtype=torch.float32)
        _launch("tt_render_bwd_geo_h2mask" if h2_mask else "tt_render_bwd_geo", packed, wst, rays_o, rays_d, t_starts,
                t_ends, cfg, opacity, depth, trans, sdf, sdf_grad, features, g_op, g_depth, g_rgb, g_zvar, g_nacc,
                g_weights, g_sdf, g_sdf_grad, g_k_rays, workspace, grad_packed, gst, *h2_mask, label="tt_render_bwd_geo")
        _launch("tt_render_bwd_tex", packed, wst, rays_o, rays_d, t_starts, t_ends, cfg_tex, weights, features, g_rgb,
                g_features, grad_packed, gst, label="tt_render_bwd_tex")
        g_packed = None
        if ctx.needs_input_grad[0]:
            g_packed = grad_packed[0] if copies == 1 else grad_packed.sum(dim=0)
        g_inv_std = None
        if g_k_rays is not None:
            g_inv_std = g_k_rays.double().sum().float().reshape(ctx.inv_std_shape)
        return (g_packed, *gw, None, None, None, None, None, None, None, g_inv_std)


def render_samples(space_cache: Optional[Tensor], sdf_w: Sequence[Tensor], feat_w: Sequence[Tensor], rays_o: Tensor,
                   rays_d: Tensor, t_starts: Tensor, t_ends: Tensor, rays_per_view: int, rc: RenderConfig,
                   image_w: int = 0, packed: Optional[Tensor] = None):
    names = ("opacity", "depth", "rgb_fg", "z_variance", "normal_acc", "weights", "sdf", "sdf_grad", "features",
             "trans")
    if packed is None:
        packed = pack_planes(space_cache)
    outs = _TriplaneRenderFn.apply(packed, sdf_w[0], sdf_w[1], sdf_w[2], feat_w[0], feat_w[1], feat_w[2],
                                   rays_o.contiguous(), rays_d.contiguous(), t_starts.contiguous(),
                                   t_ends.contiguous(), rays_per_view, rc, int(image_w), rc.inv_std_t)
    return dict(zip(names, outs))


@torch.no_grad()
def decode_rays(packed: Tensor, sdf_w: Sequence[Tensor], feat_w: Optional[Sequence[Tensor]], rays_o: Tensor,
                rays_d: Tensor, t_starts: Tensor, t_ends: Tensor, rays_per_view: int, rc: RenderConfig,
                need_normal: bool = False, need_features: bool = False, image_w: int = 0):
    packed, rays_o, rays_d, t_starts, t_ends = _ray_args(packed, rays_o, rays_d, t_starts, t_ends)
    n_rays, S = t_starts.shape
    cfg = _make_cfg(packed, n_rays, rays_per_view, S, rc, False, image_w)
    wst, keep = _weights_struct(sdf_w, feat_w if need_features else None)
    f32 = dict(device=packed.device, dtype=torch.float32)
    sdf = torch.empty((n_rays, S), **f32)
    grad = torch.empty((n_rays, S, 3), **f32) if need_normal else None
    feat = torch.empty((n_rays, S, 3), **f32) if need_features else None
    flags = (_lib.TT_Q_NORMAL if need_normal else 0) | (_lib.TT_Q_TEX if need_features else 0)
    _launch("tt_decode_rays", packed, wst, rays_o, rays_d, t_starts, t_ends, cfg, flags, sdf, grad, feat,
            label="tt_decode_rays")
    return sdf, grad, feat


class _PatchCompositeFn(torch.autograd.Function):

    @staticmethod
    def forward(ctx, low, patch, py, px, H, W, detach_low):
        low, patch = _chk(low, "low"), _chk(patch, "patch")
        B, h, w, C = low.shape
        PS = patch.shape[1]
        if patch.shape != (B, PS, PS, C):
            raise ValueError(f"patch {tuple(patch.shape)} does not match low {tuple(low.shape)}")
        out = torch.empty((B, H, W, C), device=low.device, dtype=torch.float32)
        _launch("tt_patch_composite_fwd", low, patch, out, B, h, w, H, W, C, PS, py, px)
        ctx.meta = (B, h, w, H, W, C, PS, py, px, detach_low)
        return out

    @staticmethod
    @torch.autograd.function.once_differentiable
    def backward(ctx, g_out):
        B, h, w, H, W, C, PS, py, px, detach_low = ctx.meta
        want_low = ctx.needs_input_grad[0] and not detach_low
        g_low = torch.empty((B, h, w, C), device=g_out.device, dtype=torch.float32) if want_low else None
        g_patch = torch.empty((B, PS, PS, C), device=g_out.device, dtype=torch.float32)
        _launch("tt_patch_composite_bwd", g_out.contiguous(), g_low, g_patch, B, h, w, H, W, C, PS, py, px)
        return g_low, (g_patch if ctx.needs_input_grad[1] else None), None, None, None, None, None


def patch_composite(low: Tensor, patch: Tensor, py: int, px: int, H: int, W: int, detach_low: bool = False) -> Tensor:
    return _PatchCompositeFn.apply(low, patch, int(py), int(px), int(H), int(W), bool(detach_low))


_COMPOSITE_MODES = {"world": 0, "camera": 1, "front": 2}


class _CompositeFn(torch.autograd.Function):

    @staticmethod
    def forward(ctx, opacity, depth, rgb_fg, normal_acc, bg, cam_dist, c2w, rays_per_view, mode, view_group):
        opacity, depth = _chk(opacity, "opacity"), _chk(depth, "depth")
        rgb_fg, normal_acc = _chk(rgb_fg, "rgb_fg"), _chk(normal_acc, "normal_acc")
        bg, cam_dist = _chk(bg, "bg_color"), _chk(cam_dist, "camera_distances")
        n = opacity.numel()
        if rays_per_view <= 0 or n % rays_per_view != 0:
            raise ValueError(f"n_rays={n} is not a multiple of rays_per_view={rays_per_view}")
        views = n // rays_per_view
        if cam_dist.numel() != views:
            raise ValueError(f"camera_distances has {cam_dist.numel()} elements, expected one per view ({views})")
        if c2w is None:
            if mode != 0:
                raise ValueError("c2w is required for normal_direction 'camera' / 'front' (renderer :478-530)")
        else:
            c2w = _chk(c2w, "c2w", (views, 4, 4))
        if view_group <= 0 or views % view_group != 0:
            raise ValueError(f"view_group={view_group} does not divide the number of views ({views})")
        bg_stride = 0 if bg.numel() == 3 else 3
        if bg_stride and bg.numel() != 3 * n:
            raise ValueError("bg_color must have 3 or 3 * n_rays elements")
        f32 = dict(device=opacity.device, dtype=torch.float32)
        comp_rgb, comp_normal = torch.empty((n, 3), **f32), torch.empty((n, 3), **f32)
        disparity = torch.empty((n, 1), **f32)
        vis = torch.empty((n, 3), **f32) if mode == 1 else None
        vis_white = torch.empty((n, 3), **f32) if mode != 0 else None
        _launch("tt_composite_fwd", opacity, depth, rgb_fg, normal_acc, bg, bg_stride, cam_dist, c2w, n, rays_per_view,
                mode, view_group, comp_rgb, disparity, comp_normal, vis, vis_white)
        ctx.save_for_backward(opacity, depth, rgb_fg, normal_acc, bg, cam_dist, *(() if c2w is None else (c2w,)))
        ctx.meta = (n, bg_stride, rays_per_view, mode, view_group)
        ctx.set_materialize_grads(False)
        dummy = comp_rgb.new_zeros(0)
        outs = (comp_rgb, disparity, comp_normal, vis if vis is not None else dummy,
                vis_white if vis_white is not None else dummy)
        return outs

    @staticmethod
    @torch.autograd.function.once_differentiable
    def backward(ctx, g_rgb, g_disp, g_cn, g_vis, g_visw):
        opacity, depth, rgb_fg, normal_acc, bg, cam_dist, *rest = ctx.saved_tensors
        c2w = rest[0] if rest else None
        n, bg_stride, rays_per_view, mode, view_group = ctx.meta
        g_rgb, g_disp, g_cn, g_vis, g_visw = (
            _contig(t) if t is not None and t.numel() else None for t in (g_rgb, g_disp, g_cn, g_vis, g_visw))
        f32 = dict(device=opacity.device, dtype=torch.float32)
        g_op, g_dep = torch.empty((n, 1), **f32), torch.empty((n, 1), **f32)
        g_fg, g_na = torch.empty((n, 3), **f32), torch.empty((n, 3), **f32)
        g_bg = torch.empty((n, 3), **f32) if ctx.needs_input_grad[4] else None
        _launch("tt_composite_bwd", opacity, depth, rgb_fg, normal_acc, bg, bg_stride, cam_dist, c2w, n, rays_per_view,
                mode, view_group, g_rgb, g_disp, g_cn, g_vis, g_visw, g_op, g_dep, g_fg, g_na, g_bg)
        if g_bg is not None:
            g_bg = g_bg.sum(dim=0).view_as(bg) if bg_stride == 0 else g_bg.view_as(bg)
        return g_op, g_dep, g_fg, g_na, g_bg, None, None, None, None, None


def composite(opacity: Tensor, depth: Tensor, rgb_fg: Tensor, normal_acc: Tensor, bg_color: Tensor,
              camera_distances: Tensor, c2w: Optional[Tensor], rays_per_view: int, normal_direction: str = "camera",
              view_group: int = 1):
    mode = _COMPOSITE_MODES[normal_direction]
    views = opacity.numel() // max(int(rays_per_view), 1)
    camera_distances = camera_distances.reshape(-1).float()
    if camera_distances.numel() == 1 and views > 1:
        camera_distances = camera_distances.expand(views)
    camera_distances = camera_distances.contiguous()
    if c2w is not None:
        c2w = c2w.float().contiguous()
    rgb, disp, cn, vis, visw = _CompositeFn.apply(opacity, depth, rgb_fg, normal_acc, bg_color, camera_distances, c2w,
                                                  int(rays_per_view), mode, int(view_group))
    return rgb, disp, cn, (vis if mode == 1 else None), (visw if mode != 0 else None)


class _EikonalFn(torch.autograd.Function):

    @staticmethod
    def forward(ctx, sdf_grad):
        g = _chk(sdf_grad, "sdf_grad", (None, 3))
        loss = torch.empty((), device=g.device, dtype=torch.float32)
        _launch("tt_eikonal_fwd", g, g.shape[0], loss)
        ctx.save_for_backward(g)
        return loss

    @staticmethod
    @torch.autograd.function.once_differentiable
    def backward(ctx, g_loss):
        g, = ctx.saved_tensors
        out = torch.empty_like(g)
        _launch("tt_eikonal_bwd", g, g_loss.contiguous().float(), g.shape[0], out)
        return out


def eikonal_loss(sdf_grad: Tensor) -> Tensor:
    return _EikonalFn.apply(sdf_grad)


class _MarchingCubesFn(torch.autograd.Function):

    @staticmethod
    def forward(ctx, level, deformation, isovalue):
        R = level.shape[0]
        ws = _workspace("tt_mc_workspace_bytes", R, device=level.device)
        totals = torch.empty(2, device=level.device, dtype=torch.int32)
        _launch("tt_mc_count", level, R, isovalue, ws, totals)
        n_vert, n_tri = (int(x) for x in totals.cpu())
        v_pos = torch.empty((n_vert, 3), device=level.device, dtype=torch.float32)
        t_pos_idx = torch.empty((n_tri, 3), device=level.device, dtype=torch.int32)
        if n_vert > 0:
            _launch("tt_mc_emit", level, deformation, R, isovalue, ws, v_pos, t_pos_idx)
        ctx.save_for_backward(level, deformation, ws)
        ctx.isovalue = isovalue
        ctx.mark_non_differentiable(t_pos_idx)
        return v_pos, t_pos_idx

    @staticmethod
    @torch.autograd.function.once_differentiable
    def backward(ctx, g_v, g_t):
        level, deformation, ws = ctx.saved_tensors
        if g_v is None or not (ctx.needs_input_grad[0] or ctx.needs_input_grad[1]):
            return None, None, None
        R = level.shape[0]
        g_level = torch.empty_like(level)
        g_def = torch.empty_like(deformation) if deformation is not None else None
        if g_v.shape[0] == 0:
            g_level.zero_()
            if g_def is not None:
                g_def.zero_()
        else:
            _launch("tt_mc_bwd", level, deformation, R, ctx.isovalue, ws, g_v.contiguous(), g_level, g_def)
        return (g_level if ctx.needs_input_grad[0] else None,
                g_def if ctx.needs_input_grad[1] else None, None)


def marching_cubes(level: Tensor, deformation: Optional[Tensor] = None, isovalue: float = 0.0) -> Tuple[Tensor, Tensor]:
    if level.dim() != 3 or not (level.shape[0] == level.shape[1] == level.shape[2]):
        raise ValueError(f"level must be (R,R,R), got {tuple(level.shape)}")
    R = level.shape[0]
    level = _chk(level, "level")
    if deformation is not None:
        deformation = _chk(deformation, "deformation", (R, R, R, 3))
    return _MarchingCubesFn.apply(level, deformation, float(isovalue))


_TET_BASE_EDGES = (0, 1, 0, 2, 0, 3, 1, 2, 1, 3, 2, 3)


class TetGrid:

    def __init__(self, vertices: Tensor, indices: Tensor):
        self.vertices = _chk(vertices, "vertices", (None, 3))
        indices = _chk_index(indices, "indices", 4)
        Nv, Nt = int(vertices.shape[0]), int(indices.shape[0])
        if Nv < 1 or Nt < 1:
            raise ValueError(f"a tet grid needs a vertex and a tet: Nv={Nv}, Nt={Nt}")
        _chk_size("tet grid too large for tt_mt_*", Nv=Nv, Nt=Nt)
        _chk_range("indices", *_minmax(indices).tolist(), Nv)
        self.n_vertices, self.n_tets = Nv, Nt
        self.tets = indices.int().contiguous()
        pairs = indices.long()[:, list(_TET_BASE_EDGES)].reshape(-1, 2)
        key = torch.add(pairs.amax(1), pairs.amin(1), alpha=Nv)
        uniq, inverse = torch.unique(key, return_inverse=True)
        self.edges = torch.stack([uniq // Nv, uniq % Nv], dim=1).int().contiguous()
        self.tet_edge = inverse.reshape(Nt, 6).int().contiguous()
        Ne = self.n_edges = int(uniq.shape[0])
        _chk_size("tet grid too large for tt_mt_*", Ne=Ne)
        ends = self.edges.long().t().reshape(-1)
        self.vert_ptr, self.vert_col = _csr(ends, torch.arange(Ne, device=ends.device).repeat(2), Nv, Ne)


class _MarchingTetsFn(torch.autograd.Function):

    @staticmethod
    def forward(ctx, pos, level, grid):
        dev = level.device
        ws = _workspace("tt_mt_workspace_bytes", grid.n_edges, grid.n_tets, device=dev)
        totals = torch.empty(3, device=dev, dtype=torch.int32)
        _launch("tt_mt_count", level, grid.edges, grid.tets, grid.n_edges, grid.n_tets, ws, totals)
        n_vert, n_one, n_two = (int(x) for x in totals.cpu())
        v_pos = torch.empty((n_vert, 3), device=dev, dtype=torch.float32)
        t_pos_idx = torch.empty((n_one + 2 * n_two, 3), device=dev, dtype=torch.int32)
        if n_vert > 0:
            _launch("tt_mt_emit", pos, level, grid.edges, grid.tet_edge, grid.n_edges, grid.n_tets, ws, v_pos,
                    t_pos_idx)
        ctx.save_for_backward(pos, level, ws)
        ctx.grid = grid
        ctx.mark_non_differentiable(t_pos_idx)
        return v_pos, t_pos_idx

    @staticmethod
    @torch.autograd.function.once_differentiable
    def backward(ctx, g_v, g_t):
        pos, level, ws = ctx.saved_tensors
        grid = ctx.grid
        if g_v is None or not (ctx.needs_input_grad[0] or ctx.needs_input_grad[1]):
            return None, None, None
        g_level, g_pos = torch.empty_like(level), torch.empty_like(pos)
        if g_v.shape[0] == 0:
            g_level.zero_()
            g_pos.zero_()
        else:
            _launch("tt_mt_bwd", pos, level, grid.edges, grid.vert_ptr, grid.vert_col, grid.n_vertices, grid.n_edges,
                    grid.n_tets, ws, g_v.contiguous(), g_level, g_pos)
        return (g_pos if ctx.needs_input_grad[0] else None, g_level if ctx.needs_input_grad[1] else None, None)


def marching_tets(pos: Tensor, level: Tensor, grid: TetGrid) -> Tuple[Tensor, Tensor]:
    if not isinstance(grid, TetGrid):
        raise TypeError("grid must be an ops.TetGrid")
    Nv = grid.n_vertices
    if not isinstance(level, torch.Tensor) or level.numel() != Nv:
        raise ValueError(f"level must hold one value per grid vertex ({Nv})")
    pos = _chk(pos, "pos", (Nv, 3))
    level = _chk(level.reshape(Nv), "level")
    if pos.device != grid.tets.device:
        raise RuntimeError(f"pos lives on {pos.device}, the tet grid on {grid.tets.device}")
    return _MarchingTetsFn.apply(pos, level, grid)


class FaceEdgeSort(NamedTuple):
    perm: Tensor
    uniq: Tensor
    inverse: Tensor
    counts: Tensor
    starts: Tensor
    base: int

    def edges(self) -> Tensor:
        return torch.stack([self.uniq // self.base, self.uniq % self.base], dim=1)

# ... 873 lines not shown
```

Baseline: 8.089 million.

## Save layer-1 ReLU sign mask in forward to skip h1 recompute in backward

The forward pass can now write a per-sample sign bitmask for the first hidden layer alongside the existing h2 mask. The geometry backward kernel uses that mask instead of recomputing the W1 matvec and ReLU, and drops the feature-weight gather and the qb term. For the three-plane case it batches all texel loads before accumulating. The aim is to remove backward MLP and gather work, at the cost of extra mask writes and reads and more template variants. The path is disabled in fp32 precision mode, which the static_assert and the prec check in the Python code rule out.

```diff
diff --git a/include/tt_abi.h b/include/tt_abi.h
--- a/include/tt_abi.h
+++ b/include/tt_abi.h
@@ -122,6 +122,11 @@
                          float* depth, float* rgb_fg, float* z_variance, float* normal_acc, float* weights, float* trans,
                          float* sdf, float* sdf_grad, float* features, uint32_t* h2_mask, void* stream);
 
+int tt_render_fwd_masks(const float* packed, const tt_mlp_weights* w, const float* rays_o, const float* rays_d,
+                        const float* t_starts, const float* t_ends, const tt_render_cfg* cfg, float* opacity,
+                        float* depth, float* rgb_fg, float* z_variance, float* normal_acc, float* weights, float* trans,
+                        float* sdf, float* sdf_grad, float* features, uint32_t* h2_mask, uint32_t* h1_mask, void* stream);
+
 int tt_render_eval(const float* packed, const tt_mlp_weights* w, const float* rays_o, const float* rays_d,
                    const float* t_starts, const float* t_ends, const tt_render_cfg* cfg, float transmittance_eps,
                    float weight_eps, float* opacity, float* depth, float* rgb_fg, float* z_variance, float* normal_acc,
@@ -153,6 +158,15 @@
                              const float* g_normal_acc, const float* g_weights, const float* g_sdf,
                              const float* g_sdf_grad, float* g_inv_std_rays, float* workspace, float* grad_packed,
                              const tt_mlp_grads* grads, const uint32_t* h2_mask, void* stream);
+
+int tt_render_bwd_geo_masks(const float* packed, const tt_mlp_weights* w, const float* rays_o, const float* rays_d,
+                            const float* t_starts, const float* t_ends, const tt_render_cfg* cfg,
+                            const float* opacity, const float* depth, const float* trans, const float* sdf,
+                            const float* sdf_grad, const float* features, const float* g_opacity,
+                            const float* g_depth, const float* g_rgb_fg, const float* g_z_variance,
+                            const float* g_normal_acc, const float* g_weights, const float* g_sdf,
+                            const float* g_sdf_grad, float* g_inv_std_rays, float* workspace, float* grad_packed,
+                            const tt_mlp_grads* grads, const uint32_t* h2_mask, const uint32_t* h1_mask, void* stream);
 
 int tt_render_bwd_tex(const float* packed, const tt_mlp_weights* w, const float* rays_o, const float* rays_d,
                       const float* t_starts, const float* t_ends, const tt_render_cfg* cfg, const float* weights,
diff --git a/triplaneturbo_amd/csrc/tt_backward.hip b/triplaneturbo_amd/csrc/tt_backward.hip
--- a/triplaneturbo_amd/csrc/tt_backward.hip
+++ b/triplaneturbo_amd/csrc/tt_backward.hip
@@ -13,6 +13,7 @@
     int* queue;
     const float* ws;
     const unsigned* h2_mask;
+    const unsigned* h1_mask;
     int n_copies;
     float* grad_packed;
     MlpGradPtrs grads;
@@ -20,6 +21,7 @@
 };
 
 #define GEO_SCRATCH_FLOATS (2 * 64 * XS)
+enum { FMASK_NONE = 0, FMASK_H2 = 1, FMASK_H1H2 = 2 };
 template <int PREC, bool FMASK>
 struct GeoMap : LdsMap<PREC, LdsImage<64, 32>, LdsImage<64, 64, !(FMASK && PREC != PREC_F32)>, LdsRows<1, 64>,
                        LdsImage<32, 64>, LdsImage<64, 64>> {
@@ -31,11 +33,13 @@
     typedef typename GeoMap::template at<4> CT;
 };
 
-template <int PREC, bool STATS = false, bool FMASK = false>
+template <int PREC, bool STATS = false, int FMASK = FMASK_NONE>
 __global__ __launch_bounds__(256, 1) void k_decode_bwd_geo(BwdGeoParams p) {
     constexpr bool EXACT = PREC == PREC_F32;
     constexpr bool WG16 = !EXACT;
-    typedef GeoMap<PREC, FMASK> G;
+    constexpr bool M1 = FMASK == FMASK_H1H2;
+    static_assert(!(M1 && EXACT), "the fp32-MFMA mode stays on the h2-only path");
+    typedef GeoMap<PREC, FMASK != FMASK_NONE> G;
     constexpr int NT = PrecNT<PREC>::value, WF = G::FLOATS;
     __shared__ __attribute__((aligned(16))) float L[WF + 4 * (GEO_SCRATCH_FLOATS + SCATTER_TAG_INTS)];
     stage_weights<PREC>(L, typename G::W1{}, p.w.w1);
@@ -111,6 +115,7 @@
             f32x4 up;
             float ts, te;
             unsigned m2;
+            unsigned m1;
         };
         auto load_step = [&](int sb0) {
             StepIn r;
@@ -120,6 +125,7 @@
             r.ts = p.rays_d ? p.t_starts[sidx] : 0.f;
             r.te = p.rays_d ? p.t_ends[sidx] : 0.f;
             r.m2 = FMASK ? p.h2_mask[2 * sidx + hi] : 0u;
+            r.m1 = M1 ? p.h1_mask[2 * sidx + hi] : 0u;
             return r;
         };
         StepIn in = load_step(ck * tg.chunk), in_next;
@@ -141,7 +147,7 @@
                         Z = scale_coord(pz, cfg.radius);
             float f[16], u[16];
             unsigned pmask;
-            const bool any = __any(gather_geo_bwd_c(p.packed, (unsigned)(pofs / TT_C), H, W, X, Y, Z, rvalid, sbar, gbx,
+            const bool any = __any(gather_geo_bwd_c<!M1>(p.packed, (unsigned)(pofs / TT_C), H, W, X, Y, Z, rvalid, sbar, gbx,
                                                     gby, gbz, ju, jv, lane, Xs, f, u, pmask,
                                                     tile_stat_ptr(st, TT_STAT_INBOUNDS)));
             TT_PHASE(1);
@@ -149,10 +155,19 @@
             const bool one = single_plane(pmask);
             tile_stat_executed(st, one);
             float h1[32], h2[32], a1[32], q[16], u1, uh2;
-            mvx<PREC, true>(L, typename G::W1{}, f, h1, i, hi, 1.f, &u1);
-#pragma unroll
-            for (int r = 0; r < 32; ++r) h1[r] = fmaxf(h1[r], 0.f);
+            if constexpr (!M1) {
+                mvx<PREC, true>(L, typename G::W1{}, f, h1, i, hi, 1.f, &u1);
+#pragma unroll
+                for (int r = 0; r < 32; ++r) h1[r] = fmaxf(h1[r], 0.f);
+            }
             const unsigned m2w = FMASK ? in.m2 & (0u - (unsigned)vf) : 0u;
+            const unsigned m1w = M1 ? in.m1 & (0u - (unsigned)vf) : 0u;
+            auto m1_keep = [&](int r, float x) {
+                if constexpr (M1)
+                    return __builtin_bit_cast(float, __builtin_bit_cast(int, x) & ((int)(m1w << (31 - r)) >> 31));
+                else
+                    return h1[r] > 0.f ? x : 0.f;
+            };
             if constexpr (!FMASK) {
                 mvx<PREC, true>(L, typename G::W2{}, h1, h2, i, hi, u1, &uh2);
 #pragma unroll
@@ -181,7 +196,7 @@
                 mvtx_copy<PREC>(L, typename G::CT{}, typename G::W2{}, a2, a1, i, hi);
             }
 #pragma unroll
-            for (int r = 0; r < 32; ++r) a1[r] = h1[r] > 0.f ? a1[r] : 0.f;
+            for (int r = 0; r < 32; ++r) a1[r] = m1_keep(r, a1[r]);
             float uq = 1.f;
             if (WG16) {
                 split16_vec<64, PAIR_SEQ, NT>(a1, sA1 * ua1, a1s);
@@ -192,8 +207,10 @@
             TT_PHASE(3);
             {
                 float qb[16];
-#pragma unroll
-                for (int r = 0; r < 16; ++r) qb[r] = fmaf(-sbar, f[r], u[r]);
+                if constexpr (!M1) {
+#pragma unroll
+                    for (int r = 0; r < 16; ++r) qb[r] = fmaf(-sbar, f[r], u[r]);
+                }
                 const bool region = WG16 || cfg.flags >= 0;
                 const bool do_wgrad = region && !TT_DBG(cfg.flags, TT_DBG_NO_WGRAD);
                 if (do_wgrad) {
@@ -208,13 +225,18 @@
                     }
                 }
                 TT_PHASE(7);
-                float t1[32];
-                mvx<PREC>(L, typename G::W1{}, qb, t1, i, hi);
-#pragma unroll
-                for (int r = 0; r < 32; ++r) t1[r] = h1[r] > 0.f ? t1[r] : 0.f;
-                float v[32];
-#pragma unroll
-                for (int r = 0; r < 32; ++r) v[r] = fmaf(sbar * u1, h1[r], t1[r]);
+                float t1[32], v[32];
+                if constexpr (M1) {
+                    mvx<PREC>(L, typename G::W1{}, u, t1, i, hi);
+#pragma unroll
+                    for (int r = 0; r < 32; ++r) v[r] = m1_keep(r, t1[r]);
+                } else {
+                    mvx<PREC>(L, typename G::W1{}, qb, t1, i, hi);
+#pragma unroll
+                    for (int r = 0; r < 32; ++r) t1[r] = h1[r] > 0.f ? t1[r] : 0.f;
+#pragma unroll
+                    for (int r = 0; r < 32; ++r) v[r] = fmaf(sbar * u1, h1[r], t1[r]);
+                }
                 TT_PHASE(4);
                 if (do_wgrad) {
                     if (WG16) {
@@ -300,12 +322,17 @@
     tt_dispatch_prec(tt_prec_of_r(p.cfg.flags), [&](auto P) {
         constexpr int PREC = decltype(P)::value;
         const dim3 grid((unsigned)blocks), block(256);
-        if (p.cfg.stats && p.h2_mask)
-            hipLaunchKernelGGL((k_decode_bwd_geo<PREC, true, true>), grid, block, 0, s, p);
+        constexpr int BOTH = PREC == PREC_F32 ? FMASK_H2 : FMASK_H1H2;
+        if (p.cfg.stats && p.h2_mask && p.h1_mask)
+            hipLaunchKernelGGL((k_decode_bwd_geo<PREC, true, BOTH>), grid, block, 0, s, p);
+        else if (p.h2_mask && p.h1_mask)
+            hipLaunchKernelGGL((k_decode_bwd_geo<PREC, false, BOTH>), grid, block, 0, s, p);
+        else if (p.cfg.stats && p.h2_mask)
+            hipLaunchKernelGGL((k_decode_bwd_geo<PREC, true, FMASK_H2>), grid, block, 0, s, p);
         else if (p.cfg.stats)
             hipLaunchKernelGGL((k_decode_bwd_geo<PREC, true>), grid, block, 0, s, p);
         else if (p.h2_mask)
-            hipLaunchKernelGGL((k_decode_bwd_geo<PREC, false, true>), grid, block, 0, s, p);
+            hipLaunchKernelGGL((k_decode_bwd_geo<PREC, false, FMASK_H2>), grid, block, 0, s, p);
         else
             hipLaunchKernelGGL((k_decode_bwd_geo<PREC>), grid, block, 0, s, p);
     });
@@ -317,7 +344,8 @@
                           const float* features, const float* g_opacity, const float* g_depth, const float* g_rgb_fg,
                           const float* g_z_variance, const float* g_normal_acc, const float* g_weights,
                           const float* g_sdf, const float* g_sdf_grad, float* g_inv_std_rays, float* workspace,
-                          float* grad_packed, const tt_mlp_grads* grads, const uint32_t* h2_mask, void* stream) {
+                          float* grad_packed, const tt_mlp_grads* grads, const uint32_t* h2_mask, const uint32_t* h1_mask,
+                          void* stream) {
     int st = tt_validate_cfg(cfg);
     if (st != TT_OK) return st;
     if (!packed || !w || !rays_o || !rays_d || !t_starts || !t_ends || !opacity || !depth || !trans || !sdf ||
@@ -337,6 +365,7 @@
     p.cfg.flags |= debug_flags();
     p.ws = workspace;
     p.h2_mask = h2_mask;
+    p.h1_mask = h1_mask;
     p.grad_packed = grad_packed;
     p.n_copies = cfg->grad_copies > 0 ? cfg->grad_copies : 1;
     p.grads = to_gptrs(grads);
@@ -356,7 +385,7 @@
                                  float* grad_packed, const tt_mlp_grads* grads, void* stream) {
     return render_bwd_geo(packed, w, rays_o, rays_d, t_starts, t_ends, cfg, opacity, depth, trans, sdf, sdf_grad, features,
                           g_opacity, g_depth, g_rgb_fg, g_z_variance, g_normal_acc, g_weights, g_sdf, g_sdf_grad,
-                          g_inv_std_rays, workspace, grad_packed, grads, nullptr, stream);
+                          g_inv_std_rays, workspace, grad_packed, grads, nullptr, nullptr, stream);
 }
 
 extern "C" int tt_render_bwd_geo_h2mask(const float* packed, const tt_mlp_weights* w, const float* rays_o,
@@ -371,7 +400,23 @@
     if (!h2_mask) return TT_ERR_BAD_ARG;
     return render_bwd_geo(packed, w, rays_o, rays_d, t_starts, t_ends, cfg, opacity, depth, trans, sdf, sdf_grad, features,
                           g_opacity, g_depth, g_rgb_fg, g_z_variance, g_normal_acc, g_weights, g_sdf, g_sdf_grad,
-                          g_inv_std_rays, workspace, grad_packed, grads, h2_mask, stream);
+                          g_inv_std_rays, workspace, grad_packed, grads, h2_mask, nullptr, stream);
+}
+
+extern "C" int tt_render_bwd_geo_masks(const float* packed, const tt_mlp_weights* w, const float* rays_o,
+                                       const float* rays_d, const float* t_starts, const float* t_ends,
+                                       const tt_render_cfg* cfg, const float* opacity, const float* depth,
+                                       const float* trans, const float* sdf, const float* sdf_grad,
+                                       const float* features, const float* g_opacity, const float* g_depth,
+                                       const float* g_rgb_fg, const float* g_z_variance, const float* g_normal_acc,
+                                       const float* g_weights, const float* g_sdf, const float* g_sdf_grad,
+                                       float* g_inv_std_rays, float* workspace, float* grad_packed,
+                                       const tt_mlp_grads* grads, const uint32_t* h2_mask, const uint32_t* h1_mask,
+                                       void* stream) {
+    if (!h2_mask || !h1_mask) return TT_ERR_BAD_ARG;
+    return render_bwd_geo(packed, w, rays_o, rays_d, t_starts, t_ends, cfg, opacity, depth, trans, sdf, sdf_grad, features,
+                          g_opacity, g_depth, g_rgb_fg, g_z_variance, g_normal_acc, g_weights, g_sdf, g_sdf_grad,
+                          g_inv_std_rays, workspace, grad_packed, grads, h2_mask, h1_mask, stream);
 }
 
 __global__ void k_interleave_ws(const float* __restrict__ g_sdf, const float* __restrict__ g_sdf_grad,
@@ -408,6 +453,7 @@
     tt_fill_rays(p, packed, w, points, nullptr, nullptr, nullptr, cfg);
     p.ws = workspace;
     p.h2_mask = nullptr;
+    p.h1_mask = nullptr;
     p.grad_packed = grad_packed;
     p.n_copies = 1;
     p.grads = to_gptrs(grads);
diff --git a/triplaneturbo_amd/csrc/tt_device.h b/triplaneturbo_amd/csrc/tt_device.h
--- a/triplaneturbo_amd/csrc/tt_device.h
+++ b/triplaneturbo_amd/csrc/tt_device.h
@@ -351,6 +351,12 @@
         if (l < 4) atomicAdd(st.p + l, (unsigned long long)st.w[l]);
     }
 }
+__device__ __forceinline__ void tile_stats_flush_late(const TileStats& st) {
+    if (st.p) {
+        const int l = (int)__builtin_amdgcn_mbcnt_hi(~0u, __builtin_amdgcn_mbcnt_lo(~0u, 0u));
+        if (l < 4) atomicAdd(st.p + l, (unsigned long long)st.w[l]);
+    }
+}
 
 __device__ __forceinline__ bool single_plane(unsigned pmask) { return pmask != 0u && (pmask & (pmask - 1u)) == 0u; }
 __device__ __forceinline__ int single_plane_index(unsigned pmask) { return __builtin_ctz(pmask | 8u); }
@@ -591,6 +597,7 @@
     for (int k = 0; k < 4; ++k) coef[k] = fmaf(cn.w[k], sbar, fmaf(cn.du[k], gu, cn.dv[k] * gv));
 }
 
+template <bool NEED_F = true>
 __device__ __forceinline__ bool gather_geo_bwd_c(const float* __restrict__ planes, unsigned tex0, int H, int W, float X,
                                                  float Y, float Z, bool valid, float sbar, float gux, float guy,
                                                  float guz, float jscale_u, float jscale_v, int lane, float* T,
@@ -620,8 +627,10 @@
             const unsigned b = tex0 + (unsigned)(p * HW);
             const ti32x4 o = {(int)(b + cn.off[0]), (int)(b + cn.off[1]), (int)(b + cn.off[2]), (int)(b + cn.off[3])};
             *reinterpret_cast<ti32x4*>(Toff + (p * 32 + i) * 4) = o;
-            const f32x4 w = {cn.w[0], cn.w[1], cn.w[2], cn.w[3]};
-            *reinterpret_cast<f32x4*>(Tw + (p * 32 + i) * 4) = w;
+            if (NEED_F) {
+                const f32x4 w = {cn.w[0], cn.w[1], cn.w[2], cn.w[3]};
+                *reinterpret_cast<f32x4*>(Tw + (p * 32 + i) * 4) = w;
+            }
         } else {
             const f32x4 w = {coef[0], coef[1], coef[2], coef[3]};
             *reinterpret_cast<f32x4*>(Tc + (p * 32 + i) * 4) = w;
@@ -634,6 +643,27 @@
         af[n] = z;
         au[n] = z;
     }
+    if (!NEED_F && pmask == 7u) {
+        f32x4 t[3][4][4];
+#pragma unroll
+        for (int p = 0; p < 3; ++p)
+#pragma unroll
+            for (int n = 0; n < 4; ++n) {
+                const ti32x4 o4 = *reinterpret_cast<const ti32x4*>(Toff + (p * 32 + 8 * n + js) * 4);
+#pragma unroll
+                for (int k = 0; k < 4; ++k) t[p][n][k] = *gc_addr(planes, o4[k], 16u * (unsigned)c);
+            }
+#pragma unroll
+        for (int p = 0; p < 3; ++p)
+#pragma unroll
+            for (int n = 0; n < 4; ++n) {
+                const f32x4 c4 = *reinterpret_cast<const f32x4*>(Tc + (p * 32 + 8 * n + js) * 4);
+#pragma unroll
+                for (int k = 0; k < 4; ++k)
+#pragma unroll
+                    for (int ee = 0; ee < 4; ++ee) au[n][ee] = fmaf(c4[k], t[p][n][k][ee], au[n][ee]);
+            }
+    } else
 #pragma unroll
     for (int p = 0; p < 3; ++p) {
         if (!anyp[p]) continue;
@@ -648,24 +678,27 @@
 #pragma unroll
         for (int n = 0; n < 4; ++n) {
             const int sidx = (p * 32 + 8 * n + js) * 4;
-            const f32x4 w4 = *reinterpret_cast<const f32x4*>(Tw + sidx);
+            f32x4 w4 = {0.f, 0.f, 0.f, 0.f};
+            if (NEED_F) w4 = *reinterpret_cast<const f32x4*>(Tw + sidx);
             const f32x4 c4 = *reinterpret_cast<const f32x4*>(Tc + sidx);
 #pragma unroll
             for (int k = 0; k < 4; ++k)
 #pragma unroll
                 for (int ee = 0; ee < 4; ++ee) {
-                    af[n][ee] = fmaf(w4[k], t[n][k][ee], af[n][ee]);
+                    if (NEED_F) af[n][ee] = fmaf(w4[k], t[n][k][ee], af[n][ee]);
                     au[n][ee] = fmaf(c4[k], t[n][k][ee], au[n][ee]);
                 }
         }
     }
-#pragma unroll
-    for (int n = 0; n < 4; ++n) *reinterpret_cast<f32x4*>(R + (8 * n + js) * 36 + 4 * c) = af[n];
-#pragma unroll
-    for (int q = 0; q < 4; ++q) {
-        const f32x4 v = *reinterpret_cast<const f32x4*>(R + i * 36 + 4 * (hi + 2 * q));
-#pragma unroll
-        for (int ee = 0; ee < 4; ++ee) f[4 * q + ee] = v[ee];
+    if (NEED_F) {
+#pragma unroll
+        for (int n = 0; n < 4; ++n) *reinterpret_cast<f32x4*>(R + (8 * n + js) * 36 + 4 * c) = af[n];
+#pragma unroll
+        for (int q = 0; q < 4; ++q) {
+            const f32x4 v = *reinterpret_cast<const f32x4*>(R + i * 36 + 4 * (hi + 2 * q));
+#pragma unroll
+            for (int ee = 0; ee < 4; ++ee) f[4 * q + ee] = v[ee];
+        }
     }
 #pragma unroll
     for (int n = 0; n < 4; ++n) *reinterpret_cast<f32x4*>(R + (8 * n + js) * 36 + 4 * c) = au[n];
diff --git a/triplaneturbo_amd/csrc/tt_forward.hip b/triplaneturbo_amd/csrc/tt_forward.hip
--- a/triplaneturbo_amd/csrc/tt_forward.hip
+++ b/triplaneturbo_amd/csrc/tt_forward.hip
@@ -184,10 +184,11 @@
     if (valid) mask[2 * sidx + hi] = m;
 }
 
-template <bool NEED_N, int PREC, bool MASK = false>
+enum { MASK_NONE = 0, MASK_H2 = 1, MASK_H1H2 = 2 };
+template <bool NEED_N, int PREC, int MASK = MASK_NONE>
 __device__ __forceinline__ void decode_geo_fwd(const float* L, const DecodeCfg& dc, float X, float Y, float Z,
                                                bool valid, int i, int hi, float& s0, float (&gq)[3],
-                                               unsigned* mask = nullptr, long long sidx = 0) {
+                                               unsigned* mask = nullptr, long long sidx = 0, unsigned* mask1 = nullptr) {
     typedef FwdMap<PREC> F;
     s0 = 0.f;
     gq[0] = gq[1] = gq[2] = 0.f;
@@ -214,10 +215,13 @@
         mvx<PREC, true>(L, typename F::W1{}, f, h1, i, hi, 1.f, &u1);
 #pragma unroll
         for (int r = 0; r < 32; ++r) h1[r] = fmaxf(h1[r], 0.f);
+        if constexpr (MASK == MASK_H1H2) {
+            store_mask_word(mask1, sidx, hi, valid, sign_mask32(h1));
+        }
         mvx<PREC, true>(L, typename F::W2{}, h1, h2, i, hi, u1, &u2);
 #pragma unroll
         for (int r = 0; r < 32; ++r) h2[r] = fmaxf(h2[r], 0.f);
-        if constexpr (MASK) {
+        if constexpr (MASK != MASK_NONE) {
             store_mask_word(mask, sidx, hi, valid, sign_mask32(h2));
         }
         s0 = dot_lds<64>(lds_at(L, typename F::W3{}), h2, hi) * u2;
@@ -245,19 +249,20 @@
             gq[1] = sy + __shfl_xor(sy, 32);
             gq[2] = sz + __shfl_xor(sz, 32);
         }
-    } else if constexpr (MASK) {
+    } else if constexpr (MASK != MASK_NONE) {
         store_mask_word(mask, sidx, hi, valid, 0u);
-    }
-}
-
-template <bool NEED_N, bool NEED_TEX, int PREC, bool MASK = false>
+        if constexpr (MASK == MASK_H1H2) store_mask_word(mask1, sidx, hi, valid, 0u);
+    }
+}
+
+template <bool NEED_N, bool NEED_TEX, int PREC, int MASK = MASK_NONE>
 __device__ __forceinline__ void decode_fwd(const float* L, const DecodeCfg& dc, float px, float py, float pz,
                                            bool valid, int i, int hi, float& s0, float (&gq)[3], float (&c)[3],
-                                           unsigned* mask = nullptr, long long sidx = 0) {
+                                           unsigned* mask = nullptr, long long sidx = 0, unsigned* mask1 = nullptr) {
     const float X = scale_coord(px, dc.radius), Y = scale_coord(py, dc.radius), Z = scale_coord(pz, dc.radius);
     c[0] = c[1] = c[2] = 0.f;
     if (NEED_TEX) decode_tex_fwd<PREC>(L, dc, X, Y, Z, valid, i, hi, c);
-    decode_geo_fwd<NEED_N, PREC, MASK>(L, dc, X, Y, Z, valid, i, hi, s0, gq, mask, sidx);
+    decode_geo_fwd<NEED_N, PREC, MASK>(L, dc, X, Y, Z, valid, i, hi, s0, gq, mask, sidx, mask1);
 }
 
 struct QueryParams {
@@ -415,9 +420,10 @@
     float* sdf_grad;
     float* features;
     unsigned* h2_mask;
+    unsigned* h1_mask;
 };
 
-template <bool NEED_N, bool NEED_TEX, int PREC, bool MASK = false>
+template <bool NEED_N, bool NEED_TEX, int PREC, int MASK = MASK_NONE>
 __global__ __launch_bounds__(DECODE_THREADS) void k_decode_rays(DecodeRaysParams p) {
     __shared__ __attribute__((aligned(16))) float L[FwdMap<PREC>::FLOATS + (DECODE_THREADS / 64) * GC_SCRATCH_FLOATS];
     float* T = L + FwdMap<PREC>::FLOATS + (threadIdx.x >> 6) * GC_SCRATCH_FLOATS;
@@ -475,7 +481,7 @@
             float tm, px, py, pz;
             sample_position(ox, oy, oz, dx, dy, dz, ts, te, tm, px, py, pz);
             float s0, gq[3], c[3];
-            decode_fwd<NEED_N, NEED_TEX, PREC, MASK>(L, dc, px, py, pz, rvalid, i, hi, s0, gq, c, p.h2_mask, sidx);
+            decode_fwd<NEED_N, NEED_TEX, PREC, MASK>(L, dc, px, py, pz, rvalid, i, hi, s0, gq, c, p.h2_mask, sidx, p.h1_mask);
             float nrm;
             const float sdf = s0 + sphere_bias(px, py, pz, cfg.sdf_bias_radius, nrm);
             if (rvalid && hi == 0 && !TT_DBG(cfg.flags, TT_DBG_NO_STORE)) {
@@ -493,7 +499,10 @@
             }
         }
     }
-    tile_stats_flush(st);
+    if constexpr (MASK == MASK_H1H2)
+        tile_stats_flush_late(st);
+    else
+        tile_stats_flush(st);
 }
 
 struct RenderEvalParams {
@@ -801,7 +810,7 @@
 static int render_fwd(const float* packed, const tt_mlp_weights* w, const float* rays_o, const float* rays_d,
                       const float* t_starts, const float* t_ends, const tt_render_cfg* cfg, float* opacity, float* depth,
                       float* rgb_fg, float* z_variance, float* normal_acc, float* weights, float* trans, float* sdf,
-                      float* sdf_grad, float* features, uint32_t* h2_mask, void* stream) {
+                      float* sdf_grad, float* features, uint32_t* h2_mask, uint32_t* h1_mask, void* stream) {
     int st = tt_validate_cfg(cfg);
     if (st != TT_OK) return st;
     if (!packed || !w || !rays_o || !rays_d || !t_starts || !t_ends || !opacity || !depth || !rgb_fg || !z_variance ||
@@ -817,13 +826,16 @@
     p.sdf_grad = sdf_grad;
     p.features = features;
     p.h2_mask = h2_mask;
+    p.h1_mask = h1_mask;
     hipStream_t s = (hipStream_t)stream;
     st = tt_plan_queue(cfg, (long long)cus * (DECODE_THREADS / 64), s, &p.geom, &p.n_items, &p.queue, 12);
     if (st != TT_OK) return st;
     const dim3 grid((unsigned)tt_persistent_blocks(p.n_items, cus, DECODE_THREADS / 64));
     tt_dispatch_prec(tt_prec_of_r(cfg->flags), [&](auto P) {
-        if (h2_mask)
-            hipLaunchKernelGGL((k_decode_rays<true, true, decltype(P)::value, true>), grid, dim3(DECODE_THREADS), 0, s, p);
+        if (h2_mask && h1_mask)
+            hipLaunchKernelGGL((k_decode_rays<true, true, decltype(P)::value, MASK_H1H2>), grid, dim3(DECODE_THREADS), 0, s, p);
+        else if (h2_mask)
+            hipLaunchKernelGGL((k_decode_rays<true, true, decltype(P)::value, MASK_H2>), grid, dim3(DECODE_THREADS), 0, s, p);
         else
             hipLaunchKernelGGL((k_decode_rays<true, true, decltype(P)::value>), grid, dim3(DECODE_THREADS), 0, s, p);
     });
@@ -838,7 +850,7 @@
                              float* depth, float* rgb_fg, float* z_variance, float* normal_acc, float* weights,
                              float* trans, float* sdf, float* sdf_grad, float* features, void* stream) {
     return render_fwd(packed, w, rays_o, rays_d, t_starts, t_ends, cfg, opacity, depth, rgb_fg, z_variance, normal_acc,
-                      weights, trans, sdf, sdf_grad, features, nullptr, stream);
+                      weights, trans, sdf, sdf_grad, features, nullptr, nullptr, stream);
 }
 
 extern "C" int tt_render_fwd_h2mask(const float* packed, const tt_mlp_weights* w, const float* rays_o,
@@ -848,7 +860,17 @@
                                     float* sdf_grad, float* features, uint32_t* h2_mask, void* stream) {
     if (!h2_mask) return TT_ERR_BAD_ARG;
     return render_fwd(packed, w, rays_o, rays_d, t_starts, t_ends, cfg, opacity, depth, rgb_fg, z_variance, normal_acc,
-                      weights, trans, sdf, sdf_grad, features, h2_mask, stream);
+                      weights, trans, sdf, sdf_grad, features, h2_mask, nullptr, stream);
+}
+
+extern "C" int tt_render_fwd_masks(const float* packed, const tt_mlp_weights* w, const float* rays_o,
+                                   const float* rays_d, const float* t_starts, const float* t_ends,
+                                   const tt_render_cfg* cfg, float* opacity, float* depth, float* rgb_fg,
+                                   float* z_variance, float* normal_acc, float* weights, float* trans, float* sdf,
+                                   float* sdf_grad, float* features, uint32_t* h2_mask, uint32_t* h1_mask, void* stream) {
+    if (!h2_mask || !h1_mask) return TT_ERR_BAD_ARG;
+    return render_fwd(packed, w, rays_o, rays_d, t_starts, t_ends, cfg, opacity, depth, rgb_fg, z_variance, normal_acc,
+                      weights, trans, sdf, sdf_grad, features, h2_mask, h1_mask, stream);
 }
 
 extern "C" int tt_decode_rays(const float* packed, const tt_mlp_weights* w, const float* rays_o, const float* rays_d,
@@ -869,6 +891,7 @@
     p.sdf_grad = sdf_grad;
     p.features = features;
     p.h2_mask = nullptr;
+    p.h1_mask = nullptr;
     hipStream_t s = (hipStream_t)stream;
     const long long slots = (long long)cus * (DECODE_THREADS / 64);
     int steps_per_item = 12, min_items_per_slot = 8;
diff --git a/triplaneturbo_amd/ops.py b/triplaneturbo_amd/ops.py
--- a/triplaneturbo_amd/ops.py
+++ b/triplaneturbo_amd/ops.py
@@ -169,6 +169,24 @@
     inv_std_t: Optional[Tensor] = None
     stats: Optional[Tensor] = None
     fwd_mask: bool = True
+    fwd_mask_h1: bool = True
+
+
+def sign_mask_bits(words: Tensor) -> Tensor:
+    if words.ndim != 2 or words.shape[1] != 2:
+        raise ValueError(f"sign-mask words: expected (n, 2), got {tuple(words.shape)}")
+    w = words.to(torch.int64) & 0xFFFFFFFF
+    e = torch.arange(64, device=words.device)
+    return ((w[:, (e >> 2) & 1] >> ((e & 3) + 4 * (e >> 3))[None, :]) & 1).bool()
+
+
+def sign_mask_words(bits: Tensor) -> Tensor:
+    if bits.ndim != 2 or bits.shape[1] != 64:
+        raise ValueError(f"sign-mask bits: expected (n, 64), got {tuple(bits.shape)}")
+    e = torch.arange(64, device=bits.device)
+    contrib = bits.to(torch.int64) << ((e & 3) + 4 * (e >> 3))[None, :]
+    w = torch.stack([contrib[:, ((e >> 2) & 1) == d].sum(dim=1) for d in (0, 1)], dim=1)
+    return torch.where(w >= 1 << 31, w - (1 << 32), w).to(torch.int32)
 
 
 def planes_pack(space_cache: Tensor) -> Tensor:
@@ -396,7 +414,10 @@
 
 def render_forward_raw(packed: Tensor, sdf_w: Sequence[Tensor], feat_w: Sequence[Tensor], rays_o: Tensor,
                        rays_d: Tensor, t_starts: Tensor, t_ends: Tensor, rays_per_view: int, rc: RenderConfig,
-                       per_sample: bool = True, image_w: int = 0, h2_mask: Union[bool, Tensor] = False):
+                       per_sample: bool = True, image_w: int = 0, h2_mask: Union[bool, Tensor] = False,
+                       h1_mask: Union[bool, Tensor] = False):
+    if h1_mask is not False and h2_mask is False:
+        raise ValueError("h1_mask needs h2_mask (tt_render_fwd_masks writes both)")
     packed, rays_o, rays_d, t_starts, t_ends = _ray_args(packed, rays_o, rays_d, t_starts, t_ends)
     n_rays, S = t_starts.shape
     cfg = _make_cfg(packed, n_rays, rays_per_view, S, rc, per_sample, image_w)
@@ -411,6 +432,15 @@
         out["h2_mask"] = _chk(h2_mask, "h2_mask", (n_rays * S, 2), torch.int32)
         if out["h2_mask"].data_ptr() != h2_mask.data_ptr():
             raise ValueError("h2_mask must be contiguous (the kernel writes it in place)")
+    if h1_mask is not False:
+        if h1_mask is True:
+            h1_mask = torch.empty((n_rays * S, 2), device=packed.device, dtype=torch.int32)
+        out["h1_mask"] = _chk(h1_mask, "h1_mask", (n_rays * S, 2), torch.int32)
+        if out["h1_mask"].data_ptr() != h1_mask.data_ptr():
+            raise ValueError("h1_mask must be contiguous (the kernel writes it in place)")
+        _launch("tt_render_fwd_masks", packed, wst, rays_o, rays_d, t_starts, t_ends, cfg, *out.values(),
+                label="tt_render_fwd")
+    elif h2_mask is not False:
         _launch("tt_render_fwd_h2mask", packed, wst, rays_o, rays_d, t_starts, t_ends, cfg, *out.values(),
                 label="tt_render_fwd")
     else:
@@ -537,6 +567,10 @@
     return _lib.MlpWeights(*[_ptr(t) for t in tensors])
 
 
+def _both_masks(rc: RenderConfig) -> bool:
+    return bool(rc.fwd_mask and rc.fwd_mask_h1 and rc.prec != "f32")
+
+
 class _TriplaneRenderFn(torch.autograd.Function):
 
     @staticmethod
@@ -547,7 +581,8 @@
             rc = dataclasses.replace(rc, inv_std_t=inv_std_t.detach())
         ctx.set_materialize_grads(False)
         raw = render_forward_raw(packed, (w1, w2, w3), (v1, v2, v3), rays_o, rays_d, t_starts, t_ends, rays_per_view,
-                                 rc, per_sample=True, image_w=image_w, h2_mask=need_grad and rc.fwd_mask)
+                                 rc, per_sample=True, image_w=image_w, h2_mask=need_grad and rc.fwd_mask,
+                                 h1_mask=need_grad and _both_masks(rc))
         ctx.rays_per_view = rays_per_view
         ctx.rc = rc
         ctx.image_w = image_w
@@ -555,7 +590,8 @@
         if need_grad:
             ctx.save_for_backward(packed, w1, w2, w3, v1, v2, v3, rays_o, rays_d, t_starts, t_ends, raw["opacity"],
                                   raw["depth"], raw["trans"], raw["weights"], raw["features"], raw["sdf"],
-                                  raw["sdf_grad"], *([raw["h2_mask"]] if rc.fwd_mask else []))
+                                  raw["sdf_grad"], *([raw["h2_mask"]] if rc.fwd_mask else []),
+                                  *([raw["h1_mask"]] if _both_masks(rc) else []))
         ctx.mark_non_differentiable(raw["trans"])
         return (raw["opacity"], raw["depth"], raw["rgb_fg"], raw["z_variance"], raw["normal_acc"], raw["weights"],
                 raw["sdf"], raw["sdf_grad"], raw["features"], raw["trans"])
@@ -565,7 +601,7 @@
     def backward(ctx, g_op, g_depth, g_rgb, g_zvar, g_nacc, g_weights, g_sdf, g_sdf_grad, g_features, _g_trans):
         (packed, w1, w2, w3, v1, v2, v3, rays_o, rays_d, t_starts, t_ends, opacity, depth, trans, weights,
          features, sdf, sdf_grad) = ctx.saved_tensors[:18]
-        h2_mask = ctx.saved_tensors[18:]
+        masks = ctx.saved_tensors[18:]
         n_rays, S = t_starts.shape
         cfg = _make_cfg(packed, n_rays, ctx.rays_per_view, S, ctx.rc, True, ctx.image_w, stats_row=1)
         cfg_tex = _make_cfg(packed, n_rays, ctx.rays_per_view, S, ctx.rc, True, ctx.image_w, stats_row=2)
@@ -581,9 +617,9 @@
         g_k_rays = None
         if ctx.needs_input_grad[14]:
             g_k_rays = torch.empty((n_rays,), device=packed.device, dtype=torch.float32)
-        _launch("tt_render_bwd_geo_h2mask" if h2_mask else "tt_render_bwd_geo", packed, wst, rays_o, rays_d, t_starts,
+        _launch(("tt_render_bwd_geo", "tt_render_bwd_geo_h2mask", "tt_render_bwd_geo_masks")[len(masks)], packed, wst, rays_o, rays_d, t_starts,
                 t_ends, cfg, opacity, depth, trans, sdf, sdf_grad, features, g_op, g_depth, g_rgb, g_zvar, g_nacc,
-                g_weights, g_sdf, g_sdf_grad, g_k_rays, workspace, grad_packed, gst, *h2_mask, label="tt_render_bwd_geo")
+                g_weights, g_sdf, g_sdf_grad, g_k_rays, workspace, grad_packed, gst, *masks, label="tt_render_bwd_geo")
         _launch("tt_render_bwd_tex", packed, wst, rays_o, rays_d, t_starts, t_ends, cfg_tex, weights, features, g_rgb,
                 g_features, grad_packed, gst, label="tt_render_bwd_tex")
         g_packed = None
```

Result: faster. 8.191 million (median of 6 runs) (+1.3%).
